# genome/breakdancer

Hardware: AMD Instinct MI355X
Metric: read-pairs/s, records resident in HBM -> scored SV table (SURVEY 8d timing i); end to end from BAM: config.timings.bam_to_table (vs_baseline is taken there) (higher is better)
Workload: dtype int32

## Files before the change

breakdancer_amd/csrc/bdx_api.hip:

```cpp
#include <hip/hip_runtime.h>

#include <algorithm>
#include <sys/mman.h>
#include <atomic>
#include <functional>
#include <chrono>
#include <cmath>
#include <cstdio>
#include <cstddef>
#include <cstring>
#include <string>
#include <thread>
#include <unordered_map>
#include <utility>
#include <vector>

#include "../../include/bdx.h"
#include "bdx_dev.h"
#include "bdx_k3.h"
#include "bdx_shard.h"
#include "bdx_scan.h"
#include "bdx_walk.h"
#include "bdx_bam_dev.h"

using namespace bdx;

namespace {

inline bool alloc_trace() { static const bool on = getenv("BDX_ALLOC_TRACE") != nullptr; return on; }

struct DevBuf {
    void* p = nullptr;
    size_t bytes = 0;
    hipError_t ensure(size_t b) {
        if (b <= bytes) return hipSuccess;
        const auto t0 = std::chrono::steady_clock::now();
        const bool had = p != nullptr;
        if (p) (void)hipFree(p);
        p = nullptr;
        bytes = 0;
        size_t want = b + b / 8 + 256;
        hipError_t e = hipMalloc(&p, want);
        if (alloc_trace()) fprintf(stderr, "[bdx alloc] device %12zu B %8.1f us%s\n", want, std::chrono::duration<double, std::micro>(std::chrono::steady_clock::now() - t0).count(), had ? " (regrown: hipFree first)" : "");
        if (e == hipSuccess) bytes = want;
        return e;
    }
    void release() { if (p) (void)hipFree(p); p = nullptr; bytes = 0; }
    template <class T> T* as() const { return (T*)p; }
};

struct PinBuf {
    void* p = nullptr;
    size_t bytes = 0;
    void* map_base = nullptr;
    size_t map_len = 0;
    static std::atomic<bool>& registered_switch() { static std::atomic<bool> on{true}; return on; }
    static bool use_registered() { return registered_switch().load(std::memory_order_relaxed); }
    hipError_t ensure(size_t b) {
        if (b <= bytes) return hipSuccess;
        release();
        size_t want = b + b / 8 + 256;
        const auto t0 = std::chrono::steady_clock::now();
        hipError_t e = hipErrorOutOfMemory;
        constexpr size_t kHuge = (size_t)2 << 20;
        if (want >= 2 * kHuge && use_registered()) {
            const size_t len = (want + kHuge - 1) & ~(kHuge - 1);
            void* base = mmap(nullptr, len + kHuge, PROT_READ | PROT_WRITE, MAP_PRIVATE | MAP_ANONYMOUS, -1, 0);
            if (base != MAP_FAILED) {
                void* al = (void*)(((uintptr_t)base + kHuge - 1) & ~(uintptr_t)(kHuge - 1));
                (void)madvise(al, len, MADV_HUGEPAGE);
                for (size_t o = 0; o < len; o += 4096) ((volatile char*)al)[o] = 0;
                void* dev = nullptr;
                if (hipHostRegister(al, len, hipHostRegisterMapped) == hipSuccess && hipHostGetDevicePointer(&dev, al, 0) == hipSuccess && dev == al) {
                    p = al; map_base = base; map_len = len + kHuge; want = len; e = hipSuccess;
                } else {
                    (void)hipHostUnregister(al);
                    (void)hipGetLastError();
                    munmap(base, len + kHuge);
                }
            }
        }
        if (e != hipSuccess) {
            e = hipHostMalloc(&p, want, hipHostMallocDefault);
            if (e == hipSuccess && want <= ((size_t)1 << 20)) memset(p, 0, want);
        }
        if (alloc_trace()) fprintf(stderr, "[bdx alloc] pinned %12zu B %8.1f us%s\n", want, std::chrono::duration<double, std::micro>(std::chrono::steady_clock::now() - t0).count(), map_base ? " (registered huge pages)" : "");
        if (e == hipSuccess) bytes = want; else p = nullptr;
        return e;
    }
    void release() {
        if (p && map_base) { (void)hipHostUnregister(p); munmap(map_base, map_len); }
        else if (p) (void)hipHostFree(p);
        p = nullptr; bytes = 0; map_base = nullptr; map_len = 0;
    }
    template <class T> T* as() const { return (T*)p; }
};

constexpr int kNumStages = 12;
constexpr int kK1MaxGrid = 8192;
constexpr uint32_t kK1EventPeriod = 4;

}

struct bdx_ctx {
    int device = 0;
    hipStream_t stream = nullptr;
    bdx_opts opts{};
    std::vector<bdx_lib> libs;
    int nlibs = 0, nbams = 0, ntids = 0, nkeys = 0, w0 = 0;
    std::string err;

    ReadsSoA d{};
    size_t n = 0, cap = 0;
    bool adopted = false;
    DevBuf b_tid, b_pos, b_mtid, b_mpos, b_isize, b_flag, b_qlen, b_mapq, b_lib, b_bam, b_key, b_check;
    bool groups_in_hbm = false;
    bool defer_walk = false;
    DevBuf b_groups;
    bool use_check = false;

    DevBuf b_libs, b_cls, b_tile_tot, b_tile_pre, b_tile_mono, b_blk_cnt, b_cnt, b_p1, b_fold, b_stash, b_chunk_tot;
    DevBuf b_c_tid, b_c_pos, b_c_isize, b_c_meta, b_c_key, b_c_check, b_c_idx, b_c_nn, b_c_pk;
    DevBuf b_cand, b_pre_q, b_pre_rev, b_pre_nonctx, b_c_first, b_c_maxq, b_c_rid, b_region_of, b_counts;
    DevBuf b_bcnt, b_boff, b_bcur, b_e_key, b_e_idx, b_partner, b_t_key, b_t_idx;
    DevBuf b_x_key, b_x_check, b_x_order, b_x_region, b_x_meta, b_x_isize, b_x_n;
    DevBuf b_lib_mean;
    DevBuf b_r_rec, b_r_pk, b_out_deg, b_parts, b_kdens, b_rs, b_slot, b_members, b_own, b_lib_stage, b_cn_stage,
        b_t_lambda, b_t_k, b_ws6;
    PinBuf h_p1, h_cnt, h_counts, h_regs, h_pk, h_groups, h_terms;
    DevBuf b_sv_src, b_dlists, b_ltail, b_pair_lo;
    PinBuf h_hs_rec, h_hs_aux, h_hs_lists, h_printed;
    DevBuf b_ins, b_member_ids;
    PinBuf h_flags;
    uint32_t seq = 0;
    int dbg_no_stash = 0, dbg_max_chunks = 0, dbg_ins_plain = 0, dbg_gather_walk = 0, dbg_regions_copy = 0, dbg_asm_plain = 0;
    uint32_t lb_seq = 0;
    float k1_ms_last = 0;
    bool k1_timed = false;
    bool stage_timing = false;
    bool poll = true;
    bool materialized = true;
    bool rows_packed = false;
    uint32_t n_sv_total = 0, n_groups_total = 0, n_terms_total = 0, n_cn_total = 0;
    PinBuf h_counts0, h_counts2, h_sv_out, h_lib_index, h_lib_pairs, h_cn_key, h_cn_value, h_ltail_dev;
    hipEvent_t ev_groups = nullptr, ev_regions = nullptr;
    int big_walk_mode = -1;
    int64_t last_big_groups = -1;
    FinalizeParams fp_deferred{};
    bool finalize2_deferred = false;
    bool bucketed_join = false;
    bool host_walk_only = false;
    K6Arrays k6{};
    const GroupRec* k6_in_groups = nullptr;
    const uint32_t* k6_in_goff = nullptr;
    bool force_direct_join = false;
    uint32_t k6_cap = 0;
    const RegionRec* k6_r_rec = nullptr;
    const uint32_t* k6_r_pk = nullptr;
    uint8_t* k6_taint = nullptr;
    const uint32_t* k3_tid_tail = nullptr;
    bool table_in_hbm = false;
    DevBuf b_sv_out, b_lib_index_out, b_lib_pairs_out, b_cn_key_out, b_cn_value_out, b_ltail_out, b_sv_key;

    bool ran = false;
    Pass1 p1{};
    StageCounts counts{};
    std::vector<uint32_t> cnt;
    std::vector<uint32_t> cnt_local;
    uint32_t g_covered = 0;
    int32_t g_window = 0;
    uint32_t nn_base = 0;
    int stage = 0;
    uint32_t ntiles = 0, tstride = 0;
    Compact cp{};
    K3Arrays k3{};
    K4Arrays k4{};
    std::vector<double> log_tail;
    bool collect_support = false;
    std::vector<uint32_t> ov_cnt;
    uint32_t ov_covered = 0;
    bool replayed = false;
    bool use_stash = false;
    std::atomic<int> sizing{0};
    std::string sizing_err;
    std::vector<uint32_t> sup_off;
    std::vector<uint64_t> sup_idx;
    std::vector<uint8_t> sup_flag;
    std::vector<float> seqcov, lib_density, key_density;
    std::vector<HostRegion> regions;
    std::vector<uint32_t> r_pk;
    const HostRegion* reg = nullptr;
    size_t nreg = 0;
    const uint32_t* rpk = nullptr;
    std::vector<GroupPart> parts;
    WalkResult walk;
    WalkScratch* walk_scratch = nullptr;
    uint32_t n_printed = 0;
    uint32_t n_sv_host = 0;
    int speculate = 2;
    int spec_test = 0;
    uint32_t last_na = 0;
    size_t last_n = 0;
    uint32_t na_alloc = 0;
    bool region_of_fused = false;
    uint32_t join_table_clean = 0;
    float stage_ms[kNumStages] = {0};
    hipEvent_t ev[8] = {nullptr};

    hipStream_t copy_stream = nullptr;
    hipEvent_t ev_copy = nullptr;
    bool copy_pending = false;
    bool k1_live = false;
    uint32_t k1_done = 0, k1_cap_tiles = 0;
    struct Stage {
        PinBuf buf;
        size_t cap = 0;
        hipEvent_t done = nullptr;
        bool busy = false;
    };
    Stage ring[4];
    int ring_next = 0, ring_cur = -1;
    struct KeySeg { uint64_t begin; const uint64_t* host; const uint16_t* host_qlen; const uint64_t* host_check; };
    std::vector<KeySeg> key_segs;
    DevBuf b_seg, b_lb;

    size_t cls_n = (size_t)-1;
    DevBuf b_jq, b_jc;
};

namespace {

thread_local std::string* t_err_sink = nullptr;
int fail(bdx_ctx* c, int code, const std::string& msg) {
    if (t_err_sink) *t_err_sink = msg;
    else if (c) c->err = msg;
    return code;
}
struct Sizing { uint32_t na; };
#define NOT_WHILE_SIZING(c)                                                                                                              \
    do {                                                                                                                                 \
        if ((c)->sizing.load(std::memory_order_acquire))                                                                                 \
            return fail(c, BDX_ESTATE, "the buffers of the later stages are being sized on another thread (bdx_bamdec_finish has not returned)"); \
    } while (0)
int hipfail(bdx_ctx* c, hipError_t e, const char* what) {
    return fail(c, BDX_EHIP, std::string(what) + ": " + hipGetErrorString(e));
}
#define HIPCHK(ctx, expr)                                   \
    do {                                                    \
        hipError_t _e = (expr);                             \
        if (_e != hipSuccess) return hipfail(ctx, _e, #expr); \
    } while (0)

size_t round_up(size_t x, size_t m) { return (x + m - 1) / m * m; }

hipError_t next_lb_stamp(bdx_ctx* c, uint32_t* out) {
    if (((++c->lb_seq) & 0x3FFFFFFFu) == 0) {
        if (c->b_lb.p) { const hipError_t e = hipMemsetAsync(c->b_lb.p, 0, c->b_lb.bytes, c->stream); if (e != hipSuccess) return e; }
        if (c->b_ws6.p) { const hipError_t e = hipMemsetAsync(c->b_ws6.p, 0, c->b_ws6.bytes, c->stream); if (e != hipSuccess) return e; }
        ++c->lb_seq;
    }
    *out = c->lb_seq & 0x3FFFFFFFu;
    return hipSuccess;
}

int alloc_reads(bdx_ctx* c, size_t cap) {
    cap = round_up(std::max<size_t>(cap, 1), 1024);
    if (cap <= c->cap) return BDX_OK;
    if (c->copy_stream) HIPCHK(c, hipStreamSynchronize(c->copy_stream));
    HIPCHK(c, hipStreamSynchronize(c->stream));
    c->k1_live = false;
    struct Col { DevBuf* b; size_t esz; const void** slot; };
    Col cols[] = {{&c->b_tid, 4, (const void**)&c->d.tid},     {&c->b_pos, 4, (const void**)&c->d.pos},
                  {&c->b_mtid, 4, (const void**)&c->d.mtid},   {&c->b_mpos, 4, (const void**)&c->d.mpos},
                  {&c->b_isize, 4, (const void**)&c->d.isize}, {&c->b_flag, 2, (const void**)&c->d.flag},
                  {&c->b_qlen, 2, (const void**)&c->d.qlen},   {&c->b_mapq, 1, (const void**)&c->d.mapq},
                  {&c->b_lib, 1, (const void**)&c->d.lib},     {&c->b_bam, 1, (const void**)&c->d.bam},
                  {&c->b_key, 8, (const void**)&c->d.key},     {&c->b_check, 8, (const void**)&c->d.check}};
    for (Col& col : cols) {
        if (col.b == &c->b_check && !c->use_check) continue;
        DevBuf nb;
        HIPCHK(c, nb.ensure(cap * col.esz));
        if (c->n) HIPCHK(c, hipMemcpyAsync(nb.p, col.b->p, c->n * col.esz, hipMemcpyDeviceToDevice, c->stream));
        HIPCHK(c, hipStreamSynchronize(c->stream));
        col.b->release();
        *col.b = nb;
        *col.slot = nb.p;
    }
    c->cap = cap;
    return BDX_OK;
}

void stage_view(const bdx_ctx::Stage& st, bdx_batch_buf* out) {
    char* p = (char*)st.buf.p;
    const size_t K = st.cap;
    out->name_key = (uint64_t*)p; p += K * 8;
    out->name_check = (uint64_t*)p; p += K * 8;
    out->tid = (int32_t*)p; p += K * 4;
    out->pos = (int32_t*)p; p += K * 4;
    out->mtid = (int32_t*)p; p += K * 4;
    out->mpos = (int32_t*)p; p += K * 4;
// ... 26 lines not shown
        if (tiles <= 0xFFFFFFFFull) {
            const int rc = pass1_prepare(c, (uint32_t)tiles);
            if (rc != BDX_OK) return rc;
            c->k1_live = true;
        }
    }
    hipStream_t s2 = s;
    HIPCHK(c, hipMemcpyAsync((void*)(c->d.tid + o), b.tid, n * 4, hipMemcpyHostToDevice, s));
    HIPCHK(c, hipMemcpyAsync((void*)(c->d.pos + o), b.pos, n * 4, hipMemcpyHostToDevice, s2));
    HIPCHK(c, hipMemcpyAsync((void*)(c->d.mtid + o), b.mtid, n * 4, hipMemcpyHostToDevice, s));
    HIPCHK(c, hipMemcpyAsync((void*)(c->d.mpos + o), b.mpos, n * 4, hipMemcpyHostToDevice, s2));
    HIPCHK(c, hipMemcpyAsync((void*)(c->d.isize + o), b.isize, n * 4, hipMemcpyHostToDevice, s));
    HIPCHK(c, hipMemcpyAsync((void*)(c->d.flag + o), b.flag, n * 2, hipMemcpyHostToDevice, s2));
    HIPCHK(c, hipMemcpyAsync((void*)(c->d.mapq + o), b.mapq, n, hipMemcpyHostToDevice, s2));
    if (c->nlibs > 1) HIPCHK(c, hipMemcpyAsync((void*)(c->d.lib + o), b.lib, n, hipMemcpyHostToDevice, s2));
    if (c->nbams > 1) HIPCHK(c, hipMemcpyAsync((void*)(c->d.bam + o), b.bam, n, hipMemcpyHostToDevice, s2));
    const uint64_t* dev_view = nullptr;
    const uint16_t* dev_qlen = nullptr;
    const uint64_t* dev_check = nullptr;
    if (lazy_keys && c->key_segs.size() < 64) {
        auto device_view = [](const void* hp) -> void* {
            hipPointerAttribute_t attr{};
            void* dp = nullptr;
            if (hipPointerGetAttributes(&attr, hp) == hipSuccess && attr.type == hipMemoryTypeHost &&
                hipHostGetDevicePointer(&dp, (void*)hp, 0) == hipSuccess)
                return dp;
            (void)hipGetLastError();
            return nullptr;
        };
        dev_view = (const uint64_t*)device_view(b.name_key);
        dev_qlen = dev_view ? (const uint16_t*)device_view(b.qlen) : nullptr;
        if (dev_qlen && c->use_check) dev_check = (const uint64_t*)device_view(b.name_check);
        if (!dev_qlen || (c->use_check && !dev_check)) dev_view = nullptr;
    }
    if (!dev_view) {
        HIPCHK(c, hipMemcpyAsync((void*)(c->d.key + o), b.name_key, n * 8, hipMemcpyHostToDevice, s2));
        HIPCHK(c, hipMemcpyAsync((void*)(c->d.qlen + o), b.qlen, n * 2, hipMemcpyHostToDevice, s));
        if (c->use_check) HIPCHK(c, hipMemcpyAsync((void*)(c->d.check + o), b.name_check, n * 8, hipMemcpyHostToDevice, s2));
    }
    if (c->key_segs.empty() || dev_view || c->key_segs.back().host)
        c->key_segs.push_back(bdx_ctx::KeySeg{(uint64_t)o, dev_view, dev_qlen, dev_check});
    HIPCHK(c, hipEventRecord(c->ev_copy, s));
    c->copy_pending = true;
    c->n += n;
    c->ran = false;
    if (c->k1_live) {
        const uint32_t full = (uint32_t)(c->n / kTile);
        if (full >= c->k1_done + kStreamTilesMin) {
            HIPCHK(c, hipStreamWaitEvent(c->stream, c->ev_copy, 0));
            c->copy_pending = false;
            const int rc = pass1_classify(c, full, false);
            if (rc != BDX_OK) return rc;
        }
    }
    return BDX_OK;
}

}

extern "C" {

void bdx_opts_default(bdx_opts* o) {
    if (!o) return;
    o->min_len = 7; o->cut_sd = 3; o->max_sd = 1000000000; o->min_map_qual = 35; o->min_read_pair = 2;
    o->seq_coverage_lim = 1000; o->buffer_size = 100; o->transchr_rearrange = 0; o->fisher = 0;
    o->illumina_long_insert = 0; o->cn_lib = 0; o->print_af = 0; o->score_threshold = 30; o->chr_restricted = 0;
}

const char* bdx_strerror(int code) {
    switch (code) {
        case BDX_OK: return "ok";
        case BDX_EINVAL: return "invalid argument";
        case BDX_ENOMEM: return "out of memory";
        case BDX_EHIP: return "HIP runtime error";
        case BDX_ESTATE: return "call out of order";
        case BDX_ELIMIT: return "limit exceeded";
        default: return "internal error";
    }
}
const char* bdx_last_error(const bdx_ctx* ctx) { return ctx ? ctx->err.c_str() : ""; }
int bdx_device(const bdx_ctx* ctx) { return ctx ? ctx->device : -1; }
void* bdx_stream(const bdx_ctx* ctx) { return ctx ? (void*)ctx->stream : nullptr; }

int bdx_create(bdx_ctx** out, const bdx_opts* opts, const bdx_lib* libs, int nlibs, int nbams, int ntids,
               int max_read_window_size0, int device) {
    if (!out || !opts || !libs || nlibs < 1 || nbams < 1) return BDX_EINVAL;
    if (nlibs > 255 || nbams > 254) return BDX_ELIMIT;
    const int nkeys = opts->cn_lib ? nlibs : nbams;
    if (nkeys > 60) return BDX_ELIMIT;
    for (int i = 0; i < nlibs; ++i)
        if (libs[i].bam_index < 0 || libs[i].bam_index >= nbams) return BDX_EINVAL;
    int ndev = 0;
    if (hipGetDeviceCount(&ndev) != hipSuccess || ndev <= 0 || device < 0 || device >= ndev) return BDX_EHIP;
    if (hipSetDevice(device) != hipSuccess) return BDX_EHIP;
    bdx_ctx* c = new (std::nothrow) bdx_ctx;
    if (!c) return BDX_ENOMEM;
    c->device = device;
    c->opts = *opts;
    c->libs.assign(libs, libs + nlibs);
    c->nlibs = nlibs; c->nbams = nbams; c->ntids = ntids; c->nkeys = nkeys; c->w0 = max_read_window_size0;
    if (hipStreamCreateWithFlags(&c->stream, hipStreamNonBlocking) != hipSuccess) { delete c; return BDX_EHIP; }
    for (auto& e : c->ev)
        if (hipEventCreate(&e) != hipSuccess) { delete c; return BDX_EHIP; }
    if (hipStreamCreateWithFlags(&c->copy_stream, hipStreamNonBlocking) != hipSuccess) { delete c; return BDX_EHIP; }
    if (hipEventCreateWithFlags(&c->ev_copy, hipEventDisableTiming) != hipSuccess) { delete c; return BDX_EHIP; }
    for (auto& st : c->ring)
        if (hipEventCreateWithFlags(&st.done, hipEventDisableTiming) != hipSuccess) { delete c; return BDX_EHIP; }
    if (hipEventCreateWithFlags(&c->ev_groups, hipEventDisableTiming) != hipSuccess) { delete c; return BDX_EHIP; }
    if (hipEventCreateWithFlags(&c->ev_regions, hipEventDisableTiming) != hipSuccess) { delete c; return BDX_EHIP; }
    std::vector<DevLib> dl(nlibs);
    for (int i = 0; i < nlibs; ++i) {
        dl[i].upper = libs[i].uppercutoff;
        dl[i].lower = libs[i].lowercutoff;
        dl[i].min_mapq = libs[i].min_mapping_quality < 0 ? opts->min_map_qual : libs[i].min_mapping_quality;
        dl[i].key = opts->cn_lib ? i : libs[i].bam_index;
    }
    std::vector<float> means(nlibs);
    for (int i = 0; i < nlibs; ++i) means[i] = libs[i].mean_insertsize;
    if (c->b_libs.ensure(nlibs * sizeof(DevLib)) != hipSuccess ||
        hipMemcpy(c->b_libs.p, dl.data(), nlibs * sizeof(DevLib), hipMemcpyHostToDevice) != hipSuccess ||
        c->b_lib_mean.ensure(nlibs * 4) != hipSuccess ||
        hipMemcpy(c->b_lib_mean.p, means.data(), nlibs * 4, hipMemcpyHostToDevice) != hipSuccess) {
        bdx_destroy(c);
        return BDX_EHIP;
    }
    *out = c;
    return BDX_OK;
}

void bdx_destroy(bdx_ctx* c) {
    if (!c) return;
    (void)hipSetDevice(c->device);
    if (c->copy_stream) (void)hipStreamSynchronize(c->copy_stream);
    if (c->stream) (void)hipStreamSynchronize(c->stream);
    for (auto& st : c->ring) {
        st.buf.release();
        if (st.done) (void)hipEventDestroy(st.done);
    }
    c->b_seg.release();
    c->b_lb.release();
    if (c->ev_copy) (void)hipEventDestroy(c->ev_copy);
    if (c->copy_stream) (void)hipStreamDestroy(c->copy_stream);
    DevBuf* bufs[] = {&c->b_tid, &c->b_pos, &c->b_mtid, &c->b_mpos, &c->b_isize, &c->b_flag, &c->b_qlen, &c->b_mapq, &c->b_lib,
                      &c->b_bam, &c->b_key, &c->b_check, &c->b_c_check, &c->b_x_check, &c->b_groups, &c->b_libs, &c->b_cls, &c->b_stash, &c->b_chunk_tot, &c->b_tile_tot, &c->b_tile_pre, &c->b_tile_mono,
                      &c->b_blk_cnt, &c->b_cnt, &c->b_p1, &c->b_c_tid, &c->b_c_pos, &c->b_c_isize,
                      &c->b_c_meta, &c->b_c_key, &c->b_c_idx, &c->b_c_nn, &c->b_c_pk, &c->b_cand, &c->b_pre_q, &c->b_pre_rev,
                      &c->b_pre_nonctx, &c->b_c_first, &c->b_c_maxq, &c->b_c_rid, &c->b_region_of,
                      &c->b_counts, &c->b_bcnt, &c->b_boff, &c->b_bcur, &c->b_e_key, &c->b_e_idx, &c->b_partner, &c->b_t_key,
                      &c->b_t_idx, &c->b_x_key, &c->b_x_order, &c->b_x_region,
                      &c->b_x_meta, &c->b_x_isize, &c->b_x_n, &c->b_fold, &c->b_lib_mean, &c->b_pair_lo, &c->b_sv_src, &c->b_dlists, &c->b_ltail, &c->b_r_rec, &c->b_r_pk, &c->b_out_deg,
                      &c->b_parts, &c->b_kdens, &c->b_rs, &c->b_slot, &c->b_members, &c->b_own, &c->b_lib_stage,
                      &c->b_cn_stage, &c->b_t_lambda, &c->b_t_k, &c->b_ws6, &c->b_ins, &c->b_member_ids,
                      &c->b_sv_out, &c->b_lib_index_out, &c->b_lib_pairs_out, &c->b_cn_key_out, &c->b_cn_value_out, &c->b_ltail_out, &c->b_sv_key,
                      &c->b_jq, &c->b_jc};
    for (DevBuf* b : bufs) b->release();
    PinBuf* pins[] = {&c->h_p1, &c->h_cnt, &c->h_counts, &c->h_regs, &c->h_pk, &c->h_groups, &c->h_terms, &c->h_flags, &c->h_hs_rec, &c->h_hs_aux, &c->h_hs_lists, &c->h_printed, &c->h_counts0, &c->h_counts2,
                      &c->h_sv_out, &c->h_lib_index, &c->h_lib_pairs, &c->h_cn_key, &c->h_cn_value, &c->h_ltail_dev};
    for (PinBuf* b : pins) b->release();
    if (c->walk_scratch) walk_scratch_free(c->walk_scratch);
    for (auto& e : c->ev)
        if (e) (void)hipEventDestroy(e);
    if (c->ev_groups) (void)hipEventDestroy(c->ev_groups);
    if (c->ev_regions) (void)hipEventDestroy(c->ev_regions);
    if (c->stream) (void)hipStreamDestroy(c->stream);
    delete c;
}

int bdx_reserve(bdx_ctx* c, size_t n_reads) {
    if (!c) return BDX_EINVAL;
    if (c->adopted) return fail(c, BDX_ESTATE, "reads were adopted from the caller");
    NOT_WHILE_SIZING(c);
    HIPCHK(c, hipSetDevice(c->device));
    const int rc = alloc_reads(c, n_reads);
    if (rc != BDX_OK) return rc;
    if (n_reads >= (1u << 20) && !c->ran) {
        const uint64_t prior = (uint64_t)n_reads / 32 + 4096;
        if (prior <= kMaxAnomalous) return presize_stages_here(c, (uint32_t)prior);
    }
    return BDX_OK;
}

int bdx_push(bdx_ctx* c, const bdx_batch* b) {
    if (!c || !b) return BDX_EINVAL;
    if (c->adopted) return fail(c, BDX_ESTATE, "reads were adopted from the caller");
    if (b->n == 0) return BDX_OK;
    if (!b->tid || !b->pos || !b->mtid || !b->mpos || !b->isize || !b->flag || !b->qlen || !b->mapq || !b->lib || !b->bam ||
        !b->name_key || (c->use_check && !b->name_check))
        return fail(c, BDX_EINVAL, "null array in batch");
    HIPCHK(c, hipSetDevice(c->device));
    return enqueue_batch(c, *b, true);
}

int bdx_acquire_batch(bdx_ctx* c, size_t capacity, bdx_batch_buf* out) {
    if (!c || !out || capacity == 0) return BDX_EINVAL;
    if (c->adopted) return fail(c, BDX_ESTATE, "reads were adopted from the caller");
    if (c->ring_cur >= 0) return fail(c, BDX_ESTATE, "the previous batch was not submitted");
    HIPCHK(c, hipSetDevice(c->device));
    bdx_ctx::Stage& st = c->ring[c->ring_next];
    if (st.busy) {
        HIPCHK(c, hipEventSynchronize(st.done));
        st.busy = false;
    }
    st.cap = round_up(capacity, 64);
    HIPCHK(c, st.buf.ensure(st.cap * 43 + 64));
    stage_view(st, out);
    c->ring_cur = c->ring_next;
    c->ring_next = (c->ring_next + 1) % 4;
    return BDX_OK;
}

int bdx_submit_batch(bdx_ctx* c, size_t n) {
    if (!c) return BDX_EINVAL;
    if (c->ring_cur < 0) return fail(c, BDX_ESTATE, "no batch was acquired");
    bdx_ctx::Stage& st = c->ring[c->ring_cur];
    c->ring_cur = -1;
    if (n == 0) return BDX_OK;
    HIPCHK(c, hipSetDevice(c->device));
    bdx_batch_buf v{};
    stage_view(st, &v);
    if (n > v.capacity) return fail(c, BDX_EINVAL, "more records than the acquired batch holds");
    bdx_batch b{v.tid, v.pos, v.mtid, v.mpos, v.isize, v.flag, v.qlen, v.mapq, v.lib, v.bam, v.name_key, n, v.name_check};
    const int rc = enqueue_batch(c, b, false);
    if (rc != BDX_OK) return rc;
    HIPCHK(c, hipEventRecord(st.done, c->copy_stream));
    st.busy = true;
    return BDX_OK;
}

int bdx_reset_reads(bdx_ctx* c) {
    if (!c) return BDX_EINVAL;
    HIPCHK(c, hipSetDevice(c->device));
    if (c->copy_stream) HIPCHK(c, hipStreamSynchronize(c->copy_stream));
    HIPCHK(c, hipStreamSynchronize(c->stream));
    if (c->adopted) {
        c->d = ReadsSoA{};
        c->cap = 0;
        c->adopted = false;
    }
    c->n = 0;
    c->ran = false;
    c->cls_n = (size_t)-1;
    c->k1_live = false;
    c->k1_done = 0;
    c->copy_pending = false;
    c->key_segs.clear();
    c->ring_cur = -1;
    for (auto& st : c->ring) st.busy = false;
    return BDX_OK;
}

int bdx_set_device_reads(bdx_ctx* c, const bdx_batch* b) {
    if (!c || !b) return BDX_EINVAL;
    if (c->n && !c->adopted) return fail(c, BDX_ESTATE, "context already holds pushed reads");
    const void* ptrs[] = {b->tid, b->pos, b->mtid, b->mpos, b->isize, b->flag, b->qlen, b->mapq, b->lib, b->bam, b->name_key,
                          c->use_check ? (const void*)b->name_check : (const void*)b->name_key};
    for (const void* p : ptrs)
        if (b->n && (!p || ((uintptr_t)p & 15))) return fail(c, BDX_EINVAL, "device arrays must be non-null and 16-byte aligned");
    c->d.tid = b->tid; c->d.pos = b->pos; c->d.mtid = b->mtid; c->d.mpos = b->mpos; c->d.isize = b->isize;
    c->d.flag = b->flag; c->d.qlen = b->qlen; c->d.mapq = b->mapq; c->d.lib = b->lib; c->d.bam = b->bam; c->d.key = b->name_key;
    c->d.check = c->use_check ? b->name_check : nullptr;
    c->n = b->n;
    c->cap = b->n;
    c->adopted = true;
    c->ran = false;
    c->cls_n = (size_t)-1;
    c->k1_live = false;
    c->key_segs.clear();
    return BDX_OK;
}

}

namespace {

bool wait_flag(const bdx_ctx* c, int idx, uint32_t value) {
    if (!c->poll || !c->h_flags.p) return false;
    volatile uint32_t* f = (volatile uint32_t*)c->h_flags.p + idx;
    const auto t0 = std::chrono::steady_clock::now();
    for (uint32_t spin = 0;; ++spin) {
        if (*f == value) { std::atomic_thread_fence(std::memory_order_acquire); return true; }
        __builtin_ia32_pause();
        if ((spin & 1023u) == 1023u && std::chrono::steady_clock::now() - t0 > std::chrono::milliseconds(200)) return false;
    }
}

bool flag_arrived(const bdx_ctx* c, int idx) {
    return !c->poll || !c->h_flags.p || ((volatile uint32_t*)c->h_flags.p)[idx] == c->seq;
}

int signal_ready(bdx_ctx* c, int idx, hipEvent_t ev) {
    if (c->poll) {
        if (hipStreamWriteValue32(c->stream, c->h_flags.as<uint32_t>() + idx, c->seq, 0) == hipSuccess) return BDX_OK;
        (void)hipGetLastError();
        c->poll = false;
    }
    if (ev) {
        hipError_t e = hipEventRecord(ev, c->stream);
        if (e != hipSuccess) return hipfail(c, e, "hipEventRecord");
    }
    return BDX_OK;
}

float ms_between(std::chrono::steady_clock::time_point a, std::chrono::steady_clock::time_point b) {
    return std::chrono::duration<float, std::milli>(b - a).count();
}

int do_pass1(bdx_ctx* c, uint32_t na_cap = 0, bool wait = true, bool defer_second = false);
int wait_pass1(bdx_ctx* c);

int pass1_prepare(bdx_ctx* c, uint32_t tiles_cap) {
    HIPCHK(c, hipSetDevice(c->device));
    hipStream_t s = c->stream;
    const int nlibs = c->nlibs, nbams = c->nbams, nkeys = c->nkeys;
    const int ncols = 2 + nkeys, ncnt = nlibs * kNumFlags + nlibs + nbams;
    const uint32_t tstride = (uint32_t)round_up(std::max<uint32_t>(tiles_cap, 16), 16);
    c->tstride = tstride;
    c->k1_cap_tiles = tiles_cap;
    c->k1_done = 0;
    HIPCHK(c, c->b_cls.ensure(std::max<size_t>((size_t)tiles_cap * kTile, 16)));
    c->use_stash = !c->dbg_no_stash && nkeys <= kStashKeys;
    if (c->use_stash) HIPCHK(c, c->b_stash.ensure(std::max<size_t>((size_t)tiles_cap * kStashCap * sizeof(StashRec), 64)));
    HIPCHK(c, c->b_tile_tot.ensure((size_t)ncols * tstride * 4));
    HIPCHK(c, c->b_tile_pre.ensure((size_t)ncols * tstride * 4));
    HIPCHK(c, c->b_tile_mono.ensure((size_t)nbams * tstride * sizeof(MonoRec)));
    HIPCHK(c, c->b_blk_cnt.ensure((size_t)kCntCopies * ncnt * 4));
    HIPCHK(c, c->b_cnt.ensure((size_t)ncnt * 4));
    HIPCHK(c, c->b_p1.ensure(sizeof(Pass1)));
    HIPCHK(c, c->h_p1.ensure(sizeof(Pass1)));
    HIPCHK(c, c->h_cnt.ensure((size_t)ncnt * 4));
    HIPCHK(c, c->h_counts.ensure(sizeof(StageCounts)));
    HIPCHK(c, c->b_counts.ensure(sizeof(StageCounts)));
    const size_t w_tot = (size_t)ncols * tstride, w_mono = (size_t)nbams * tstride * sizeof(MonoRec) / 4;
    if (w_tot > 0xFFFFFFFFull || w_mono > 0xFFFFFFFFull) {
        HIPCHK(c, hipMemsetAsync(c->b_tile_tot.p, 0, w_tot * 4, s));
        HIPCHK(c, hipMemsetAsync(c->b_tile_mono.p, 0xFF, w_mono * 4, s));
    }
    InitList il{};
    int k = 0;
    auto add = [&](void* p, size_t words, uint32_t value) { il.ptr[k] = (uint32_t*)p; il.words[k] = (uint32_t)words; il.value[k] = value; ++k; };
    if (w_tot <= 0xFFFFFFFFull && w_mono <= 0xFFFFFFFFull) { add(c->b_tile_tot.p, w_tot, 0u); add(c->b_tile_mono.p, w_mono, 0xFFFFFFFFu); }
    add(c->b_blk_cnt.p, (size_t)kCntCopies * ncnt, 0u);
    add(c->b_p1.p, sizeof(Pass1) / 4, 0u);
    add(c->b_counts.p, sizeof(StageCounts) / 4, 0u);
    il.n = k;
    launch_init(il, s);
    return BDX_OK;
}

int pass1_classify(bdx_ctx* c, uint32_t upto, bool timed) {
    hipStream_t s = c->stream;
    if (upto <= c->k1_done) return BDX_OK;
    K1Params k1{};
    k1.r = c->d; k1.n = c->n; k1.ntiles = upto; k1.tstride = c->tstride; k1.tile0 = c->k1_done;
    k1.nlibs = c->nlibs; k1.nbams = c->nbams; k1.nkeys = c->nkeys;
    k1.max_sd = c->opts.max_sd; k1.opt_t = c->opts.transchr_rearrange; k1.opt_l = c->opts.illumina_long_insert;
    k1.libs = c->b_libs.as<DevLib>(); k1.cls = c->b_cls.as<uint8_t>(); k1.tile_tot = c->b_tile_tot.as<uint32_t>();
    k1.tile_mono = c->b_tile_mono.as<MonoRec>();
    k1.blk_cnt = c->b_blk_cnt.as<uint32_t>();
    k1.stash = c->use_stash ? c->b_stash.as<StashRec>() : nullptr;
    const uint32_t span = upto - c->k1_done;
    const int grid1 = (int)std::min<uint32_t>((span + kWaves - 1) / kWaves, (uint32_t)kK1MaxGrid);
    launch_k1(k1, grid1, k1_lds_bytes(c->nlibs, c->nbams, c->nkeys), s, timed ? c->ev[0] : nullptr, timed ? c->ev[1] : nullptr);
    c->k1_done = upto;
    return BDX_OK;
}

int do_pass1(bdx_ctx* c, uint32_t na_cap, bool wait, bool defer_second) {
    HIPCHK(c, hipSetDevice(c->device));
    hipStream_t s = c->stream;
    const int nlibs = c->nlibs, nbams = c->nbams, nkeys = c->nkeys;
    const int ncols = 2 + nkeys, ncnt = nlibs * kNumFlags + nlibs + nbams;
    if (c->n >= ((size_t)1 << 32)) return fail(c, BDX_ELIMIT, "more than 2^32 - 1 reads in one context (read indices and the prefix counters are 32-bit)");
    const uint32_t ntiles = (uint32_t)((c->n + kTile - 1) / kTile);
    c->ntiles = ntiles;
    c->ran = false; c->stage = 0; c->replayed = false;
    c->cls_n = (size_t)-1;
    c->na_alloc = 0;
    c->regions.clear(); c->r_pk.clear(); c->parts.clear();
    c->reg = nullptr; c->nreg = 0; c->rpk = nullptr;
    c->walk.clear();
    if (!c->walk_scratch) c->walk_scratch = walk_scratch_new();
    c->n_printed = 0;
    memset(&c->counts, 0, sizeof(c->counts));
    for (float& m : c->stage_ms) m = 0;

    if (c->copy_pending) {
        HIPCHK(c, hipStreamWaitEvent(s, c->ev_copy, 0));
        c->copy_pending = false;
    }
    if (!(c->k1_live && c->k1_cap_tiles >= ntiles)) {
        const int rc = pass1_prepare(c, ntiles);
        if (rc != BDX_OK) return rc;
    }
    c->k1_live = false;
    const uint32_t tstride = c->tstride;
    const bool time_k1 = (c->stage_timing || c->seq % kK1EventPeriod == 0) && c->k1_done == 0 && ntiles > 0;
    {
        const int rc = pass1_classify(c, ntiles, time_k1);
        if (rc != BDX_OK) return rc;
    }
    FinalizeParams fp{};
    fp.ntiles = ntiles; fp.tstride = tstride; fp.nblk = 0;
    fp.nfold = std::max<uint32_t>(1, std::min<uint32_t>(64, (ntiles + 1023) / 1024));
    HIPCHK(c, c->b_fold.ensure((size_t)nbams * fp.nfold * sizeof(MonoRec)));
    fp.fold_part = c->b_fold.as<MonoRec>();
    fp.nlibs = nlibs; fp.nbams = nbams; fp.nkeys = nkeys; fp.ncols = ncols; fp.ncnt = ncnt; fp.w0 = c->w0;
    fp.tile_tot = c->b_tile_tot.as<uint32_t>(); fp.tile_pre = c->b_tile_pre.as<uint32_t>(); fp.tile_mono = c->b_tile_mono.as<MonoRec>();
    {
        const uint32_t nsuper = (ntiles + kK2TilesPerWave - 1) / kK2TilesPerWave;
        const uint32_t round = 4096;
        const uint32_t rounds = std::max<uint32_t>(1, (nsuper + round - 1) / round);
        const uint32_t max_chunks = c->dbg_max_chunks > 0 ? (uint32_t)std::min(c->dbg_max_chunks, (int)kMaxChunks) : (uint32_t)kMaxChunks;
        fp.chunk_super = round * ((rounds + max_chunks - 1) / max_chunks);
        fp.nchunk = std::max<uint32_t>(1, (nsuper + fp.chunk_super - 1) / fp.chunk_super);
        HIPCHK(c, c->b_chunk_tot.ensure((size_t)ncols * kMaxChunks * 8));
        fp.chunk_tot = c->b_chunk_tot.as<uint32_t>();
        fp.chunk_base = fp.chunk_tot + (size_t)ncols * kMaxChunks;
    }
    fp.blk_cnt = c->b_blk_cnt.as<uint32_t>(); fp.cnt = c->b_cnt.as<uint32_t>(); fp.p1 = c->b_p1.as<Pass1>();
    HIPCHK(c, c->b_kdens.ensure(64 * 4));
    fp.libs = c->b_libs.as<DevLib>(); fp.cn_lib = c->opts.cn_lib; fp.key_density = c->b_kdens.as<float>();
    fp.cnt_host = c->h_cnt.as<uint32_t>(); fp.p1_host = c->h_p1.as<Pass1>();
    memset(c->h_p1.p, 0, sizeof(Pass1));
    HIPCHK(c, c->h_flags.ensure(64));
    ++c->seq;
    fp.flag_host = c->h_flags.as<uint32_t>(); fp.flag_value = c->seq;
    fp.na_cap = na_cap;
    c->fp_deferred = fp;
    c->finalize2_deferred = defer_second;
    launch_finalize(fp, s, !defer_second);
    c->k1_timed = time_k1;
    return wait ? wait_pass1(c) : BDX_OK;
}

int wait_pass1(bdx_ctx* c) {
    const int ncnt = c->nlibs * kNumFlags + c->nlibs + c->nbams;
    if (!wait_flag(c, 0, c->seq)) {
        HIPCHK(c, hipStreamSynchronize(c->stream));
        if (c->h_flags.p && *((volatile uint32_t*)c->h_flags.p) != c->seq) return fail(c, BDX_EINTERNAL, "the pass-1 record did not arrive: its kernel was not launched");
    }
    c->p1 = *c->h_p1.as<Pass1>();
    c->cnt_local.assign(c->h_cnt.as<uint32_t>(), c->h_cnt.as<uint32_t>() + ncnt);
    if (c->k1_timed) {
        float ms = 0;
        if (hipEventElapsedTime(&ms, c->ev[0], c->ev[1]) == hipSuccess) c->k1_ms_last = ms;
    }
    c->stage_ms[0] = c->k1_ms_last;
    if (c->p1.n_anom > kMaxAnomalous) return fail(c, BDX_ELIMIT, "more than 2^31 anomalous reads in one context");
    if (!c->na_alloc && c->p1.n_anom) c->na_alloc = (uint32_t)std::min<uint64_t>((uint64_t)c->p1.n_anom + c->p1.n_anom / 8 + 1024, kMaxAnomalous);
    c->stage = 1;
    c->cls_n = c->n;
    return BDX_OK;
}

int32_t window_from(const bdx_ctx* c, const uint32_t* cnt, uint32_t covered) {
    int W = c->w0;
    for (int i = 0; i < c->nlibs; ++i) {
        const int nd = (int)(cnt[i * kNumFlags + F_LARGE] + cnt[i * kNumFlags + F_SMALL]);
        const int tmp = nd > 0 ? (int)((float)covered / (float)nd) : 50;
        W = std::min(W, tmp);
    }
    return W;
}

int set_pass1(bdx_ctx* c, const uint32_t* cnt, uint32_t covered, int32_t window, bool upload) {
    const int nlibs = c->nlibs, nkeys = c->nkeys;
    const int ncnt = nlibs * kNumFlags + nlibs + c->nbams;
    c->cnt.assign(cnt, cnt + ncnt);
    c->g_covered = covered;
    c->g_window = window;
    const uint32_t* lib_cnt = c->cnt.data() + nlibs * kNumFlags;
    const uint32_t* bam_cnt = lib_cnt + nlibs;
    c->seqcov.assign(nlibs, 0.f);
    c->lib_density.assign(nlibs, 0.f);
    c->key_density.assign(nkeys, 0.000001f);
    for (int i = 0; i < nlibs; ++i) {
        float covg = 0;
        if (lib_cnt[i] != 0 && covered != 0) covg = float(lib_cnt[i]) * c->libs[i].readlens / covered;
        c->seqcov[i] = covg;
        float dens = 0.000001f;
        if (c->opts.cn_lib) {
            if (lib_cnt[i] != 0) dens = float(lib_cnt[i]) / covered;
        } else {
            dens = float(bam_cnt[c->libs[i].bam_index]) / covered;
        }
        c->lib_density[i] = dens;
        c->key_density[c->opts.cn_lib ? i : c->libs[i].bam_index] = dens;
    }
    struct { uint32_t covered; int32_t window; } hdr{covered, window};
    static_assert(offsetof(Pass1, covered_ref_len) == 0 && offsetof(Pass1, window) == 4, "Pass1 header layout");
    if (upload) {
        HIPCHK(c, hipMemcpyAsync(c->b_p1.p, &hdr, sizeof(hdr), hipMemcpyHostToDevice, c->stream));
        HIPCHK(c, hipStreamSynchronize(c->stream));
    }
    c->stage = 2;
    return BDX_OK;
}

int do_compact(bdx_ctx* c, uint32_t nn_base, const uint32_t* pk_base, bool prepare_join, const Sizing* sz = nullptr) {
    HIPCHK(c, hipSetDevice(c->device));
    hipStream_t s = c->stream;
    const int nkeys = c->nkeys;
    const uint32_t na = sz ? sz->na : c->na_alloc;
    if (c->stage_timing && !sz) HIPCHK(c, hipEventRecord(c->ev[2], s));
    Compact cp_sz{};
    K3Arrays k3_sz{};
    Compact& cp = sz ? cp_sz : c->cp;
    K3Arrays& k3 = sz ? k3_sz : c->k3;
    cp = Compact{};
    k3 = K3Arrays{};
    if (na) {
        if (na > kMaxAnomalous) return fail(c, BDX_ELIMIT, "more than 2^31 anomalous reads in one context");
        const size_t cap = na;
        HIPCHK(c, c->b_c_tid.ensure(cap * 4)); HIPCHK(c, c->b_c_pos.ensure(cap * 4)); HIPCHK(c, c->b_c_isize.ensure(cap * 4));
        HIPCHK(c, c->b_c_meta.ensure(cap * 4)); HIPCHK(c, c->b_c_key.ensure(cap * 8)); HIPCHK(c, c->b_c_nn.ensure(cap * 4));
        HIPCHK(c, c->b_c_idx.ensure(cap * 4));
        if (c->use_check) HIPCHK(c, c->b_c_check.ensure(cap * 8));
        HIPCHK(c, c->b_c_pk.ensure(cap * 4 * nkeys));
        cp.tid = c->b_c_tid.as<int32_t>(); cp.pos = c->b_c_pos.as<int32_t>(); cp.isize = c->b_c_isize.as<int32_t>();
        cp.meta = c->b_c_meta.as<uint32_t>(); cp.key = c->b_c_key.as<uint64_t>(); cp.nn = c->b_c_nn.as<uint32_t>();
        cp.idx = c->b_c_idx.as<uint32_t>();
        cp.check = c->use_check ? c->b_c_check.as<uint64_t>() : nullptr;
        cp.pk = c->b_c_pk.as<uint32_t>(); cp.cap = na;
        K2Params k2{};
        k2.r = c->d; k2.n = c->n; k2.ntiles = c->ntiles; k2.tstride = c->tstride; k2.nkeys = nkeys; k2.nlibs = c->nlibs; k2.libs = c->b_libs.as<DevLib>();
        k2.cls = c->b_cls.as<uint8_t>(); k2.tile_pre = c->b_tile_pre.as<uint32_t>(); k2.c = cp;
        k2.tile_tot = c->b_tile_tot.as<uint32_t>(); k2.stash = c->use_stash ? c->b_stash.as<StashRec>() : nullptr;
        k2.chunk_tot = c->fp_deferred.chunk_tot; k2.chunk_base = c->fp_deferred.chunk_base; k2.chunk_super = c->fp_deferred.chunk_super;
        k2.nn_base = nn_base;
        for (int k = 0; k < nkeys; ++k) k2.pk_base[k] = pk_base ? pk_base[k] : 0u;
        HIPCHK(c, c->b_c_maxq.ensure(cap * 4));
        k2.fill_ptr[0] = c->b_c_maxq.as<uint32_t>(); k2.fill_words[0] = na; k2.fill_value[0] = 0u;
        if (!sz) c->join_table_clean = 0;
        if (prepare_join && (c->force_direct_join || (!c->bucketed_join && na <= kDirectJoinMax))) {
            const uint32_t slots = direct_join_slots(na);
            HIPCHK(c, c->b_t_key.ensure((size_t)slots * 8)); HIPCHK(c, c->b_partner.ensure((size_t)na * 4));
            k2.fill_ptr[1] = c->b_t_key.as<uint32_t>(); k2.fill_words[1] = 2 * slots; k2.fill_value[1] = 0xFFFFFFFFu;
            k2.fill_ptr[2] = c->b_partner.as<uint32_t>(); k2.fill_words[2] = na; k2.fill_value[2] = 0xFFFFFFFFu;
            HIPCHK(c, c->b_pair_lo.ensure((size_t)na * 4));
            k2.fill_ptr[3] = c->b_pair_lo.as<uint32_t>(); k2.fill_words[3] = na; k2.fill_value[3] = 0xFFFFFFFFu;
            if (!sz) c->join_table_clean = slots;
        }
        if (sz) return BDX_OK;
        {
            bool any_host = false;
            for (auto const& sg : c->key_segs) any_host |= sg.host != nullptr;
            if (any_host && !c->adopted) {
                const size_t ns = c->key_segs.size();
                std::vector<uint64_t> tab(4 * ns + 1);
                for (size_t i = 0; i < ns; ++i) {
                    const bdx_ctx::KeySeg& sg = c->key_segs[i];
                    tab[i] = sg.begin;
                    tab[ns + 1 + i] = (uint64_t)(uintptr_t)(sg.host ? sg.host - sg.begin : c->d.key);
                    tab[2 * ns + 1 + i] = (uint64_t)(uintptr_t)(sg.host ? sg.host_qlen - sg.begin : c->d.qlen);
                    tab[3 * ns + 1 + i] = (uint64_t)(uintptr_t)(sg.host ? sg.host_check - sg.begin : c->d.check);
                }
                tab[ns] = c->n;
                HIPCHK(c, c->b_seg.ensure(tab.size() * 8));
                HIPCHK(c, hipMemcpyAsync(c->b_seg.p, tab.data(), tab.size() * 8, hipMemcpyHostToDevice, s));
                HIPCHK(c, hipStreamSynchronize(s));
                k2.nseg = (int)ns;
                k2.seg_begin = c->b_seg.as<uint64_t>();
                k2.seg_ptr = (const uint64_t* const*)(c->b_seg.as<uint64_t>() + ns + 1);
                k2.seg_qlen = (const uint16_t* const*)(c->b_seg.as<uint64_t>() + 2 * ns + 1);
                k2.seg_check = (const uint64_t* const*)(c->b_seg.as<uint64_t>() + 3 * ns + 1);
            }
        }
        launch_k2(k2, k2_lds_bytes(nkeys), s, c->finalize2_deferred ? &c->fp_deferred : nullptr);
        c->finalize2_deferred = false;
    }
    if (sz) return BDX_OK;
    if (c->finalize2_deferred) {
        launch_finalize2_only(c->fp_deferred, s);
        c->finalize2_deferred = false;
    }
    if (c->stage_timing) HIPCHK(c, hipEventRecord(c->ev[3], s));
    c->nn_base = nn_base;
    return BDX_OK;
}

// ... 84 lines not shown
    K4Arrays& k4 = sz ? k4_sz : c->k4;
    k4 = K4Arrays{};
    if (!n) return BDX_OK;
    k4.g_cap = n / 2 + 1;
    if (c->groups_in_hbm) {
        HIPCHK(c, c->b_groups.ensure((size_t)k4.g_cap * sizeof(GroupRec)));
        k4.g_rec = c->b_groups.as<GroupRec>();
    } else {
        HIPCHK(c, c->h_groups.ensure((size_t)k4.g_cap * sizeof(GroupRec)));
        k4.g_rec = c->h_groups.as<GroupRec>();
    }
    const size_t n_own = en.n_local ? std::min<size_t>(n, std::max<uint32_t>(c->na_alloc, 1u)) : n;
    HIPCHK(c, c->b_partner.ensure(n_own * 4));
    k4.partner = c->b_partner.as<int32_t>();
    if (sz) return BDX_OK;
    if (c->force_direct_join || (!c->bucketed_join && n <= kDirectJoinMax)) {
        uint32_t slots = direct_join_slots(n);
        if (c->join_table_clean && (uint64_t)n * 2 <= c->join_table_clean) slots = c->join_table_clean;
        const bool want_lo = en.c_rid || en.want_pair_lo;
        if (c->join_table_clean != slots) {
            HIPCHK(c, c->b_t_key.ensure((size_t)slots * 8));
            HIPCHK(c, hipMemsetAsync(c->b_t_key.p, 0xFF, (size_t)slots * 8, s));
            HIPCHK(c, hipMemsetAsync(c->b_partner.p, 0xFF, n_own * 4, s));
            if (en.want_pair_lo) {
                HIPCHK(c, c->b_pair_lo.ensure(n_own * 4));
                HIPCHK(c, hipMemsetAsync(c->b_pair_lo.p, 0xFF, n_own * 4, s));
            }
        }
        k4.pair_lo = ((c->join_table_clean == slots && want_lo) || en.want_pair_lo) ? c->b_pair_lo.as<int32_t>() : nullptr;
        c->join_table_clean = 0;
        k4.direct = 1; k4.t_mask = slots - 1;
        k4.t_key = c->b_t_key.as<uint64_t>(); k4.t_idx = c->b_t_idx.as<int32_t>();
        if (join_only) launch_k4_join_only(k4, en, n_ptr, n, c->b_counts.as<StageCounts>(), s);
        else launch_k4(k4, en, n_ptr, n, c->b_counts.as<StageCounts>(), s);
        return BDX_OK;
    }
    uint32_t nb = 1, lg = 0;
    while (nb < (uint32_t)kMaxBuckets && (size_t)nb * 384 < n) { nb <<= 1; ++lg; }
    k4.nbuckets = nb; k4.log2b = lg;
    if ((size_t)nb * 4 > c->b_bcnt.bytes) {
        HIPCHK(c, c->b_bcnt.ensure((size_t)kMaxBuckets * 4));
        HIPCHK(c, hipMemsetAsync(c->b_bcnt.p, 0, c->b_bcnt.bytes, s));
    }
    HIPCHK(c, c->b_boff.ensure((nb + 1) * 4)); HIPCHK(c, c->b_bcur.ensure(nb * 4));
    HIPCHK(c, c->b_e_key.ensure((size_t)n * 8)); HIPCHK(c, c->b_e_idx.ensure((size_t)n * 4));
    HIPCHK(c, c->b_t_key.ensure((size_t)n * 16)); HIPCHK(c, c->b_t_idx.ensure((size_t)n * 8));
    k4.bcnt = c->b_bcnt.as<uint32_t>(); k4.boff = c->b_boff.as<uint32_t>(); k4.bcur = c->b_bcur.as<uint32_t>();
    k4.e_key = c->b_e_key.as<uint64_t>(); k4.e_idx = c->b_e_idx.as<uint32_t>();
    k4.t_key = c->b_t_key.as<uint64_t>(); k4.t_idx = c->b_t_idx.as<int32_t>();
    if (join_only) launch_k4_join_only(k4, en, n_ptr, n, c->b_counts.as<StageCounts>(), s);
    else launch_k4(k4, en, n_ptr, n, c->b_counts.as<StageCounts>(), s);
    return BDX_OK;
}

int readback(bdx_ctx* c, bool with_groups) {
    hipStream_t s = c->stream;
    const uint32_t na = c->p1.n_anom;
    if (!na) return BDX_OK;
    HIPCHK(c, hipMemcpyAsync(c->h_counts.p, c->b_counts.p, sizeof(StageCounts), hipMemcpyDeviceToHost, s));
    HIPCHK(c, hipStreamSynchronize(s));
    HIPCHK(c, hipGetLastError());
    c->counts = *c->h_counts.as<StageCounts>();
    if (c->counts.overflow) return fail(c, BDX_EINTERNAL, "group list overflow");
    (void)with_groups;
    return BDX_OK;
}

constexpr uint32_t kBorrowRegionsMin = 32768;
void decode_regions(bdx_ctx* c, const RegionRec* rr, const uint32_t* pk, uint32_t nr, uint32_t ph, bool borrow) {
    static_assert(sizeof(HostRegion) == sizeof(RegionRec) && offsetof(HostRegion, first) == offsetof(RegionRec, first), "region layout");
    const int nkeys = c->nkeys;
    if (borrow && !ph) {
        c->reg = (const HostRegion*)rr; c->nreg = nr; c->rpk = pk;
        return;
    }
    c->regions.resize(nr + ph);
    if (ph) c->regions[0] = HostRegion{-1, -1, -1, 0, 0, 0, 0, 0, 0};
    if (nr) memcpy(c->regions.data() + ph, rr, (size_t)nr * sizeof(RegionRec));
    c->r_pk.assign((size_t)ph * 2 * nkeys, 0u);
    c->r_pk.insert(c->r_pk.end(), pk, pk + (size_t)nr * 2 * nkeys);
    c->reg = c->regions.data(); c->nreg = c->regions.size(); c->rpk = c->r_pk.data();
}

void decode_groups(bdx_ctx* c, const GroupRec* gr, uint32_t ng, uint32_t ph) {
    c->parts.resize(ng);
    for (uint32_t i = 0; i < ng; ++i) {
        const uint64_t k = gr[i].key;
        c->parts[i] = GroupPart{(uint32_t)(k >> 38) + ph, (uint32_t)((k >> 12) & ((1u << 26) - 1)) + ph, (uint8_t)(k & 15),
                                (uint8_t)((k >> 4) & 255), gr[i].pairs, gr[i].sum_isize};
    }
}

int do_k6(bdx_ctx* c, bool force_host, int part = 0, const Sizing* sz = nullptr, int rounds = 0) {
    hipStream_t s = c->stream;
    K6Arrays a_sz{};
    K6Arrays& a = sz ? a_sz : c->k6;
    if (part == 2) {
        if (!a.cap) return BDX_OK;
        launch_k6_components(a, a.cap, s);
        if (!c->poll) {
            const int rc = signal_ready(c, 1, c->ev_groups);
            if (rc != BDX_OK) return rc;
        }
        if (!c->defer_walk) launch_k6_walk(a, a.cap, s);
        return BDX_OK;
    }
    if (part == 3) {
        if (a.cap) launch_k6_walk(a, a.cap, s);
        return BDX_OK;
    }
    const uint32_t na = std::max(sz ? sz->na : c->na_alloc, c->k6_cap);
    const int nkeys = c->nkeys, nlibs = c->nlibs;
    a = K6Arrays{};
    if (!na) return BDX_OK;
    const size_t cap = na;
    HIPCHK(c, c->b_out_deg.ensure(cap * 6 * 4));
    HIPCHK(c, c->b_parts.ensure(cap * sizeof(PartRec)));
    HIPCHK(c, c->b_rs.ensure(cap * sizeof(RegSum)));
    HIPCHK(c, c->b_members.ensure(cap * kK6MaxMembers * sizeof(MemberInfo)));
    HIPCHK(c, c->b_own.ensure(cap * 7 * 4 + 64 * 4 * 4));
    const int big_walk = c->big_walk_mode >= 0 ? c->big_walk_mode : (c->last_big_groups >= 0 ? c->last_big_groups > 2000 : na > 500000u);
    if (big_walk) HIPCHK(c, c->b_member_ids.ensure(cap * kK6BigMembers * 4));
    a.sv_cap = na / 2 + 1; a.term_cap = na / 2 + 1; a.cn_cap = (na / 2 + 1) * (uint32_t)nkeys;
    a.lib_stride = (uint32_t)std::min(nlibs, kK6LibStride);
    HIPCHK(c, c->b_slot.ensure(cap * sizeof(SvOut)));
    HIPCHK(c, c->b_lib_stage.ensure(cap * a.lib_stride * sizeof(LibStage)));
    HIPCHK(c, c->b_cn_stage.ensure(cap * (size_t)nkeys * sizeof(CnStage) + 16));
    HIPCHK(c, c->b_t_lambda.ensure((size_t)a.term_cap * 8)); HIPCHK(c, c->b_t_k.ensure((size_t)a.term_cap * 4));
    const size_t nblk = scan_grid(na, 1) + 1;
    if (c->table_in_hbm) {
        HIPCHK(c, c->b_sv_out.ensure((size_t)a.sv_cap * sizeof(SvOut))); HIPCHK(c, c->b_sv_key.ensure((size_t)a.sv_cap * 8));
        HIPCHK(c, c->b_lib_index_out.ensure((size_t)a.term_cap * 4)); HIPCHK(c, c->b_lib_pairs_out.ensure((size_t)a.term_cap * 4));
        HIPCHK(c, c->b_cn_key_out.ensure((size_t)a.cn_cap * 4 + 16)); HIPCHK(c, c->b_cn_value_out.ensure((size_t)a.cn_cap * 4 + 16));
        HIPCHK(c, c->b_ltail_out.ensure((size_t)a.term_cap * 8));
    } else {
        HIPCHK(c, c->h_sv_out.ensure((size_t)a.sv_cap * sizeof(SvOut)));
        HIPCHK(c, c->h_lib_index.ensure((size_t)a.term_cap * 4)); HIPCHK(c, c->h_lib_pairs.ensure((size_t)a.term_cap * 4));
        HIPCHK(c, c->h_cn_key.ensure((size_t)a.cn_cap * 4 + 16)); HIPCHK(c, c->h_cn_value.ensure((size_t)a.cn_cap * 4 + 16));
        HIPCHK(c, c->h_ltail_dev.ensure((size_t)a.term_cap * 8));
    }
    HIPCHK(c, c->h_counts2.ensure(sizeof(StageCounts)));
    HIPCHK(c, c->b_sv_src.ensure((size_t)a.sv_cap * 16)); HIPCHK(c, c->b_ltail.ensure((size_t)a.term_cap * 8));
    HIPCHK(c, c->b_dlists.ensure((size_t)a.term_cap * 4 + (size_t)a.cn_cap * 8 + 64));
    {
        size_t p2 = 1;
        while (p2 < a.sv_cap) p2 <<= 1;
        const size_t svc = a.sv_cap;
        const size_t nsort = std::min<size_t>(svc, kK6RankSortMax);
        HIPCHK(c, c->b_ins.ensure(p2 * 12 + svc * 8 + (svc + 1) * 16 + nsort * 12 + nsort * 4 * kK6RankSlices + 64));
        a.old_key = c->b_ins.as<uint64_t>(); a.hs_key_dev = a.old_key + p2;
        a.old_slot = (uint32_t*)(a.hs_key_dev + svc); a.ins_T = a.old_slot + p2; a.ins_src = a.ins_T + svc + 1;
        a.ins_pre_l = a.ins_src + svc + 1; a.ins_pre_c = a.ins_pre_l + svc + 1;
        a.sorted_key = (uint64_t*)(((uintptr_t)(a.ins_pre_c + svc + 1) + 7) & ~(uintptr_t)7); a.sorted_slot = (uint32_t*)(a.sorted_key + nsort);
        a.rank_part = a.sv_cap > 2048u ? a.sorted_slot + nsort : nullptr;
    }
    a.sv_begin = c->b_sv_src.as<uint2>(); a.sv_src = (uint32_t*)(a.sv_begin + a.sv_cap); a.ltail = c->b_ltail.as<double>();
    a.d_lib_index = c->b_dlists.as<int32_t>(); a.d_cn_key = a.d_lib_index + a.term_cap; a.d_cn_value = (float*)(a.d_cn_key + a.cn_cap);
    a.cap = na;
    a.r_rec = c->k6_r_rec ? c->k6_r_rec : c->b_r_rec.as<RegionRec>(); a.r_pk = c->k6_r_pk ? c->k6_r_pk : c->b_r_pk.as<uint32_t>();
    a.taint = c->k6_taint;
    a.region_of = c->k3.region_of; a.partner = c->k4.partner; a.pair_lo = c->k4.pair_lo; a.meta = c->cp.meta; a.isize = c->cp.isize;
    a.in_groups = c->k6_in_groups; a.in_goff = c->k6_in_goff; a.first_of = c->k6_in_groups ? c->k6_in_goff : nullptr;
    a.parts = c->b_parts.as<PartRec>();
    a.rs = c->b_rs.as<RegSum>();
    a.out_deg = c->b_out_deg.as<uint32_t>(); a.label = a.out_deg + cap; a.bad_v = a.out_deg + 2 * cap; a.bad = a.out_deg + 3 * cap;
    a.mcount = a.out_deg + 4 * cap; a.pcount = a.out_deg + 5 * cap;
    a.members = c->b_members.as<MemberInfo>();
    a.own_nsv = c->b_own.as<uint32_t>(); a.own_nacc = a.own_nsv + cap; a.own_ncn = a.own_nsv + 2 * cap; a.own_first = a.own_nsv + 3 * cap; a.slot_next = a.own_nsv + 4 * cap; a.owners = a.own_nsv + 5 * cap; a.owners_big = a.own_nsv + 6 * cap; a.emit_part = a.own_nsv + 7 * cap;
    a.member_ids = big_walk ? c->b_member_ids.as<uint32_t>() : nullptr;
    a.sv_stage = c->b_slot.as<SvOut>(); a.lib_stage = c->b_lib_stage.as<LibStage>(); a.cn_stage = c->b_cn_stage.as<CnStage>();
    if (c->table_in_hbm) {
        a.sv_out = c->b_sv_out.as<SvOut>(); a.lib_index = c->b_lib_index_out.as<int32_t>(); a.lib_pairs = c->b_lib_pairs_out.as<int32_t>();
        a.cn_key = c->b_cn_key_out.as<int32_t>(); a.cn_value = c->b_cn_value_out.as<float>();
        a.sv_key = c->b_sv_key.as<unsigned long long>();
    } else {
        a.sv_out = c->h_sv_out.as<SvOut>(); a.lib_index = c->h_lib_index.as<int32_t>(); a.lib_pairs = c->h_lib_pairs.as<int32_t>();
        a.cn_key = c->h_cn_key.as<int32_t>(); a.cn_value = c->h_cn_value.as<float>();
    }
    a.sv_vx = a.sv_key ? a.sv_src + a.sv_cap : nullptr;
    a.t_lambda = c->b_t_lambda.as<double>(); a.t_k = c->b_t_k.as<int32_t>();
    a.g_rec = c->k4.g_rec; a.g_cap = c->k4.g_cap;
    {
        const size_t words = 4 * nblk;
        if (c->b_ws6.bytes < words * 8) {
            HIPCHK(c, c->b_ws6.ensure(words * 8));
            HIPCHK(c, hipMemsetAsync(c->b_ws6.p, 0, c->b_ws6.bytes, s));
        }
        a.lb_state = c->b_ws6.as<unsigned long long>();
        if (!sz) HIPCHK(c, next_lb_stamp(c, &a.lb_stamp));
    }
    if (sz) return BDX_OK;
    a.counts = c->b_counts.as<StageCounts>();
    a.hist = c->b_cnt.as<uint32_t>();
    a.key_density = c->b_kdens.as<float>();
    a.lib_mean = c->b_lib_mean.as<float>();
    a.counts_host = c->h_counts.as<StageCounts>();
    a.counts_host2 = c->h_counts2.as<StageCounts>();
    memset(c->h_counts.p, 0, sizeof(StageCounts));
    memset(c->h_counts2.p, 0, sizeof(StageCounts));
    a.p1 = c->b_p1.as<Pass1>();
    a.nlibs = nlibs; a.nkeys = nkeys; a.min_read_pair = c->opts.min_read_pair; a.chr_restricted = c->opts.chr_restricted;
    a.period = std::max(1, c->opts.buffer_size + 1);
    a.force_host = force_host ? 1 : 0;
    a.big_walk = big_walk;
    a.ins_plain = c->dbg_ins_plain;
    a.asm_plain = c->dbg_asm_plain;
    a.propagation_rounds = rounds ? rounds : (a.big_walk ? kK6LabelRoundsBig : kK6LabelRounds);
    if (c->poll) {
        a.flag_value = c->seq;
        a.flag_groups = c->h_flags.as<uint32_t>() + 1;
        if (c->k3.host_copy_later) a.flag_regions = c->h_flags.as<uint32_t>() + 3;
        a.mirror_in_walk = (force_host || c->defer_walk) ? 0 : 1;
    }
    if (part == 4) return BDX_OK;
    if (part == 1) {
        launch_k6_pairs(a, na, s);
        return BDX_OK;
    }
    launch_k6_groups(a, na, s);
    if (!c->poll) {
        const int rc = signal_ready(c, 1, c->ev_groups);
        if (rc != BDX_OK) return rc;
    }
    launch_k6_walk(a, na, s);
    return BDX_OK;
}

int presize_stages(bdx_ctx* c, uint32_t na) {
    struct Guard {
        bdx_ctx* c;
        std::string* keep;
        explicit Guard(bdx_ctx* c_) : c(c_), keep(t_err_sink) { c->sizing.fetch_add(1, std::memory_order_acq_rel); c->sizing_err.clear(); t_err_sink = &c->sizing_err; }
        ~Guard() { t_err_sink = keep; c->sizing.fetch_sub(1, std::memory_order_acq_rel); }
    } guard(c);
    const Sizing sz{na};
    int r = do_compact(c, 0, nullptr, true, &sz);
    if (r == BDX_OK) r = do_cut(c, 0, 0, 0, true, false, &sz);
    if (r == BDX_OK) r = do_join_local(c, na, Entries{}, nullptr, true, &sz);
    if (r == BDX_OK) r = do_k6(c, false, 0, &sz);
    return r;
}

int presize_stages_here(bdx_ctx* c, uint32_t na) {
    const int r = presize_stages(c, na);
    if (r != BDX_OK) c->err = c->sizing_err;
    return r;
}

int do_k6_table(bdx_ctx* c) {
    hipStream_t s = c->stream;
    K6Arrays& a = c->k6;
    const uint32_t na = a.cap;
    if (!na) return BDX_OK;
    const WalkResult& H = c->walk;
    const uint32_t nh = (uint32_t)H.svs.size(), nt = (uint32_t)H.terms.size(), nc = (uint32_t)H.cn_key.size();
    a.nh = nh;
    if (nh) {
        const uint64_t period = (uint64_t)std::max(1, c->opts.buffer_size + 1);
        HIPCHK(c, c->h_hs_rec.ensure((size_t)nh * sizeof(SvOut)));
        HIPCHK(c, c->h_hs_aux.ensure((size_t)nh * 12 + 16));
        HIPCHK(c, c->h_hs_lists.ensure((size_t)nt * 16 + (size_t)nc * 8 + 16));
        memcpy(c->h_hs_rec.p, H.svs.data(), (size_t)nh * sizeof(HostSv));
        uint64_t* hkey = c->h_hs_aux.as<uint64_t>();
        uint32_t* hcnt = (uint32_t*)(hkey + nh);
        for (uint32_t j = 0; j < nh; ++j) {
            const uint64_t key = H.sv_key[j];
            const bool from_old = !((key >> 32) & 1ull);
            const uint64_t start = key & 0xffffffffull;
            const uint64_t T = from_old ? (key >> 33) * period : start;
            hkey[j] = (T << 34) | (from_old ? 0ull : 1ull << 33) | (start << 7);
            if (a.force_host) hkey[j] = 0;
            hcnt[j] = (uint32_t)H.svs[j].sv.lib_count | ((uint32_t)H.svs[j].sv.cn_count << 16);
        }
        double* lam = c->h_hs_lists.as<double>();
        int32_t* li = (int32_t*)(lam + nt);
        int32_t* lp = li + nt;
        int32_t* ck = lp + nt;
        float* cv = (float*)(ck + nc);
        for (uint32_t i = 0; i < nt; ++i) { lam[i] = H.terms[i].lambda; li[i] = H.lib_index[i]; lp[i] = H.lib_pairs[i]; }
        for (uint32_t i = 0; i < nc; ++i) { ck[i] = H.cn_key[i]; cv[i] = H.cn_value[i]; }
        a.hs_rec = c->h_hs_rec.as<SvOut>(); a.hs_key = hkey; a.hs_cnt = hcnt;
        a.hs_lambda = lam; a.hs_lib_index = li; a.hs_lib_pairs = lp; a.hs_cn_key = ck; a.hs_cn_value = cv;
    }
    a.ltail_host = c->table_in_hbm ? c->b_ltail_out.as<double>() : (c->opts.fisher ? c->h_ltail_dev.as<double>() : nullptr);
    a.fin_regions = (c->counts.n_regions && c->counts.n_regions <= na) ? c->counts.n_regions : na;
    HIPCHK(c, c->h_printed.ensure((size_t)k6_score_grid(a) * 4));
    a.printed_host = c->h_printed.as<uint32_t>();
    if (c->poll) { a.flag_done = c->h_flags.as<uint32_t>() + 2; a.flag_value = c->seq; }
    a.wire_rows = c->table_in_hbm ? 0 : 1;
    c->rows_packed = a.wire_rows != 0;
    launch_k6_table(a, na, std::log(10), c->opts.score_threshold, c->opts.fisher ? 0 : 1, s);
    if (!a.flag_done) {
        const int rc = signal_ready(c, 2, nullptr);
        if (rc != BDX_OK) return rc;
    }
    return BDX_OK;
}

int materialize(bdx_ctx* c) {
    if (c->materialized) return BDX_OK;
    WalkResult& M = c->walk;
    M.clear();
    const uint32_t n = c->n_sv_total, nt = c->n_terms_total, nc = c->n_cn_total;
    if (c->rows_packed) {
        const SvWire* w = c->h_sv_out.as<SvWire>();
        M.svs.resize(n);
        int32_t lb = 0, cb = 0;
        for (uint32_t i = 0; i < n; ++i) {
            const SvWire& r = w[i];
            HostSv& o = M.svs[i];
            bdx_sv& v = o.sv;
            const HostRegion& ra = c->reg[r.region[0]];
            const HostRegion& rb = r.region[1] >= 0 ? c->reg[r.region[1]] : ra;
            v.chr[0] = ra.tid; v.chr[1] = rb.tid;
            v.pos[0] = r.pos[0]; v.pos[1] = r.pos[1];
            v.fwd[0] = (int32_t)(ra.n - ra.rev); v.rev[0] = (int32_t)ra.rev;
            v.fwd[1] = (int32_t)(rb.n - rb.rev); v.rev[1] = (int32_t)rb.rev;
            v.flag = (int32_t)((r.bits >> 16) & 15u); v.size = r.size; v.score = r.score; v.num_reads = r.num_reads; v.printed = (int32_t)((r.bits >> 23) & 1u);
            v.region[0] = r.region[0]; v.region[1] = r.region[1];
            v.lib_begin = lb; v.lib_count = (int32_t)(r.bits & 255u); lb += v.lib_count;
            v.cn_begin = cb; v.cn_count = (int32_t)((r.bits >> 8) & 255u); cb += v.cn_count;
            v.allele_frequency = r.allele_frequency; v.logp = r.logp;
            o.grp_mask = (r.bits >> 20) & 7u; o.start = r.start;
        }
    } else {
        const HostSv* d = c->h_sv_out.as<HostSv>();
        M.svs.assign(d, d + n);
    }
    M.lib_index.assign(c->h_lib_index.as<int32_t>(), c->h_lib_index.as<int32_t>() + nt);
    M.lib_pairs.assign(c->h_lib_pairs.as<int32_t>(), c->h_lib_pairs.as<int32_t>() + nt);
    M.cn_key.assign(c->h_cn_key.as<int32_t>(), c->h_cn_key.as<int32_t>() + nc);
    M.cn_value.assign(c->h_cn_value.as<float>(), c->h_cn_value.as<float>() + nc);
    if (c->opts.fisher) c->log_tail.assign(c->h_ltail_dev.as<double>(), c->h_ltail_dev.as<double>() + nt); else c->log_tail.clear();
    M.n_groups = c->n_groups_total;
    c->materialized = true;
    return BDX_OK;
}

int finish_table(bdx_ctx* c) {
    hipStream_t s = c->stream;
    const auto tf0 = std::chrono::steady_clock::now();
    if (!wait_flag(c, 2, c->seq)) {
        HIPCHK(c, hipStreamSynchronize(s));
        if (!flag_arrived(c, 2)) return fail(c, BDX_EINTERNAL, "the SV table did not arrive: its kernels were not launched");
    }
    const auto tf1 = std::chrono::steady_clock::now();
    static_assert(sizeof(HostSv) == sizeof(SvOut) && offsetof(HostSv, grp_mask) == offsetof(SvOut, grp_mask) &&
                      offsetof(HostSv, start) == offsetof(SvOut, start), "SV record layout");
    c->n_sv_host = (uint32_t)c->walk.svs.size();
    c->n_groups_total = c->walk.n_groups + c->counts.n_groups_dev;
    const StageCounts c2 = *c->h_counts2.as<StageCounts>();
    if (c2.overflow) return fail(c, BDX_EINTERNAL, "SV list overflow");
    c->n_sv_total = c2.n_sv_dev; c->n_terms_total = c2.n_terms_dev; c->n_cn_total = c2.n_cn_dev;
    c->counts.n_sv_dev = c2.n_sv_dev - c->n_sv_host;
    {
        const uint32_t g = c->k6.printed_host ? k6_score_grid(c->k6) : 0u;
        const uint32_t* pb = c->k6.printed_host;
        uint32_t np = 0;
        for (uint32_t i = 0; i < g; ++i) np += pb[i];
        c->n_printed = np;
    }
    c->counts.n_old = c2.n_old;
    c->materialized = false;
    if (c->opts.fisher && !c->table_in_hbm) {
        materialize(c);
        finish_scores(c->opts, c->log_tail.data(), c->walk.svs.data(), c->walk.svs.size(), &c->n_printed);
    }
    const auto tf2 = std::chrono::steady_clock::now();
    c->stage_ms[8] = ms_between(tf0, tf1);
    c->stage_ms[9] = ms_between(tf1, tf2);
    c->stage_ms[10] = 0;
    c->ran = true;
    c->stage = 4;
    return BDX_OK;
}

int host_walk(bdx_ctx* c, int32_t last_maxq, bool any_anomalous) {
    HIPCHK(c, hipSetDevice(c->device));
    WalkInput wi{};
    wi.opts = c->opts; wi.libs = c->libs.data(); wi.nlibs = c->nlibs; wi.nbams = c->nbams; wi.nkeys = c->nkeys;
    wi.hist = c->cnt.data(); wi.covered_ref_len = c->g_covered; wi.key_density = c->key_density.data();
    wi.regions = c->reg; wi.nregions = c->nreg; wi.r_pk = c->rpk; wi.parts = &c->parts; wi.last_maxq = last_maxq;
    wi.any_anomalous = any_anomalous;
    c->walk.clear();
    if (!c->parts.empty()) greedy_walk(wi, c->walk_scratch, c->walk);
    return BDX_OK;
}

int score_host_terms(bdx_ctx* c) {
    hipStream_t s = c->stream;
    const uint32_t nt = (uint32_t)c->walk.terms.size();
    if (nt) {
        HIPCHK(c, c->h_terms.ensure((size_t)nt * 20 + 16));
        double* hl = c->h_terms.as<double>();
        int32_t* hk = (int32_t*)(hl + nt);
        double* ho = (double*)((char*)c->h_terms.p + (((size_t)nt * 12 + 7) & ~(size_t)7));
        for (uint32_t i = 0; i < nt; ++i) { hl[i] = c->walk.terms[i].lambda; hk[i] = c->walk.terms[i].k; }
        launch_k5(hl, hk, ho, nt, s);
    }
    return BDX_OK;
}

int finish_host_walk(bdx_ctx* c) {
    hipStream_t s = c->stream;
    HIPCHK(c, hipStreamSynchronize(s));
    HIPCHK(c, hipGetLastError());
    const uint32_t nt = (uint32_t)c->walk.terms.size();
    const double* host_tail = nt ? (const double*)((char*)c->h_terms.p + (((size_t)nt * 12 + 7) & ~(size_t)7)) : nullptr;
    c->log_tail.assign(host_tail, host_tail + nt);
    finish_scores(c->opts, c->log_tail.data(), c->walk.svs.data(), c->walk.svs.size(), &c->n_printed);
    c->n_sv_host = c->n_sv_total = (uint32_t)c->walk.svs.size();
    c->n_terms_total = nt; c->n_cn_total = (uint32_t)c->walk.cn_key.size();
    c->n_groups_total = c->walk.n_groups;
    c->counts.n_sv_dev = 0;
    c->materialized = true;
    c->ran = true;
    c->stage = 4;
    return BDX_OK;
}

int collect_support(bdx_ctx* c, uint32_t ph) {
    c->sup_off.assign(1, 0);
    c->sup_idx.clear();
    c->sup_flag.clear();
    const uint32_t na = c->p1.n_anom;
    std::vector<int32_t> partner(na), region_of(na);
    std::vector<uint32_t> idx(na), meta(na);
    if (na) {
        HIPCHK(c, hipMemcpy(partner.data(), c->k4.partner, (size_t)na * 4, hipMemcpyDeviceToHost));
        HIPCHK(c, hipMemcpy(region_of.data(), c->k3.region_of, (size_t)na * 4, hipMemcpyDeviceToHost));
        HIPCHK(c, hipMemcpy(idx.data(), c->cp.idx, (size_t)na * 4, hipMemcpyDeviceToHost));
        HIPCHK(c, hipMemcpy(meta.data(), c->cp.meta, (size_t)na * 4, hipMemcpyDeviceToHost));
    }
    std::vector<std::pair<uint32_t, uint32_t>> pairs;
    for (const HostSv& hs : c->walk.svs) {
        pairs.clear();
        const uint32_t rA = (uint32_t)hs.sv.region[0], rB = (uint32_t)hs.sv.region[1];
        const uint32_t glo[3] = {rA, rA, rB}, ghi_[3] = {rA, rB, rB};
        for (uint32_t g = 0; g < 3; ++g) {
            if (!(hs.grp_mask & (1u << g))) continue;
            const uint32_t lo = glo[g], hi = ghi_[g];
            const uint32_t f = c->reg[hi].first, n = c->reg[hi].n;
            for (uint32_t j = f; j < f + n; ++j) {
                const int32_t p = partner[j];
                if (p < 0 || (uint32_t)p >= j) continue;
                if ((uint32_t)(region_of[p] + (int32_t)ph) != lo) continue;
                pairs.emplace_back(j, (uint32_t)p);
            }
        }
        std::sort(pairs.begin(), pairs.end());
        for (auto const& pr : pairs) {
            c->sup_idx.push_back(idx[pr.first]); c->sup_flag.push_back((uint8_t)meta_flag(meta[pr.first]));
            c->sup_idx.push_back(idx[pr.second]); c->sup_flag.push_back((uint8_t)meta_flag(meta[pr.second]));
        }
        c->sup_off.push_back((uint32_t)c->sup_idx.size());
    }
    return BDX_OK;
}

int replay_arrays(bdx_ctx* c, uint32_t na, const uint64_t* key, const int32_t* region_of, const uint32_t* meta, const int32_t* isize, uint32_t ph,
                  std::vector<uint32_t>* sup) {
    ReadWalkInput ri{};
    WalkInput& wi = ri.base;
    wi.opts = c->opts; wi.libs = c->libs.data(); wi.nlibs = c->nlibs; wi.nbams = c->nbams; wi.nkeys = c->nkeys;
    wi.hist = c->cnt.data(); wi.covered_ref_len = c->g_covered; wi.key_density = c->key_density.data();
    wi.regions = c->reg; wi.nregions = c->nreg; wi.r_pk = c->rpk; wi.parts = nullptr; wi.last_maxq = c->counts.last_maxq;
    wi.any_anomalous = na != 0;
    ri.n_reads = na; ri.key = key; ri.region_of = region_of; ri.meta = meta; ri.isize = isize;
    ri.phantom = ph;
    if (sup) { ri.support_off = &c->sup_off; ri.support = sup; }
    c->walk.clear();
    read_level_walk(ri, c->walk);
    c->counts.n_groups = 0; c->counts.n_pairs = 0;
    int rc = score_host_terms(c);
    if (rc == BDX_OK) rc = finish_host_walk(c);
    if (rc != BDX_OK) return rc;
    c->replayed = true;
    return BDX_OK;
}

void unify_names(uint64_t* key, const uint64_t* check, size_t n) {
    struct PairHash {
        size_t operator()(const std::pair<uint64_t, uint64_t>& p) const { return (size_t)(p.first ^ (p.second * 0x9E3779B97F4A7C15ull)); }
    };
    std::unordered_map<std::pair<uint64_t, uint64_t>, uint64_t, PairHash> ids;
    ids.reserve(n);
    for (size_t i = 0; i < n; ++i) key[i] = ids.emplace(std::make_pair(key[i], check[i]), (uint64_t)ids.size()).first->second;
}

int replay_reads(bdx_ctx* c, uint32_t ph) {
    hipStream_t s = c->stream;
    HIPCHK(c, hipStreamSynchronize(s));
    const uint32_t na = c->p1.n_anom;
    std::vector<uint64_t> key(na);
    std::vector<int32_t> region_of(na), isize(na);
    std::vector<uint32_t> meta(na);
    HIPCHK(c, hipMemcpy(key.data(), c->cp.key, (size_t)na * 8, hipMemcpyDeviceToHost));
    HIPCHK(c, hipMemcpy(region_of.data(), c->k3.region_of, (size_t)na * 4, hipMemcpyDeviceToHost));
    HIPCHK(c, hipMemcpy(meta.data(), c->cp.meta, (size_t)na * 4, hipMemcpyDeviceToHost));
    HIPCHK(c, hipMemcpy(isize.data(), c->cp.isize, (size_t)na * 4, hipMemcpyDeviceToHost));
    if (c->cp.check && na) {
        std::vector<uint64_t> check(na);
        HIPCHK(c, hipMemcpy(check.data(), c->cp.check, (size_t)na * 8, hipMemcpyDeviceToHost));
        unify_names(key.data(), check.data(), na);
    }
    if (ph)
        for (int32_t& r : region_of)
            if (r >= 0) r += (int32_t)ph;
    std::vector<uint32_t> sup;
    int rc = replay_arrays(c, na, key.data(), region_of.data(), meta.data(), isize.data(), ph, c->collect_support ? &sup : nullptr);
    if (rc != BDX_OK) return rc;
    if (c->collect_support) {
        std::vector<uint32_t> idx(na);
        HIPCHK(c, hipMemcpy(idx.data(), c->cp.idx, (size_t)na * 4, hipMemcpyDeviceToHost));
        c->sup_idx.resize(sup.size());
// ... 604 lines not shown
```

breakdancer_amd/csrc/bdx_dev.h:

```cpp
#pragma once
#include <hip/hip_runtime.h>
#include <stdint.h>

namespace bdx {

constexpr int kTile = 256;
constexpr int kBlock = 256;
constexpr int kWaves = kBlock / 64;
constexpr int kNumFlags = 11;
constexpr int kK2TilesPerWave = 4;
constexpr int kCntCopies = 64;
constexpr int kMaxChunks = 64;
constexpr int kStashCap = 16;
constexpr int kStashKeys = 2;

struct StashRec {
    int32_t tid, pos, isize;
    uint32_t meta;
    uint32_t where;
    uint32_t proper;
    uint32_t pad[2];
};
static_assert(sizeof(StashRec) == 32, "two 16-byte stores");

enum : int { F_NA = 0, F_FF = 1, F_LARGE = 2, F_SMALL = 3, F_RF = 4, F_RR = 5, F_NORMAL_FR = 6, F_NORMAL_RF = 7,
             F_CTX = 8, F_MATE_UNMAPPED = 9, F_UNMAPPED = 10 };

struct DevLib {
    float upper, lower;
    int32_t min_mapq;
    int32_t key;
};

struct ReadsSoA {
    const int32_t *tid, *pos, *mtid, *mpos, *isize;
    const uint16_t *flag, *qlen;
    const uint8_t *mapq, *lib, *bam;
    const uint64_t* key;
    const uint64_t* check;
};

struct MonoRec {
    int32_t ft, fp, lt, lp;
    long long sum;
};

constexpr int kColAnom = 0, kColNormal = 1, kColKey0 = 2;

struct K1Params {
    ReadsSoA r;
    uint64_t n;
    uint32_t ntiles, tstride;
    uint32_t tile0;
    int nlibs, nbams, nkeys;
    int max_sd, opt_t, opt_l;
    const DevLib* libs;
    uint8_t* cls;
    uint32_t* tile_tot;
    MonoRec* tile_mono;
    uint32_t* blk_cnt;
    StashRec* stash;
};

struct Pass1 {
    uint32_t covered_ref_len;
    int32_t window;
    uint32_t n_anom;
    uint32_t n_normal;
    uint32_t key_tot[60];
    unsigned long long ref_len[256];
};

struct FinalizeParams {
    uint32_t ntiles, tstride, nblk;
    uint32_t nfold;
    MonoRec* fold_part;
    int nlibs, nbams, nkeys, ncols, ncnt;
    int w0;
    const uint32_t* tile_tot;
    uint32_t* tile_pre;
    uint32_t* chunk_tot;
    uint32_t* chunk_base;
    uint32_t chunk_super, nchunk;
    const MonoRec* tile_mono;
    const uint32_t* blk_cnt;
    uint32_t* cnt;
    Pass1* p1;
    uint32_t* cnt_host;
    Pass1* p1_host;
    const DevLib* libs;
    int cn_lib;
    float* key_density;
    uint32_t* flag_host;
    uint32_t flag_value;
    uint32_t na_cap;
};

struct InitList {
    uint32_t* ptr[6];
    uint32_t words[6];
    uint32_t value[6];
    int n;
};
void launch_init(const InitList& l, hipStream_t s);

struct Compact {
    int32_t* tid;
    int32_t* pos;
    int32_t* isize;
    uint32_t* meta;
    uint64_t* key;
    uint64_t* check;
    uint32_t* idx;
    uint32_t* nn;
    uint32_t* pk;
    uint32_t cap;
};

struct K2Params {
    ReadsSoA r;
    uint64_t n;
    uint32_t ntiles, tstride;
    int nkeys, nlibs;
    const DevLib* libs;
    const uint8_t* cls;
    const uint32_t* tile_pre;
    const uint32_t* chunk_tot;
    const uint32_t* chunk_base;
    uint32_t chunk_super;
    const uint32_t* tile_tot;
    const StashRec* stash;
    Compact c;
    uint32_t nn_base;
    uint32_t pk_base[60];
    uint32_t* fill_ptr[4];
    uint32_t fill_words[4];
    uint32_t fill_value[4];
    int nseg;
    const uint64_t* seg_begin;
    const uint64_t* const* seg_ptr;
    const uint16_t* const* seg_qlen;
    const uint64_t* const* seg_check;
};

__device__ __forceinline__ uint32_t meta_pack(int flag, int rev, int lib, int qlen) {
    return (uint32_t)flag | ((uint32_t)rev << 4) | ((uint32_t)lib << 8) | ((uint32_t)qlen << 16);
}
__host__ __device__ __forceinline__ int meta_flag(uint32_t m) { return m & 15; }
__host__ __device__ __forceinline__ int meta_rev(uint32_t m) { return (m >> 4) & 1; }
__host__ __device__ __forceinline__ int meta_lib(uint32_t m) { return (m >> 8) & 255; }
__host__ __device__ __forceinline__ int meta_qlen(uint32_t m) { return m >> 16; }

__device__ __forceinline__ int lane_id() { return threadIdx.x & 63; }
__device__ __forceinline__ int wave_id() { return threadIdx.x >> 6; }
__device__ __forceinline__ uint64_t ballot64(bool p) { return __builtin_amdgcn_ballot_w64(p); }
__device__ __forceinline__ int popc64(uint64_t m) { return __popcll(m); }

__device__ __forceinline__ uint32_t wave_incl_scan(uint32_t v) {
    const int l = lane_id();
#pragma unroll
    for (int o = 1; o < 64; o <<= 1) {
        uint32_t t = __shfl_up(v, o);
        if (l >= o) v += t;
    }
    return v;
}

struct K8Params {
    const int32_t *tid, *pos, *isize;
    const uint8_t* key;
    const uint8_t* cls;
    uint64_t n;
    const int32_t *q_tid, *q_a, *q_b;
    uint32_t nq;
    int nkeys;
    int32_t lmax;
    uint32_t* counts;
};

void launch_k8(const K8Params& p, hipStream_t s);
void launch_k1(const K1Params& p, int grid, size_t lds, hipStream_t s, hipEvent_t start = nullptr, hipEvent_t stop = nullptr);
size_t k1_lds_bytes(int nlibs, int nbams, int nkeys);
void launch_finalize(const FinalizeParams& p, hipStream_t s, bool second_level = true);
void launch_finalize2_only(const FinalizeParams& p, hipStream_t s);
void launch_k2(const K2Params& p, size_t lds, hipStream_t s, const FinalizeParams* side = nullptr);
size_t k2_lds_bytes(int nkeys);

}
```

breakdancer_amd/csrc/bdx_finalize.h:

```cpp
#pragma once
#include <cstddef>

#include "bdx_dev.h"

namespace bdx {

__device__ __forceinline__ MonoRec mono_combine(const MonoRec& a, const MonoRec& b) {
    if (a.ft == -1) return b;
    if (b.ft == -1) return a;
    MonoRec r;
    r.ft = a.ft; r.fp = a.fp; r.lt = b.lt; r.lp = b.lp;
    r.sum = a.sum + b.sum + (a.lt == b.ft ? (long long)b.fp - (long long)a.lp : 0ll);
    return r;
}
__device__ __forceinline__ MonoRec mono_shfl_down(const MonoRec& a, int o) {
    MonoRec r;
    r.ft = __shfl_down(a.ft, o); r.fp = __shfl_down(a.fp, o); r.lt = __shfl_down(a.lt, o); r.lp = __shfl_down(a.lp, o);
    r.sum = __shfl_down(a.sum, o);
    return r;
}

__device__ __forceinline__ void finalize2_body(const FinalizeParams& p) {
    __shared__ uint32_t s_acc[255 * 12 + 256];
    __shared__ unsigned long long s_ref[256];
    __shared__ uint32_t s_head[2];
    __shared__ uint32_t s_col[64];
    const int t = threadIdx.x, lane = t & 63, w = t >> 6;
    for (int i = t; i < p.ncnt; i += 256) s_acc[i] = 0;
    __syncthreads();
    for (int idx = t; idx < kCntCopies * p.ncnt; idx += 256) {
        const uint32_t v = p.blk_cnt[idx];
        if (v) atomicAdd(&s_acc[idx % p.ncnt], v);
    }
    __syncthreads();
    for (int i = t; i < p.ncnt; i += 256) {
        const uint32_t v = s_acc[i];
        p.cnt[i] = v;
        if (p.cnt_host) p.cnt_host[i] = v;
    }
    for (int c0 = 0; c0 < p.ncols; c0 += 4) {
        const int c = c0 + w;
        uint32_t v = (c < p.ncols && (uint32_t)lane < p.nchunk) ? p.chunk_tot[(size_t)c * kMaxChunks + lane] : 0u;
        {
            uint32_t inc = v;
#pragma unroll
            for (int o = 1; o < 64; o <<= 1) {
                const uint32_t u = __shfl_up(inc, o);
                if (lane >= o) inc += u;
            }
            if (c < p.ncols) p.chunk_base[(size_t)c * kMaxChunks + lane] = inc - v;
        }
#pragma unroll
        for (int o = 32; o > 0; o >>= 1) v += __shfl_xor(v, o);
        if (lane == 0 && c < p.ncols) {
            s_col[c] = v;
            if (c == kColAnom) p.p1->n_anom = v;
            else if (c == kColNormal) p.p1->n_normal = v;
            else p.p1->key_tot[c - kColKey0] = v;
        }
    }
    for (int b0 = 0; b0 < p.nbams; b0 += 4) {
        const int b = b0 + w;
        MonoRec acc;
        acc.ft = -1; acc.fp = 0; acc.lt = 0; acc.lp = 0; acc.sum = 0;
        if (b < p.nbams && (uint32_t)lane < p.nfold) acc = p.fold_part[(size_t)b * p.nfold + lane];
#pragma unroll
        for (int o = 1; o < 64; o <<= 1) {
            const MonoRec other = mono_shfl_down(acc, o);
            if (lane + o < 64 && ((lane & (2 * o - 1)) == 0)) acc = mono_combine(acc, other);
        }
        if (lane == 0 && b < p.nbams) {
            const unsigned long long r = acc.ft == -1 ? 0ull : (unsigned long long)acc.sum;
            s_ref[b] = r;
            p.p1->ref_len[b] = r;
        }
    }
    __syncthreads();
    if (t == 0) {
        uint32_t covered = 0;
        for (int b = 0; b < p.nbams; ++b)
            if ((unsigned long long)covered < s_ref[b]) covered = (uint32_t)s_ref[b];
        p.p1->covered_ref_len = covered;
        int W = p.w0;
        for (int i = 0; i < p.nlibs; ++i) {
            const int nd = (int)(s_acc[i * kNumFlags + F_LARGE] + s_acc[i * kNumFlags + F_SMALL]);
            const int tmp = nd > 0 ? (int)__fdiv_rn((float)covered, (float)nd) : 50;
            W = min(W, tmp);
        }
        p.p1->window = W;
        s_head[0] = covered; s_head[1] = (uint32_t)W;
        if (p.key_density) {
            const uint32_t* lib_cnt = s_acc + p.nlibs * kNumFlags;
            const uint32_t* bam_cnt = lib_cnt + p.nlibs;
            for (int k = 0; k < p.nkeys; ++k) p.key_density[k] = 0.000001f;
            for (int i = 0; i < p.nlibs; ++i) {
                const int key = p.libs[i].key;
                float dens = 0.000001f;
                if (p.cn_lib) {
                    if (lib_cnt[i] != 0) dens = __fdiv_rn((float)lib_cnt[i], (float)covered);
                } else {
                    dens = __fdiv_rn((float)bam_cnt[key], (float)covered);
                }
                p.key_density[key] = dens;
            }
        }
    }
    if (p.p1_host) {
        __syncthreads();
        uint32_t* dst = (uint32_t*)p.p1_host;
        static_assert(offsetof(Pass1, covered_ref_len) == 0 && offsetof(Pass1, window) == 4 && offsetof(Pass1, n_anom) == 8 &&
                          offsetof(Pass1, n_normal) == 12 && offsetof(Pass1, key_tot) == 16 && offsetof(Pass1, ref_len) % 8 == 0, "Pass1 mirror");
        static_assert(kColAnom == 0 && kColNormal == 1 && kColKey0 == 2, "the record's words 2.. are the column totals in column order");
        constexpr int kRefWord = (int)(offsetof(Pass1, ref_len) / 4);
        const int words = kRefWord + 2 * p.nbams;
        for (int i = t; i < words; i += 256) {
            uint32_t v;
            if (i < 2) v = s_head[i];
            else if (i < kRefWord) v = i - 2 < p.ncols ? s_col[i - 2] : 0u;
            else v = (uint32_t)(s_ref[(i - kRefWord) >> 1] >> (32 * ((i - kRefWord) & 1)));
            dst[i] = v;
        }
        if (p.flag_host) {
            __threadfence_system();
            __syncthreads();
            if (t == 0) *(volatile uint32_t*)p.flag_host = p.flag_value;
        }
    }
    if (p.na_cap) {
        __syncthreads();
        if (t == 0 && s_col[kColAnom] > p.na_cap) p.p1->n_anom = 0;
    }
}

}
```

breakdancer_amd/csrc/bdx_k3.h:

```cpp
#pragma once
#include "../../include/bdx.h"
#include "bdx_dev.h"

namespace bdx {

struct U4;

struct StageCounts {
    uint32_t n_cand;
    uint32_t n_regions;
    int32_t last_maxq;
    uint32_t n_pairs;
    uint32_t n_groups;
    uint32_t n_entries;
    uint32_t overflow;
    uint32_t n_printed;
    uint32_t n_sv_dev;
    uint32_t n_terms_dev;
    uint32_t n_cn_dev;
    uint32_t n_groups_dev;
    uint32_t stage_sv;
    uint32_t stage_lib;
    uint32_t stage_cn;
    uint32_t n_owners;
    uint32_t n_owners_big;
    uint32_t n_groups_big;
    uint32_t n_old;
    uint32_t n_ins;
    uint32_t sort_done;
    uint32_t irregular;
};

struct RegionRec {
    int32_t tid, start, end;
    uint32_t n, rev, nonctx, nnormal;
    int32_t maxq;
    uint32_t first;
};

struct GroupRec {
    uint64_t key;
    uint32_t pairs;
    uint32_t sum_isize;
};

struct K3Arrays {
    uint32_t cap;
    int32_t* cand;
    uint32_t *pre_q, *pre_rev, *pre_nonctx;
    uint32_t* c_first;
    int32_t* c_maxq;
    int32_t* c_rid;
    int32_t* region_of;
    RegionRec* r_rec;
    uint32_t* r_pk;
    RegionRec* r_rec_dev;
    uint32_t* r_pk_dev;
    int host_copy_later;
    uint32_t* out_deg;
    unsigned long long* lb_state;
    uint32_t lb_stamp;
    StageCounts* counts;
    StageCounts* counts_host;
};

struct K3Tail {
    int has_next;
    int32_t qlen;
    uint32_t nn;
    const uint32_t* tid_tail;
};

void launch_k3(const K3Arrays& a, const Compact& cp, const Pass1* p1, uint32_t n_anom_host, int min_len, int seq_coverage_lim,
               int nkeys, uint32_t nn_base, K3Tail tail, bool region_of_launch, hipStream_t s);

constexpr int kMaxBuckets = 8192;
constexpr int kJoinLdsSlots = 8192;
constexpr uint32_t kDirectJoinMax = 1u << 22;
inline uint32_t direct_join_slots(uint32_t n) {
    uint32_t slots = 1024;
    while (slots < 4 * (uint64_t)n) slots <<= 1;
    return slots;
}
constexpr int kAggSlots = 4096;

struct K4Arrays {
    uint32_t nbuckets;
    uint32_t log2b;
    uint32_t* bcnt;
    uint32_t* boff;
    uint32_t* bcur;
    uint64_t* e_key;
    uint32_t* e_idx;
    int32_t* partner;
    int32_t* pair_lo;
    uint64_t* t_key;
    int32_t* t_idx;
    uint32_t direct;
    uint32_t t_mask;
    GroupRec* g_rec;
    uint32_t g_cap;
};

__host__ __device__ __forceinline__ uint64_t group_pack(uint32_t rlo, uint32_t rhi, uint32_t lib, uint32_t flag) {
    return ((uint64_t)rlo << 38) | ((uint64_t)rhi << 12) | ((uint64_t)lib << 4) | (uint64_t)flag;
}
constexpr uint32_t kMaxRegions = (1u << 26) - 2;
constexpr uint32_t kMaxAnomalous = 0x7FFFFF00u;

struct Entries {
    const uint64_t* key;
    const uint64_t* check;
    const int32_t* region;
    const uint32_t* order;
    const uint32_t* meta;
    const int32_t* isize;
    int32_t region_base;
    const int32_t* cand;
    const int32_t* c_rid;
    int32_t* region_out;
    const RegionRec* r_rec_dev;
    const uint32_t* r_pk_dev;
    RegionRec* r_rec_host;
    uint32_t* r_pk_host;
    const StageCounts* counts;
    int nkeys2;
    uint32_t* k6_scratch;
    uint32_t scratch_cap;
    const uint32_t* n_local;
    const uint64_t* fkey;
    const uint64_t* fcheck;
    const int32_t* fregion;
    int want_pair_lo;
};

void launch_k4(const K4Arrays& k4, const Entries& e, const uint32_t* n_ptr, uint32_t n_upper, StageCounts* counts, hipStream_t s);

constexpr int kMaxRanks = 64;
struct ExchangeEntry {
    uint64_t key;
    uint32_t order;
    int32_t region;
    uint32_t meta;
    int32_t isize;
    uint64_t check;
};
static_assert(sizeof(ExchangeEntry) == 32, "exchange entries travel as four 64-bit words");
__host__ __device__ __forceinline__ uint32_t exchange_owner(uint64_t k, uint32_t world) {
    k = (k ^ (k >> 33)) * 0xff51afd7ed558ccdull;
    k ^= k >> 29;
    return (uint32_t)(k % world);
}
struct GatherPackage { uint64_t regions_off, pk_off, groups_off; uint32_t nr, ng; };
struct GatherDesc { GatherPackage p[kMaxRanks]; int world; };
void launch_k8_place_regions(const char* all, const GatherDesc& D, uint32_t max_nr, const uint64_t* rbase, int ntids, int nkeys2, RegionRec* r_rec,
                             uint32_t* r_pk, uint32_t* err, hipStream_t s);

void launch_k4_join_only(const K4Arrays& k4, const Entries& e, const uint32_t* n_ptr, uint32_t n_upper, StageCounts* counts, hipStream_t s);

void launch_k5(const double* lambda, const int32_t* k, double* out, uint32_t n, hipStream_t s);

constexpr int kK6MaxMembers = 4;
constexpr int kK6MaxIn = 3;
constexpr int kK6BigMembers = 64;
constexpr int kK6LibStride = 16;
constexpr int kK6LabelRoundsBig = 8;
constexpr uint32_t kK6RankSlices = 16;
constexpr uint32_t kK6RankSortMax = 1u << 17;
constexpr int kK6LabelRounds = 2;
constexpr int kK6LabelRoundsGather = 3;

struct RegSum {
    uint32_t np_all;
    uint32_t np_emit;
    uint32_t np_self;
    uint32_t w_self;
    uint32_t n_in;
    uint32_t n_pairs;
    uint32_t n_weak;
    uint32_t big;
    uint32_t e_lo[kK6MaxIn];
    uint32_t e_w[kK6MaxIn];
    uint32_t e_off[kK6MaxIn];
    uint32_t e_cnt[kK6MaxIn];
};
constexpr uint64_t kWeakPart = 1ull << 63;

struct PartRec {
    uint64_t key;
    uint32_t pairs;
    uint32_t sum;
};

struct MemberInfo {
    uint32_t r;
    RegionRec rec;
    uint32_t np_all, np_self, w_self, n_in;
    uint32_t e_lo[kK6MaxIn], e_w[kK6MaxIn], e_off[kK6MaxIn], e_cnt[kK6MaxIn];
    uint32_t stored;
    uint32_t pad;
};
constexpr int kMemberWords = sizeof(MemberInfo) / 4;

struct SvOut {
    bdx_sv sv;
    uint32_t grp_mask;
    uint32_t start;
};

struct SvWire {
    int32_t pos[2], region[2];
    int32_t size, score, num_reads;
    float allele_frequency;
    double logp;
    uint32_t start;
    uint32_t bits;
};
static_assert(sizeof(SvWire) == 48, "twelve 32-bit words");
constexpr int kWireWords = sizeof(SvWire) / 4;

struct LibStage { int32_t lib, rc; double lambda; };
struct CnStage { int32_t key; float value; };

struct K6Arrays {
    uint32_t cap;
    const RegionRec* r_rec;
    const uint32_t* r_pk;
    const int32_t* region_of;
    const int32_t* partner;
    const int32_t* pair_lo;
    const uint32_t* meta;
    const int32_t* isize;
    const GroupRec* in_groups;
    const uint32_t* in_goff;
    const uint32_t* first_of;
    PartRec* parts;
    RegSum* rs;
    uint32_t* out_deg;
    uint32_t* label;
    uint32_t* bad_v;
    uint32_t* bad;
    uint32_t* mcount;
    uint32_t* pcount;
    MemberInfo* members;
    uint32_t* owners;
    uint32_t* own_nsv;
    uint32_t* own_nacc;
    uint32_t* own_ncn;
    uint32_t* own_first;
    uint32_t* slot_next;
    uint32_t* emit_part;
    uint32_t* owners_big;
    uint32_t* member_ids;
    SvOut* sv_stage;
    LibStage* lib_stage;
    CnStage* cn_stage;
    uint32_t lib_stride;
    uint32_t* sv_src;
    uint2* sv_begin;
    uint32_t* sv_vx;
    int32_t* d_lib_index;
    int32_t* d_cn_key;
    float* d_cn_value;
    double* t_lambda;
    int32_t* t_k;
    SvOut* sv_out;
    int32_t* lib_index;
    int32_t* lib_pairs;
    int32_t* cn_key;
    float* cn_value;
    uint32_t sv_cap, term_cap, cn_cap;
    double* ltail;
    uint32_t* printed_host;
    double* ltail_host;
    const SvOut* hs_rec;
    const uint64_t* hs_key;
    const uint32_t* hs_cnt;
    uint64_t* old_key;
    uint32_t* old_slot;
    uint64_t* sorted_key;
    uint32_t* sorted_slot;
    uint32_t* rank_part;
    uint64_t* hs_key_dev;
    uint32_t* ins_T;
    uint32_t* ins_src;
    uint32_t* ins_pre_l;
    uint32_t* ins_pre_c;
    const int32_t* hs_lib_index;
    const int32_t* hs_lib_pairs;
    const double* hs_lambda;
    const int32_t* hs_cn_key;
    const float* hs_cn_value;
    uint32_t nh;
    GroupRec* g_rec;
    uint32_t g_cap;
    unsigned long long* lb_state;
    uint32_t lb_stamp;
    StageCounts* counts;
    StageCounts* counts_host;
    StageCounts* counts_host2;
    uint32_t* flag_regions;
    uint32_t* flag_groups;
    uint32_t* flag_done;
    uint32_t flag_value;
    const uint32_t* hist;
    const float* key_density;
    const float* lib_mean;
    const Pass1* p1;
    int nlibs, nkeys, min_read_pair, chr_restricted, period, force_host;
    int mirror_in_walk;
    int big_walk;
    uint32_t fin_regions;
    int asm_plain;
    int ins_plain;
    int propagation_rounds;
    uint8_t* taint;
    int wire_rows;
    unsigned long long* sv_key;
};

void launch_k6_groups(const K6Arrays& a, uint32_t n_anom_host, hipStream_t s);
void launch_k6_pairs(const K6Arrays& a, uint32_t n_upper, hipStream_t s);
void launch_k6_components(const K6Arrays& a, uint32_t n_upper, hipStream_t s);
void launch_k6_scratch_init(uint32_t* out_deg, uint32_t cap, hipStream_t s);
void launch_k6_walk(const K6Arrays& a, uint32_t n_anom_host, hipStream_t s);
void launch_k6_table(const K6Arrays& a, uint32_t n_anom_host, double ln10, int score_threshold, int with_scores, hipStream_t s);
uint32_t k6_score_grid(const K6Arrays& a);

}
```

breakdancer_amd/csrc/k1_classify.hip:

```cpp
#include <cstddef>

#include <hip/hip_ext.h>

#include "bdx_dev.h"
#include "bdx_finalize.h"

#include <limits.h>

#ifdef BDX_KPROF
#include "bdx_scan.h"
#else
#define KPROF(row, col) do {} while (0)
#endif

namespace bdx {

constexpr int kMixedLibs = 8;

typedef int v4i __attribute__((ext_vector_type(4)));
typedef unsigned short v4us __attribute__((ext_vector_type(4)));
typedef unsigned char v4uc __attribute__((ext_vector_type(4)));
__device__ __forceinline__ int4 ldnt(const int32_t* p) { const v4i v = __builtin_nontemporal_load((const v4i*)p); return make_int4(v.x, v.y, v.z, v.w); }
__device__ __forceinline__ ushort4 ldnt(const uint16_t* p) { const v4us v = __builtin_nontemporal_load((const v4us*)p); return make_ushort4(v.x, v.y, v.z, v.w); }
__device__ __forceinline__ uchar4 ldnt(const uint8_t* p) { const v4uc v = __builtin_nontemporal_load((const v4uc*)p); return make_uchar4(v.x, v.y, v.z, v.w); }
// ... 425 lines not shown
                        if (lane_r == 0) atomicAdd(&s_libcnt[v], (unsigned)popc64(m));
                        todo &= ~m;
                    }
                    todo = ballot64(p1c[r]);
                    while (todo) {
                        const int ld = __ffsll((long long)todo) - 1;
                        const unsigned v = __shfl(bam[r], ld);
                        const uint64_t m = ballot64(p1c[r] && bam[r] == v);
                        if (lane_r == 0) atomicAdd(&s_bamcnt[v], (unsigned)popc64(m));
                        todo &= ~m;
                    }
                }
            }
            if (!uni) {
                for (int k = 0; k < nkeys_r; ++k) {
                    unsigned ck = 0;
#pragma unroll
                    for (int r = 0; r < 4; ++r) ck += popc64(ballot64(pk[r] && key[r] == k));
                    if (lane_r == kColKey0 + k) colval = ck;
                }
            }
            if (lane_r < ncols_r) p.tile_tot[(size_t)lane_r * p.tstride + tile] = colval;
            if (p.stash && na && one_key) {
                unsigned ra = 0;
#pragma unroll
                for (int r = 0; r < 4; ++r) ra = __builtin_amdgcn_mbcnt_hi((uint32_t)(ba[r] >> 32), __builtin_amdgcn_mbcnt_lo((uint32_t)ba[r], ra));
                uint32_t* idx = (uint32_t*)s_stash[w];
#pragma unroll
                for (int r = 0; r < 4; ++r) {
                    if (anom[r] && ra < (unsigned)kStashCap) idx[ra] = (uint32_t)(lane_r * 4 + r);
                    ra += anom[r] ? 1u : 0u;
                }
                __builtin_amdgcn_wave_barrier();
                const unsigned nrec = na < (unsigned)kStashCap ? na : (unsigned)kStashCap;
                const uint32_t where = idx[(unsigned)lane_r < nrec ? lane_r : 0];
                const unsigned l = where >> 2, rr = where & 3u;
                const uint64_t below = (1ull << l) - 1ull;
                unsigned rn = 0, rk = 0;
#pragma unroll
                for (int r = 0; r < 4; ++r) {
                    const uint64_t mn = ballot64(nleft[r]), mp = ballot64(pk[r]);
                    rn += popc64(mn & below) + ((unsigned)r < rr ? (unsigned)((mn >> l) & 1ull) : 0u);
                    rk += popc64(mp & below) + ((unsigned)r <= rr ? (unsigned)((mp >> l) & 1ull) : 0u);
                }
                if ((unsigned)lane_r < nrec) {
                    const uint64_t i = (uint64_t)tile * kTile + where;
                    const unsigned cb = (idx[kStashCap + l] >> (8 * rr)) & 0xffu;
                    unsigned L = nlibs_r > 1 ? (unsigned)p.r.lib[i] : 0u;
                    if (L >= (unsigned)nlibs_r) L = 0;
                    typedef unsigned v4u __attribute__((ext_vector_type(4)));
                    const v4u x0 = {(uint32_t)p.r.tid[i], (uint32_t)p.r.pos[i], (uint32_t)abs(p.r.isize[i]), (cb & 15u) | ((((unsigned)p.r.flag[i] >> 4) & 1u) << 4) | (L << 8)};
                    const v4u x1 = {where | (rn << 8) | ((uint32_t)k_first << 20), rk, 0u, 0u};
                    v4u* dst = (v4u*)(p.stash + (size_t)tile * kStashCap + lane_r);
                    dst[0] = x0;
                    dst[1] = x1;
                }
                __builtin_amdgcn_wave_barrier();
            } else if (p.stash && (unsigned)lane_r < (na < (unsigned)kStashCap ? na : (unsigned)kStashCap)) {
                p.stash[(size_t)tile * kStashCap + lane_r].where = 0xFFFFFFFFu;
            }
        }
        }

        {
            const int tw = __builtin_amdgcn_readfirstlane(tid[0]);
            bool same = true;
#pragma unroll
            for (int r = 0; r < 4; ++r) same = same && (r >= nvalid || tid[r] == tw);
            const bool one_tid = __all(same);
            if (one_tid && one_file && __all(nvalid == 4)) {
                const int first = __builtin_amdgcn_readfirstlane(pos[0]), last = __builtin_amdgcn_readlane(pos[3], 63);
                if (lane == 0) {
                    MonoRec m;
                    m.ft = tw; m.fp = first; m.lt = tw; m.lp = last; m.sum = (long long)last - (long long)first;
                    p.tile_mono[(size_t)file0 * p.tstride + tile] = m;
                }
            } else {
            int lane_m = lane, nbams_m = nbams;
            asm volatile("" : "+v"(lane_m), "+s"(nbams_m));
            unsigned bam[4];
#pragma unroll
            for (int r = 0; r < 4; ++r) {
                const unsigned v = (bamp >> (8 * r)) & 0xffu;
                bam[r] = v < (unsigned)nbams_m ? v : 0u;
            }
            if (one_tid && nbams_m <= 64) {
                int my_first = 0, my_last = 0;
                bool present = false;
                unsigned pending = (1u << nvalid) - 1u;
                while (true) {
                    const uint64_t any = ballot64(pending != 0);
                    if (!any) break;
                    const int ld = __ffsll((long long)any) - 1;
                    const int lowp = pending ? __ffs(pending) - 1 : 0;
                    const unsigned v = __shfl(bam[lowp], ld);
                    unsigned mine = 0;
#pragma unroll
                    for (int r = 0; r < 4; ++r)
                        if (((pending >> r) & 1u) && bam[r] == v) mine |= 1u << r;
                    pending &= ~mine;
                    const uint64_t M = ballot64(mine != 0);
                    const int fl = __ffsll((long long)M) - 1, ll = 63 - __clzll((long long)M);
                    const int fs = mine ? __ffs(mine) - 1 : 0, ls = mine ? 31 - __clz(mine) : 0;
                    const int first = __shfl(pos[fs], fl), last = __shfl(pos[ls], ll);
                    if (lane_m == (int)v) { present = true; my_first = first; my_last = last; }
                }
                if (present) {
                    MonoRec m;
                    m.ft = tw; m.fp = my_first; m.lt = tw; m.lp = my_last; m.sum = (long long)my_last - (long long)my_first;
                    p.tile_mono[(size_t)lane_m * p.tstride + tile] = m;
                }
            } else {
                if (lane_m == 0)
                    for (int b = 0; b < nbams_m; ++b) my_mono[b].ft = -1;
                for (int L = 0; L < 64; ++L) {
#pragma unroll
                    for (int r = 0; r < 4; ++r) {
                        const int nv = __shfl(nvalid, L);
                        if (r >= nv) continue;
                        const int rt = __shfl(tid[r], L), rp = __shfl(pos[r], L);
                        const unsigned rb = __shfl(bam[r], L);
                        if (lane_m == 0) {
                            MonoRec m = my_mono[rb];
                            if (m.ft == -1) { m.ft = rt; m.fp = rp; m.sum = 0; }
                            else if (m.lt == rt) m.sum += (long long)rp - (long long)m.lp;
                            m.lt = rt; m.lp = rp;
                            my_mono[rb] = m;
                        }
                    }
                }
                if (lane_m == 0)
                    for (int b = 0; b < nbams_m; ++b)
                        if (my_mono[b].ft != -1) p.tile_mono[(size_t)b * p.tstride + tile] = my_mono[b];
            }
            }
        }
    }
    __syncthreads();
    uint32_t* out = p.blk_cnt + (size_t)(blockIdx.x & (kCntCopies - 1)) * ncnt;
    for (int i = t; i < ncnt; i += kBlock) {
        const uint32_t v = s_cnt[i];
        if (v) atomicAdd(&out[i], v);
    }
}

void launch_k1(const K1Params& p, int grid, size_t lds, hipStream_t s, hipEvent_t start, hipEvent_t stop) {
    auto kernel = p.opt_l ? k1_classify_kernel<true> : k1_classify_kernel<false>;
    if (start && stop) hipExtLaunchKernelGGL(kernel, dim3(grid), dim3(kBlock), (uint32_t)lds, s, start, stop, 0u, p);
    else hipLaunchKernelGGL(kernel, dim3(grid), dim3(kBlock), lds, s, p);
}

constexpr int kFinBlock = 1024;

__global__ __launch_bounds__(kFinBlock) void finalize_kernel(const FinalizeParams p) {
    __shared__ uint32_t s_carry;
    __shared__ MonoRec s_mono[kFinBlock / 64];
    const int t = threadIdx.x, lane = t & 63, w = t >> 6;
    KPROF(blockIdx.x * 16 + w, 0);

    const uint32_t nscan = (uint32_t)p.ncols * p.nchunk;
    if (blockIdx.x < nscan) {
        const int c = (int)(blockIdx.x / p.nchunk);
        const uint32_t g = blockIdx.x % p.nchunk;
        const uint32_t tile_lo = g * p.chunk_super * kK2TilesPerWave;
        const uint32_t tile_hi = min(p.ntiles, (g + 1) * p.chunk_super * kK2TilesPerWave);
        const uint32_t* in = p.tile_tot + (size_t)c * p.tstride;
        uint32_t* out = p.tile_pre + (size_t)c * p.tstride;
        if (t == 0) s_carry = 0;
        __syncthreads();
        constexpr int kQ = 4;
        static_assert(kK2TilesPerWave == 4 && kFinBlock == 1024, "one 16-byte load per super tile");
        __shared__ uint32_t s_wt[kQ * (kFinBlock / 64)];
        __shared__ uint32_t s_round;
        const uint32_t row_hi = min(p.tstride, (g + 1) * p.chunk_super * kK2TilesPerWave);
        for (uint32_t base = tile_lo; base < tile_hi; base += kFinBlock * kQ * 4) {
            uint32_t sum[kQ], inc[kQ];
#pragma unroll
            for (int q = 0; q < kQ; ++q) {
                const uint32_t i = base + ((uint32_t)q * kFinBlock + t) * 4;
                uint4 x = make_uint4(0, 0, 0, 0);
                if (i < row_hi) x = *(const uint4*)(in + i);
                sum[q] = x.x + x.y + x.z + x.w;
            }
            if (sum[0] != 0xFFFFFFFFu) KPROF(blockIdx.x * 16 + w, 1);
#pragma unroll
            for (int q = 0; q < kQ; ++q) inc[q] = wave_incl_scan(sum[q]);
            if (lane == 63) {
#pragma unroll
                for (int q = 0; q < kQ; ++q) s_wt[q * (kFinBlock / 64) + w] = inc[q];
            }
            __syncthreads();
            if (w == 0) {
                static_assert(kQ * (kFinBlock / 64) == 64, "one wave total per lane");
                const uint32_t v = s_wt[lane];
                const uint32_t li = wave_incl_scan(v);
                s_wt[lane] = li - v;
                if (lane == 63) s_round = li;
            }
            __syncthreads();
#pragma unroll
            for (int q = 0; q < kQ; ++q) {
                const uint32_t i = base + ((uint32_t)q * kFinBlock + t) * 4;
                if (i < row_hi) out[i / 4] = s_carry + s_wt[q * (kFinBlock / 64) + w] + inc[q] - sum[q];
            }
            __syncthreads();
            if (t == 0) s_carry += s_round;
            __syncthreads();
        }
        if (t == 0) p.chunk_tot[(size_t)c * kMaxChunks + g] = s_carry;
        KPROF(blockIdx.x * 16 + w, 2);
        return;
    }

    const uint32_t fb = blockIdx.x - nscan;
    const uint32_t chunk = (p.ntiles + p.nfold - 1) / p.nfold;
    const uint32_t c0 = fb * chunk, c1 = min(c0 + chunk, p.ntiles);
    const uint32_t per = (chunk + kFinBlock - 1) / kFinBlock;
    for (int b = 0; b < p.nbams; ++b) {
        const MonoRec* mo = p.tile_mono + (size_t)b * p.tstride;
        MonoRec acc;
        acc.ft = -1; acc.fp = 0; acc.lt = 0; acc.lp = 0; acc.sum = 0;
        const uint32_t t0 = min(c0 + (uint32_t)t * per, c1), t1 = min(t0 + per, c1);
        for (uint32_t i = t0; i < t1; i += 8) {
            MonoRec e[8];
#pragma unroll
            for (int q = 0; q < 8; ++q) {
                if (i + q < t1) e[q] = mo[i + q];
                else e[q].ft = -1;
            }
#pragma unroll
            for (int q = 0; q < 8; ++q) acc = mono_combine(acc, e[q]);
        }
        if (acc.ft != -12345) KPROF(blockIdx.x * 16 + w, 1);
#pragma unroll
        for (int o = 1; o < 64; o <<= 1) {
            const MonoRec other = mono_shfl_down(acc, o);
            if (lane + o < 64 && ((lane & (2 * o - 1)) == 0)) acc = mono_combine(acc, other);
        }
        if (lane == 0) s_mono[w] = acc;
        __syncthreads();
        if (t == 0) {
            MonoRec tot = s_mono[0];
            for (int k = 1; k < kFinBlock / 64; ++k) tot = mono_combine(tot, s_mono[k]);
            p.fold_part[(size_t)b * p.nfold + fb] = tot;
        }
        __syncthreads();
    }
    KPROF(blockIdx.x * 16 + w, 2);
}

__global__ __launch_bounds__(256) void finalize2_kernel(const FinalizeParams p) { finalize2_body(p); }

__global__ __launch_bounds__(256) void k0_init_kernel(const InitList l) {
    for (int f = 0; f < l.n; ++f)
        for (uint32_t i = blockIdx.x * 256 + threadIdx.x; i < l.words[f]; i += gridDim.x * 256) l.ptr[f][i] = l.value[f];
}

void launch_init(const InitList& l, hipStream_t s) {
    uint32_t mx = 0;
    for (int f = 0; f < l.n; ++f) mx = l.words[f] > mx ? l.words[f] : mx;
    if (!mx) return;
    const uint32_t g = (mx + 1023) / 1024;
    hipLaunchKernelGGL(k0_init_kernel, dim3(g < 1024u ? g : 1024u), dim3(256), 0, s, l);
}

void launch_finalize(const FinalizeParams& p, hipStream_t s, bool second_level) {
    hipLaunchKernelGGL(finalize_kernel, dim3(p.ncols * p.nchunk + p.nfold), dim3(kFinBlock), 0, s, p);
    if (second_level) hipLaunchKernelGGL(finalize2_kernel, dim3(1), dim3(256), 0, s, p);
}

void launch_finalize2_only(const FinalizeParams& p, hipStream_t s) { hipLaunchKernelGGL(finalize2_kernel, dim3(1), dim3(256), 0, s, p); }

}

__global__ void k1_noop_kernel() {}
namespace bdx { void warm_k1(hipStream_t s) { hipLaunchKernelGGL(k1_noop_kernel, dim3(1), dim3(64), 0, s); } }

#ifdef BDX_KPROF
extern "C" int bdx_debug_kprof1(unsigned long long* out, size_t n) {
    const int rc = (int)hipMemcpyFromSymbol(out, HIP_SYMBOL(bdx::g_kprof), n * sizeof(unsigned long long));
    void* p = nullptr;
    if (hipGetSymbolAddress(&p, HIP_SYMBOL(bdx::g_kprof)) == hipSuccess) (void)hipMemset(p, 0, sizeof(unsigned long long) * 8 * 65536);
    return rc;
}
#endif
```

breakdancer_amd/csrc/k2_compact.hip:

```cpp
#include <cstdlib>

#include "bdx_dev.h"
#include "bdx_finalize.h"

namespace bdx {

size_t k2_lds_bytes(int) { return 0; }

constexpr int kSub = kK2TilesPerWave;
constexpr int kPerLane = 4 * kSub;
constexpr int kTile2 = kTile * kSub;
constexpr int kSlice = 256;
constexpr int kOffBits = 10;
static_assert(kPerLane <= 32 && kTile2 <= (1 << kOffBits), "K2 super tile");

__device__ __forceinline__ unsigned class_byte(const uint64_t (&cq)[kSub / 2], int r) {
    uint64_t v = cq[0];
#pragma unroll
    for (int q = 1; q < kSub / 2; ++q) v = (r >> 3) == q ? cq[q] : v;
    return (unsigned)((v >> (8 * (r & 7))) & 255u);
}

__device__ __forceinline__ void key_and_qlen_of(const K2Params& p, uint64_t i, uint64_t& key, int& qlen, uint64_t& check) {
    if (p.nseg == 0) {
        key = p.r.key[i];
        qlen = (int)p.r.qlen[i];
        if (p.c.check) check = p.r.check[i];
        return;
    }
    int lo = 0, hi = p.nseg - 1;
    while (lo < hi) {
        const int mid = (lo + hi + 1) >> 1;
        if (p.seg_begin[mid] <= i) lo = mid; else hi = mid - 1;
    }
    key = p.seg_ptr[lo][i];
    qlen = (int)p.seg_qlen[lo][i];
    if (p.c.check) check = p.seg_check[lo][i];
}

__device__ __forceinline__ uint32_t wave_sum_below(uint32_t v, uint32_t chunk, int lane) {
    v = (uint32_t)lane < chunk ? v : 0u;
#pragma unroll
    for (int o = 32; o > 0; o >>= 1) v += __shfl_xor(v, o);
    return v;
}
__device__ __forceinline__ int lib_of(const K2Params& p, uint64_t i) {
    if (p.nlibs <= 1) return 0;
    const int l = p.r.lib[i];
    return l < p.nlibs ? l : 0;
}

template <bool kBases> __device__ __forceinline__ uint32_t chunk_word(const K2Params& p, int col, uint32_t chunk, int lane) {
    return kBases ? p.chunk_base[(size_t)col * kMaxChunks + chunk] : p.chunk_tot[(size_t)col * kMaxChunks + lane];
}
template <bool kBases> __device__ __forceinline__ uint32_t chunk_sum(uint32_t word, uint32_t chunk, int lane) {
    return kBases ? word : wave_sum_below(word, chunk, lane);
}
template <bool kBases> __device__ __forceinline__ uint32_t col_prefix(const K2Params& p, int col, uint32_t tile2, uint32_t chunk, int lane) {
    return p.tile_pre[(size_t)col * p.tstride + tile2] + chunk_sum<kBases>(chunk_word<kBases>(p, col, chunk, lane), chunk, lane);
}

template <bool kBases> __device__ __forceinline__ void k2_body(const K2Params& p, uint32_t nblk) {
    __shared__ uint32_t s_src[kWaves * kSlice];
    __shared__ uint32_t s_nn[kWaves * kSlice];
    const int nkeys = p.nkeys;
    const int lane = threadIdx.x & 63, w = threadIdx.x >> 6;
    const uint32_t nwaves = nblk * kWaves;
    const uint32_t ntiles2 = (p.ntiles + kSub - 1) / kSub;
    for (uint32_t tile2 = blockIdx.x * kWaves + w; tile2 < ntiles2; tile2 += nwaves) {
        const uint64_t base = (uint64_t)tile2 * kTile2 + (uint64_t)lane * kPerLane;
        const uint32_t chunk = tile2 / p.chunk_super;
        const uint32_t l_norm = p.tile_pre[(size_t)kColNormal * p.tstride + tile2], c_norm = chunk_word<kBases>(p, kColNormal, chunk, lane);
        const uint32_t l_anom = p.tile_pre[(size_t)kColAnom * p.tstride + tile2], c_anom = chunk_word<kBases>(p, kColAnom, chunk, lane);
        const uint32_t l_k0 = p.tile_pre[(size_t)kColKey0 * p.tstride + tile2], c_k0 = chunk_word<kBases>(p, kColKey0, chunk, lane);
        const uint32_t l_k1 = nkeys > 1 ? p.tile_pre[(size_t)(kColKey0 + 1) * p.tstride + tile2] : 0u;
        const uint32_t c_k1 = nkeys > 1 ? chunk_word<kBases>(p, kColKey0 + 1, chunk, lane) : 0u;
        if (p.stash) {
            static_assert(kSub == 4 && kStashKeys == 2, "lane layout of the totals");
            const int t = lane & 3, col = lane >> 2;
            uint32_t v = 0;
            if (col < 2 + nkeys && tile2 * kSub + t < p.ntiles) v = p.tile_tot[(size_t)col * p.tstride + tile2 * kSub + t];
            const uint32_t a0 = __shfl(v, 0), a1 = __shfl(v, 1), a2 = __shfl(v, 2), a3 = __shfl(v, 3);
            const uint32_t A = a0 + a1 + a2 + a3;
            if (A == 0) continue;
            if (max(max(a0, a1), max(a2, a3)) <= (uint32_t)kStashCap) {
                const uint32_t pre_norm = l_norm + chunk_sum<kBases>(c_norm, chunk, lane), rank0 = l_anom + chunk_sum<kBases>(c_anom, chunk, lane);
                const uint32_t pre_k0 = l_k0 + chunk_sum<kBases>(c_k0, chunk, lane), pre_k1 = l_k1 + chunk_sum<kBases>(c_k1, chunk, lane);
                const uint32_t q = (uint32_t)lane;
                const uint32_t tq = (q >= a0 ? 1u : 0u) + (q >= a0 + a1 ? 1u : 0u) + (q >= a0 + a1 + a2 ? 1u : 0u);
                const uint32_t before = tq == 0 ? 0u : (tq == 1 ? a0 : (tq == 2 ? a0 + a1 : a0 + a1 + a2));
                uint32_t e[3];
#pragma unroll
                for (int c = 1; c <= 3; ++c) {
                    const uint32_t x0 = __shfl(v, c * 4), x1 = __shfl(v, c * 4 + 1), x2 = __shfl(v, c * 4 + 2);
                    e[c - 1] = tq == 0 ? 0u : (tq == 1 ? x0 : (tq == 2 ? x0 + x1 : x0 + x1 + x2));
                }
                const uint32_t j = rank0 + q;
                const uint32_t tile = tile2 * kSub + min(tq, 3u);
                uint4 r0 = make_uint4(0u, 0u, 0u, 0u);
                uint2 r1 = make_uint2(0u, 0u);
                if (q < A) {
                    const StashRec* src = p.stash + (size_t)tile * kStashCap + (q - before);
                    r0 = *(const uint4*)src;
                    r1 = *(const uint2*)&src->where;
                }
                if (!__any(r1.x == 0xFFFFFFFFu)) {
                    if (q < A && j < p.c.cap) {
                        const uint64_t i = (uint64_t)tile * kTile + (r1.x & 255u);
                        const uint32_t k0 = (r1.x >> 20) & 63u;
                        uint64_t key, check = 0;
                        int qlen;
                        key_and_qlen_of(p, i, key, qlen, check);
                        p.c.tid[j] = (int32_t)r0.x;
                        p.c.pos[j] = (int32_t)r0.y;
                        p.c.isize[j] = (int32_t)r0.z;
                        p.c.meta[j] = r0.w | ((uint32_t)qlen << 16);
                        p.c.key[j] = key;
                        if (p.c.check) p.c.check[j] = check;
                        p.c.idx[j] = (uint32_t)i;
                        p.c.nn[j] = p.nn_base + pre_norm + e[0] + ((r1.x >> 8) & 511u);
                        p.c.pk[j] = p.pk_base[0] + pre_k0 + e[1] + (k0 == 0 ? r1.y : 0u);
                        if (nkeys > 1) p.c.pk[(size_t)p.c.cap + j] = p.pk_base[1] + pre_k1 + e[2] + (k0 == 1 ? r1.y : 0u);
                    }
                    continue;
                }
            }
        }
        uint64_t cq[kSub / 2];
#pragma unroll
        for (int q = 0; q < kSub / 2; ++q) cq[q] = 0;
        int nvalid = 0;
        if (base + kPerLane <= p.n) {
            nvalid = kPerLane;
#pragma unroll
            for (int q = 0; q < kSub / 4; ++q) {
                const uint4 x = *(const uint4*)(p.cls + base + 16 * q);
                cq[2 * q] = (uint64_t)x.x | ((uint64_t)x.y << 32);
                cq[2 * q + 1] = (uint64_t)x.z | ((uint64_t)x.w << 32);
            }
        } else {
#pragma unroll
            for (int r = 0; r < kPerLane; ++r)
                if (base + r < p.n) { ++nvalid; cq[r >> 3] |= (uint64_t)p.cls[base + r] << (8 * (r & 7)); }
        }
        uint32_t m_anom = 0, m_nleft = 0, m_pk = 0;
#pragma unroll
        for (int r = 0; r < kPerLane; ++r) {
            const unsigned c = (unsigned)((cq[r >> 3] >> (8 * (r & 7))) & 255u);
            const unsigned f = c & 15u;
            const bool pass = r < nvalid && (c & 0x10u);
            const bool normal = f == F_NORMAL_FR || f == F_NORMAL_RF;
            m_anom |= (pass && !normal) ? 1u << r : 0u;
            m_nleft |= (pass && (c & 0x40u)) ? 1u << r : 0u;
            m_pk |= (pass && (c & 0x20u)) ? 1u << r : 0u;
        }
        if (!__any(m_anom != 0)) continue;
        const uint32_t pre_norm = l_norm + chunk_sum<kBases>(c_norm, chunk, lane), rank0 = l_anom + chunk_sum<kBases>(c_anom, chunk, lane);
        const uint32_t pre_k0 = l_k0 + chunk_sum<kBases>(c_k0, chunk, lane), pre_k1 = l_k1 + chunk_sum<kBases>(c_k1, chunk, lane);

        const uint32_t tot = (uint32_t)__popc(m_anom) + ((uint32_t)__popc(m_nleft) << 16);
        const uint32_t ex0 = wave_incl_scan(tot) - tot;
        const uint32_t nn0 = p.nn_base + pre_norm + (ex0 >> 16);
        const uint32_t local0 = ex0 & 0xFFFFu;
        const uint32_t cnt = __shfl((ex0 + tot) & 0xFFFFu, 63);
        for (uint32_t win = 0; win < cnt; win += kSlice) {
            {
                uint32_t local = local0;
                for (uint32_t mm = m_anom; mm; mm &= mm - 1, ++local) {
                    if (local < win || local >= win + kSlice) continue;
                    const int r = __builtin_ctz(mm);
                    s_src[w * kSlice + (local - win)] = (uint32_t)(lane * kPerLane + r) | (class_byte(cq, r) << kOffBits);
                    s_nn[w * kSlice + (local - win)] = nn0 + (uint32_t)__popc(m_nleft & ((1u << r) - 1u));
                }
            }
            __builtin_amdgcn_wave_barrier();
            const uint32_t wcnt = min((uint32_t)kSlice, cnt - win);
            for (uint32_t b = 0; b < wcnt; b += 64) {
                const uint32_t q = b + lane;
                if (q < wcnt && rank0 + win + q < p.c.cap) {
                    const uint32_t src = s_src[w * kSlice + q];
                    const uint64_t i = (uint64_t)tile2 * kTile2 + (src & ((1u << kOffBits) - 1u));
                    const uint32_t j = rank0 + win + q;
                    const unsigned sam = p.r.flag[i];
                    p.c.tid[j] = p.r.tid[i];
                    p.c.pos[j] = p.r.pos[i];
                    p.c.isize[j] = abs(p.r.isize[i]);
                    uint64_t key, check = 0;
                    int qlen;
                    key_and_qlen_of(p, i, key, qlen, check);
                    p.c.meta[j] = meta_pack((int)((src >> kOffBits) & 15u), (sam >> 4) & 1u, lib_of(p, i), qlen);
                    p.c.key[j] = key;
                    if (p.c.check) p.c.check[j] = check;
                    p.c.idx[j] = (uint32_t)i;
                    p.c.nn[j] = s_nn[w * kSlice + q];
                }
            }
            __builtin_amdgcn_wave_barrier();
        }
        uint64_t kq[kSub / 2];
#pragma unroll
        for (int q = 0; q < kSub / 2; ++q) kq[q] = 0;
        if (nkeys > 1) {
#pragma unroll
            for (int r = 0; r < kPerLane; ++r)
                if (r < nvalid) kq[r >> 3] |= (uint64_t)(p.libs[lib_of(p, base + r)].key & 255) << (8 * (r & 7));
        }
        for (int k0 = 0; k0 < nkeys; k0 += 2) {
            uint32_t mk0 = 0, mk1 = 0;
            if (nkeys > 1) {
#pragma unroll
                for (int r = 0; r < kPerLane; ++r) {
                    const int key = (int)((kq[r >> 3] >> (8 * (r & 7))) & 255u);
                    if ((m_pk >> r) & 1u) { mk0 |= key == k0 ? 1u << r : 0u; mk1 |= key == k0 + 1 ? 1u << r : 0u; }
                }
            } else {
                mk0 = m_pk;
            }
            const uint32_t v = (uint32_t)__popc(mk0) + ((uint32_t)__popc(mk1) << 16);
            const uint32_t ex = wave_incl_scan(v) - v;
            const uint32_t b0 = p.pk_base[k0] + (k0 == 0 ? pre_k0 : col_prefix<kBases>(p, kColKey0 + k0, tile2, chunk, lane));
            const uint32_t b1 = k0 + 1 < nkeys ? p.pk_base[k0 + 1] + (k0 == 0 ? pre_k1 : col_prefix<kBases>(p, kColKey0 + k0 + 1, tile2, chunk, lane)) : 0u;
            uint32_t j = rank0 + local0;
            for (uint32_t mm = m_anom; mm; mm &= mm - 1, ++j) {
                if (j >= p.c.cap) break;
                const int r = __builtin_ctz(mm);
                const uint32_t upto = (2u << r) - 1u;
                p.c.pk[(size_t)k0 * p.c.cap + j] = b0 + (ex & 0xFFFFu) + (uint32_t)__popc(mk0 & upto);
                if (k0 + 1 < nkeys) p.c.pk[(size_t)(k0 + 1) * p.c.cap + j] = b1 + (ex >> 16) + (uint32_t)__popc(mk1 & upto);
            }
        }
    }
}

__device__ __forceinline__ void k2_fills(const K2Params& p) {
#pragma unroll
    for (int f = 0; f < 4; ++f)
        for (uint32_t i = blockIdx.x * kBlock + threadIdx.x; i < p.fill_words[f]; i += gridDim.x * kBlock) p.fill_ptr[f][i] = p.fill_value[f];
}

__global__ __launch_bounds__(kBlock) void k2_compact_kernel(const K2Params p) {
    k2_fills(p);
    k2_body<true>(p, gridDim.x);
}

__global__ __launch_bounds__(kBlock) void k2_compact_side_kernel(const K2Params p, const FinalizeParams fp) {
    k2_fills(p);
    if (blockIdx.x == gridDim.x - 1) {
        finalize2_body(fp);
        return;
    }
    k2_body<false>(p, gridDim.x - 1);
}

void launch_k2(const K2Params& p, size_t lds, hipStream_t s, const FinalizeParams* side) {
    const uint32_t ntiles2 = (p.ntiles + kSub - 1) / kSub;
    const uint32_t nblk = (ntiles2 + kWaves - 1) / kWaves;
    const uint32_t cap = 8192u;
    const uint32_t grid = nblk < cap ? nblk : cap;
    if (side) hipLaunchKernelGGL(k2_compact_side_kernel, dim3(grid + 1), dim3(kBlock), lds, s, p, *side);
    else hipLaunchKernelGGL(k2_compact_kernel, dim3(grid), dim3(kBlock), lds, s, p);
}

}

__global__ void k2_noop_kernel() {}
namespace bdx { void warm_k2(hipStream_t s) { hipLaunchKernelGGL(k2_noop_kernel, dim3(1), dim3(64), 0, s); } }
```

breakdancer_amd/csrc/k6_assemble.hip:

```cpp
#include <algorithm>
#include <cstdint>

#include "bdx_k3.h"

#include "bdx_poisson.h"
#include "bdx_scan.h"

namespace bdx {

namespace {

__device__ __forceinline__ uint64_t readlane64(uint64_t v, int l) {
    const uint32_t lo = (uint32_t)__builtin_amdgcn_readlane((int)(uint32_t)v, l);
    const uint32_t hi = (uint32_t)__builtin_amdgcn_readlane((int)(uint32_t)(v >> 32), l);
    return ((uint64_t)hi << 32) | lo;
}

__device__ __forceinline__ uint32_t wave_sum_u32(uint32_t v) {
#pragma unroll
    for (int o = 32; o > 0; o >>= 1) v += __shfl_xor(v, o);
    return v;
}

__device__ __forceinline__ uint32_t wave_reserve(uint32_t need, uint32_t* counter) {
// ... 883 lines not shown
                if (pl > 0 && wq[pl] != wq[pl - 1]) firstp = pl;
                win4 |= (uint32_t)firstp << (2 * pl);
            }
#pragma unroll
            for (int i = 0; i < kK6MaxMembers; ++i)
                if (i < k) {
                    if (np_all[i]) touch ^= (uint32_t)P[first[i]].key ^ (uint32_t)P[first[i] + np_all[i] - 1].key;
                    touch ^= a.r_pk[(size_t)mr[i] * 2 * nk] ^ a.r_pk[(size_t)mr[i] * 2 * nk + 2 * nk - 1];
                }
        }
        KPROF(blockIdx.x, 4);
        int ncalls = 0;
        {
            uint32_t self_done = 0, edge_done = 0, self_alive = self_has, edge_alive = edge_has;
            for (int f = 0; f < k;) {
                int fe = f + 1;
                while (fe < k && (int)((win4 >> (2 * fe)) & 3u) == f) ++fe;
                uint32_t visited = 0;
                for (int sv = 0; sv < fe; ++sv) {
                    if (visited & (1u << sv)) continue;
                    int nt = 1;
                    uint32_t tails = (uint32_t)sv;
                    while (nt) {
                        int nn = 0;
                        uint32_t newtails = 0;
                        for (int ti = 0; ti < nt; ++ti) {
                            const int tail = (int)((tails >> (2 * ti)) & 3u);
                            if (visited & (1u << tail)) continue;
                            for (int nb = 0; nb < fe; ++nb) {
                                int A, B;
                                if (nb == tail) {
                                    if (tail < f) continue;
                                    if (!((self_ok & ~self_done) & (1u << tail))) continue;
                                    self_done |= 1u << tail;
                                    A = tail; B = -1;
                                } else {
                                    const int x = min(nb, tail), y = max(nb, tail), pi = pair_index(x, y);
                                    if (y < f) continue;
                                    if (!((edge_ok & ~edge_done) & (1u << pi))) continue;
                                    edge_done |= 1u << pi;
                                    A = x; B = y;
                                }
                                if (nn < 12) { newtails |= (uint32_t)nb << (2 * nn); ++nn; }
                                const bool stA = (stored >> A) & 1u, stB = (stored >> (B >= 0 ? B : A)) & 1u;
                                uint32_t g = 0;
                                if ((self_alive & (1u << A)) && stA) { g |= 1u; self_alive &= ~(1u << A); }
                                if (B >= 0) {
                                    const int pi = pair_index(A, B);
                                    if ((edge_alive & (1u << pi)) && stA && stB) { g |= 2u; edge_alive &= ~(1u << pi); }
                                    if ((self_alive & (1u << B)) && stB) { g |= 4u; self_alive &= ~(1u << B); }
                                }
                                if (g != 0 || mrp <= 0) T.call(ncalls++) = (uint32_t)A | ((uint32_t)(B + 1) << 2) | (g << 5) | ((uint32_t)sv << 8) | ((uint32_t)f << 10);
                            }
                            visited |= 1u << tail;
                        }
                        nt = nn;
                        tails = newtails;
                    }
                }
                f = fe;
            }
        }
        if (nk < 0) a.counts->overflow = touch;
        KPROF(blockIdx.x, 5);
        {
            const GrpRange none{0, 0};
            int cur_f = -1, cur_sv = -1, max_readlen = 0;
            uint32_t W = 0, start = 0, nseq = 0, nsv = 0, nacc_tot = 0, ncn_tot = 0, prev_slot = 0;
            bool from_old = false;
            for (int c = 0; c < ncalls; ++c) {
                const uint32_t d = T.call(c);
                const int A = (int)(d & 3u), B = (int)((d >> 2) & 7u) - 1, sv = (int)((d >> 8) & 3u), f = (int)((d >> 10) & 3u);
                const uint32_t g = (d >> 5) & 7u;
                if (f != cur_f) {
                    W = T.rid(f) / period;
                    const uint32_t rl = (W + 1) * period - 1;
                    max_readlen = f == 0 ? mrl0 : (rl < NR ? a.r_rec[rl].maxq : mq_last);
                    nseq = 0;
                }
                if (f != cur_f || sv != cur_sv) {
                    if (cur_f >= 0 && !from_old && nsv) { a.own_nsv[start] = nsv; a.own_nacc[start] = nacc_tot; a.own_ncn[start] = ncn_tot; }
                    cur_f = f; cur_sv = sv;
                    start = T.rid(sv);
                    from_old = sv < f;
                    nsv = 0; nacc_tot = 0; ncn_tot = 0; prev_slot = 0;
                }
                const uint32_t slot = B >= 0 ? T.Eslot(pair_index(A, B)) : T.Sslot(A);
                const int Bi = B >= 0 ? B : A;
                GrpRange gs[3] = {none, none, none};
                if (g & 1u) gs[0] = GrpRange{T.Sbeg(A), T.Scnt(A)};
                if (g & 2u) gs[1] = GrpRange{T.Ebeg(pair_index(A, Bi)), T.Ecnt(pair_index(A, Bi))};
                if (g & 4u) gs[2] = GrpRange{T.Sbeg(Bi), T.Scnt(Bi)};
                RegionRec recA{}, recB{};
                recA.tid = (int32_t)T.Rtid(A); recA.start = (int32_t)T.Rstart(A); recA.end = (int32_t)T.Rend(A); recA.n = T.Rn(A); recA.rev = T.Rrev(A);
                recB.tid = (int32_t)T.Rtid(Bi); recB.start = (int32_t)T.Rstart(Bi); recB.end = (int32_t)T.Rend(Bi); recB.n = T.Rn(Bi); recB.rev = T.Rrev(Bi);
                const uint32_t rA = T.rid(A), rB = T.rid(Bi);
                const uint32_t* pkA = a.r_pk + (size_t)rA * 2 * nk + nk;
                const uint32_t* pkB = a.r_pk + (size_t)rB * 2 * nk;
                uint32_t nacc = 0, ncn = 0;
                if (assemble_sv(a, rc_, P, rA, B >= 0 ? (int32_t)rB : -1, recA, recB, pkA, pkB, gs, max_readlen, slot, start, true, &nacc, &ncn,
                                c == 0 ? 16384u + blockIdx.x : ~0u)) {
                    if (from_old) {
                        const uint32_t q = atomicAdd(&a.counts->n_old, 1u);
                        a.old_key[q] = ((uint64_t)(W * period) << kKeyShiftT) | ((uint64_t)start << kKeyShiftStart) | (uint64_t)(nseq & kKeySeqMask);
                        a.old_slot[q] = slot;
                        ++nseq;
                    } else {
                        if (nsv == 0) a.own_first[start] = slot; else a.slot_next[prev_slot] = slot;
                    }
                    prev_slot = slot;
                    ++nsv;
                    nacc_tot += nacc;
                    ncn_tot += ncn;
                }
                if (c == 0) KPROF(blockIdx.x, 6);
            }
            if (cur_f >= 0 && !from_old && nsv) { a.own_nsv[start] = nsv; a.own_nacc[start] = nacc_tot; a.own_ncn[start] = ncn_tot; }
        }
    }
    KPROF(blockIdx.x, 7);
}

__global__ __launch_bounds__(256) void k6_walk_big_kernel(K6Arrays a) {
    __shared__ BigTab s_big[4];
    const int lane = threadIdx.x & 63, w = threadIdx.x >> 6;
    const uint32_t NR = a.counts->n_regions, n = a.counts->n_owners_big;
    for (uint32_t oi = blockIdx.x * 4 + w; oi < n; oi += gridDim.x * 4) {
        walk_big(a, s_big[w], a.owners_big[oi], lane, NR);
        __builtin_amdgcn_wave_barrier();
    }
}

namespace {
__device__ __forceinline__ uint32_t count_below(const uint32_t* v, uint32_t n, uint32_t x) {
    uint32_t lo = 0, hi = n;
    while (lo < hi) {
        const uint32_t mid = (lo + hi) / 2;
        if (v[mid] < x) lo = mid + 1; else hi = mid;
    }
    return lo;
}
__device__ __forceinline__ uint32_t count_below64(const uint64_t* v, uint32_t n, uint64_t x) {
    uint32_t lo = 0, hi = n;
    while (lo < hi) {
        const uint32_t mid = (lo + hi) / 2;
        if (v[mid] < x) lo = mid + 1; else hi = mid;
    }
    return lo;
}
}

constexpr uint32_t kInsLds = 2048;
constexpr uint32_t kInsThreads = 1024;
constexpr uint32_t kInsBucketMax = 8192;
constexpr uint32_t kInsCntLds = 10240;
constexpr uint32_t kInsBuckets = 2048;
constexpr uint32_t kInsBucketDepth = 128;
constexpr uint32_t kInsPerBucketPath = kInsBucketMax / kInsThreads;
constexpr uint32_t kRankGrid = 256;
__device__ __forceinline__ void rank_layout(uint32_t nd, uint32_t* nchunk, uint32_t* nslice, uint32_t* per) {
    *nchunk = (nd + kScanBlock - 1) / kScanBlock;
    *nslice = min(kK6RankSlices, max(1u, kRankGrid / *nchunk));
    *per = (nd + *nslice - 1) / *nslice;
}

struct InsertJob {
    K6Arrays a;
    __device__ void operator()() const;
};

__device__ void InsertJob::operator()() const {
    constexpr uint32_t kThreads = kInsThreads;
    constexpr uint32_t kPer = kInsCntLds / kThreads;
    __shared__ uint64_t s_ord[kInsBucketMax];
    __shared__ uint32_t s_cnt[kInsCntLds];
    __shared__ uint64_t s_hk[kInsLds];
    __shared__ uint32_t s_hist[kInsBuckets + 1];
    __shared__ uint32_t s_ws[2][kThreads / 64];
    __shared__ uint32_t s_crowded;
    uint64_t* const s_dk = s_ord;
    uint32_t* const s_dv = (uint32_t*)(s_ord + kInsLds);
    uint64_t* const s_tmp = s_ord + 2 * kInsLds;
    static_assert(2 * kInsLds + kThreads <= kInsBucketMax, "keys, slots and the rank-counting copy of the smaller paths fit s_ord");
    const uint32_t tid = threadIdx.x;
    const int lane = tid & 63, w = tid >> 6;
    const uint32_t nh = a.nh;
    const uint32_t nd = a.counts->n_old;
    uint64_t* hk = nh <= kInsLds ? s_hk : a.hs_key_dev;
    for (uint32_t i = tid; i < nh; i += kThreads) hk[i] = a.hs_key[i];
    uint32_t hc[kInsLds / kThreads];
#pragma unroll
    for (uint32_t q = 0; q < kInsLds / kThreads; ++q) hc[q] = (nh <= kInsLds && tid + q * kThreads < nh) ? a.hs_cnt[tid + q * kThreads] : 0u;
    const uint32_t n = nh + nd;
    if (n > a.sv_cap) {
        if (tid == 0) { a.counts->overflow = 1; a.counts->n_ins = 0; a.ins_pre_l[0] = 0; a.ins_pre_c[0] = 0; }
        return;
    }
    if (tid == 0) a.counts->n_ins = n;
    if (n == 0) {
        if (tid == 0) { a.ins_pre_l[0] = 0; a.ins_pre_c[0] = 0; }
        return;
    }
    const bool by_rank = nd <= kThreads;
    bool by_bucket = !by_rank && nd <= kInsBucketMax && a.ins_plain != 1;
    const bool small = n <= kInsCntLds;
    uint64_t* dk = nullptr;
    uint32_t* dv = nullptr;
    uint32_t my_cnt = 0;
    if (by_bucket) {
        const uint32_t period = (uint32_t)max(a.period, 1);
        const uint32_t nwin = a.counts->n_regions / period + 2;
        constexpr uint32_t kSub = 64;
        const uint64_t span = (uint64_t)nwin * kSub + 1;
        auto bucket_of = [&](uint64_t key) {
            const uint32_t T = (uint32_t)(key >> kKeyShiftT), own = (uint32_t)(key >> 33) & 1u, start = (uint32_t)(key >> kKeyShiftStart) & 0x3FFFFFFu;
            const uint32_t W = T / period, r = T - W * period;
            uint32_t sub = kSub;
            if (!r && !own) {
                if (start >= T) sub = kSub - 1;
                else if (start + period >= T) sub = kSub / 2 + min(kSub / 2 - 1, (uint32_t)(((uint64_t)(start + period - T) * (kSub / 2)) / period));
                else sub = (uint32_t)(((uint64_t)start * (kSub / 2)) / T);
            }
            return (uint32_t)min((uint64_t)(kInsBuckets - 1), (((uint64_t)W * kSub + sub) * kInsBuckets) / span);
        };
        for (uint32_t i = tid; i <= kInsBuckets; i += kThreads) s_hist[i] = 0;
        if (tid == 0) s_crowded = a.ins_plain == 2 ? 1u : 0u;
        __syncthreads();
        uint64_t key[kInsPerBucketPath];
        uint32_t slot[kInsPerBucketPath], bk[kInsPerBucketPath], at[kInsPerBucketPath], cnt[kInsPerBucketPath];
#pragma unroll
        for (uint32_t k = 0; k < kInsPerBucketPath; ++k) {
            const uint32_t d = tid + k * kThreads;
            key[k] = d < nd ? a.old_key[d] : ~0ull;
            slot[k] = d < nd ? a.old_slot[d] : 0u;
        }
#pragma unroll
        for (uint32_t k = 0; k < kInsPerBucketPath; ++k) {
            const uint32_t d = tid + k * kThreads;
            bk[k] = 0; at[k] = 0; cnt[k] = 0;
            if (d < nd) {
                cnt[k] = (uint32_t)a.sv_stage[slot[k]].sv.lib_count | ((uint32_t)a.sv_stage[slot[k]].sv.cn_count << 16);
                bk[k] = bucket_of(key[k]);
                at[k] = atomicAdd(&s_hist[bk[k]], 1u);
                if (at[k] >= kInsBucketDepth) s_crowded = 1u;
            }
        }
        __syncthreads();
        by_bucket = s_crowded == 0;
        if (by_bucket) {
            static_assert(kInsBuckets == 2 * kThreads, "two buckets per thread");
            const uint32_t h0 = s_hist[2 * tid], h1 = s_hist[2 * tid + 1];
            const uint32_t inc = wave_incl_scan_t(h0 + h1);
            if (lane == 63) s_ws[0][w] = inc;
            __syncthreads();
            uint32_t off = inc - (h0 + h1);
            for (int q = 0; q < w; ++q) off += s_ws[0][q];
            s_hist[2 * tid] = off; s_hist[2 * tid + 1] = off + h0;
            if (tid == 0) s_hist[kInsBuckets] = nd;
            __syncthreads();
#pragma unroll
            for (uint32_t k = 0; k < kInsPerBucketPath; ++k)
                if (tid + k * kThreads < nd) s_ord[s_hist[bk[k]] + at[k]] = key[k];
            __syncthreads();
            auto below = [&](uint64_t x, uint32_t b) {
                const uint32_t lo = s_hist[b], hi = s_hist[b + 1];
                uint32_t r = lo;
                for (uint32_t j = lo; j < hi; ++j) r += s_ord[j] < x ? 1u : 0u;
                return r;
            };
#pragma unroll
            for (uint32_t k = 0; k < kInsPerBucketPath; ++k)
                if (tid + k * kThreads < nd) {
                    const uint32_t pos = below(key[k], bk[k]) + count_below64(hk, nh, key[k]);
                    a.ins_T[pos] = (uint32_t)(key[k] >> kKeyShiftT);
                    a.ins_src[pos] = slot[k];
                    if (small) s_cnt[pos] = cnt[k];
                    else { a.ins_pre_l[pos] = cnt[k] & 0xffffu; a.ins_pre_c[pos] = cnt[k] >> 16; }
                }
            static_assert(kInsLds / kThreads == 2, "two prefetched host counts per thread");
            for (uint32_t j = tid; j < nh; j += kThreads) {
                const uint64_t x = hk[j];
                const uint32_t pos = j + below(x, bucket_of(x)), c = nh <= kInsLds ? (j < kThreads ? hc[0] : hc[1]) : a.hs_cnt[j];
                a.ins_T[pos] = (uint32_t)(x >> kKeyShiftT);
                a.ins_src[pos] = 0x80000000u | j;
                if (small) s_cnt[pos] = c;
                else { a.ins_pre_l[pos] = c & 0xffffu; a.ins_pre_c[pos] = c >> 16; }
            }
        }
        __syncthreads();
    }
    if (by_bucket) {
    } else if (by_rank) {
        dk = s_dk; dv = s_dv;
        const uint64_t key = tid < nd ? a.old_key[tid] : ~0ull;
        const uint32_t slot = tid < nd ? a.old_slot[tid] : 0u;
        if (tid < nd) my_cnt = (uint32_t)a.sv_stage[slot].sv.lib_count | ((uint32_t)a.sv_stage[slot].sv.cn_count << 16);
        s_tmp[tid] = key;
        __syncthreads();
        uint32_t rank = 0;
        for (uint32_t q = 0; q < nd; ++q) rank += s_tmp[q] < key ? 1u : 0u;
        if (tid < nd) { dk[rank] = key; dv[rank] = slot; }
        __syncthreads();
        if (tid < nd) {
            const uint32_t pos = rank + count_below64(hk, nh, key);
            a.ins_T[pos] = (uint32_t)(key >> kKeyShiftT);
            a.ins_src[pos] = slot;
            if (small) s_cnt[pos] = my_cnt;
// ... 183 lines not shown
            if (g == 3) { hb1 = count_below(Tt, nh, j + 1); break; }
        }
    }
    const uint32_t ex_sv = inc.x - e.x, ex_l = inc.y - e.y, ex_c = inc.z - e.z;
    if (valid && j == n - 1) {
        const uint32_t tsv = inc.x + nh, tl = inc.y + h_l, tc = inc.z + h_c;
        a.counts->n_sv_dev = tsv; a.counts->n_terms_dev = tl; a.counts->n_cn_dev = tc;
        if (a.counts_host2) { a.counts_host2->n_sv_dev = tsv; a.counts_host2->n_terms_dev = tl; a.counts_host2->n_cn_dev = tc; a.counts_host2->n_old = a.counts->n_old; }
        if (tsv > a.sv_cap || tl > a.term_cap || tc > a.cn_cap) {
            a.counts->overflow = 1;
            if (a.counts_host2) a.counts_host2->overflow = 1;
        }
    }
    const bool wg_ok = !(carry.x + tot.x + nh > a.sv_cap || carry.y + tot.y + h_l > a.term_cap || carry.z + tot.z + h_c > a.cn_cap);
    if (!wg_ok) return;
    s_ex[0][tid] = ex_sv; s_ex[1][tid] = ex_l; s_ex[2][tid] = ex_c;
    if (tid == 0) { s_lohi[0] = nh ? count_below(Tt, nh, base) : 0u; s_lohi[1] = nh ? count_below(Tt, nh, min(n, base + kScanBlock)) : 0u; }
    __syncthreads();
    for (uint32_t jj = s_lohi[0] + tid; jj < s_lohi[1]; jj += kScanBlock) {
        const uint32_t v = Tt[jj], vt = v - base;
        const uint32_t pos = s_ex[0][vt] + jj;
        a.sv_src[pos] = a.ins_src[jj];
        a.sv_begin[pos] = make_uint2(s_ex[1][vt] + a.ins_pre_l[jj], s_ex[2][vt] + a.ins_pre_c[jj]);
        if (a.sv_vx) a.sv_vx[pos] = v;
    }
    if (!valid || !e.x) return;
    uint32_t lb = ex_l + a.ins_pre_l[hb1], cb = ex_c + a.ins_pre_c[hb1], slot = slot0;
    for (uint32_t q = 0; q < e.x; ++q) {
        const uint32_t pos = ex_sv + hb1 + q;
        a.sv_src[pos] = slot;
        a.sv_begin[pos] = make_uint2(lb, cb);
        if (a.sv_vx) a.sv_vx[pos] = j;
        if (q + 1 < e.x) {
            lb += (uint32_t)a.sv_stage[slot].sv.lib_count;
            cb += (uint32_t)a.sv_stage[slot].sv.cn_count;
            slot = a.slot_next[slot];
        }
    }
}

__global__ __launch_bounds__(kScanBlock) void k6_score_kernel(K6Arrays a, double ln10, int score_threshold, int with_scores) {
    __shared__ uint32_t s_rec[kScanBlock / 64][64 * kSvWords];
    __shared__ uint32_t s_fromw[kScanBlock / 64][64];
    __shared__ uint32_t s_printed;
    const uint32_t tid = threadIdx.x;
    const int lane = tid & 63, w = tid >> 6;
    const uint32_t bid = blockIdx.x;
    const uint32_t kp = 32768u + 16384u + (bid * 4 + w < 16384u ? bid * 4 + w : 16383u);
    (void)kp;
    KPROF(kp, 0);
    if (tid == 0) s_printed = 0;
    __syncthreads();
    const uint32_t n_sv = a.counts->overflow ? 0u : a.counts->n_sv_dev;
    for (uint32_t c0 = (bid * (kScanBlock / 64) + (uint32_t)w) * 64u; c0 < n_sv; c0 += gridDim.x * kScanBlock) {
        const uint32_t cnt = min(64u, n_sv - c0);
        const bool act = (uint32_t)lane < cnt;
        uint32_t* rec = s_rec[w];
        const uint32_t from = act ? a.sv_src[c0 + lane] : 0u;
        const uint2 bg = act ? a.sv_begin[c0 + lane] : make_uint2(0u, 0u);
        s_fromw[w][lane] = from;
        __builtin_amdgcn_wave_barrier();
        for (uint32_t i = lane; i < cnt * kSvWords; i += 64) {
            const uint32_t sv = i / kSvWords, wd = i - sv * kSvWords;
            const uint32_t f = s_fromw[w][sv];
            const uint32_t* src = (f & 0x80000000u) ? (const uint32_t*)(a.hs_rec + (f & 0x7FFFFFFFu)) : (const uint32_t*)(a.sv_stage + f);
            rec[i] = src[wd];
        }
        __builtin_amdgcn_wave_barrier();
        KPROF(kp, 3);
        SvOut* o = (SvOut*)rec + (act ? lane : 0);
        const bool hosted = (from & 0x80000000u) != 0;
        const int32_t nl = act ? o->sv.lib_count : 0, ncn = act ? o->sv.cn_count : 0;
        const int32_t l0 = o->sv.lib_begin, k0 = o->sv.cn_begin;
        if (act) { o->sv.lib_begin = (int32_t)bg.x; o->sv.cn_begin = (int32_t)bg.y; }
        int32_t max_nl = nl, max_ncn = ncn;
#pragma unroll
        for (int off = 32; off > 0; off >>= 1) { max_nl = max(max_nl, __shfl_xor(max_nl, off)); max_ncn = max(max_ncn, __shfl_xor(max_ncn, off)); }
        double logp = 0.0, err = 0.0;
        for (int32_t q = 0; q < max_nl; ++q) {
            const bool a2 = q < nl;
            double lam = 1.0;
            int32_t k = 0, li = 0;
            if (a2) {
                if (hosted) { lam = a.hs_lambda[l0 + q]; k = a.hs_lib_pairs[l0 + q]; li = a.hs_lib_index[l0 + q]; }
                else { const LibStage t = a.lib_stage[(size_t)from * a.lib_stride + q]; lam = t.lambda; k = t.rc; li = t.lib; }
            }
            const double lt = poisson_term(lam, k, a2, lane);
            if (a2) {
                a.lib_index[bg.x + q] = li;
                a.lib_pairs[bg.x + q] = k;
                if (a.ltail_host) a.ltail_host[bg.x + q] = lt;
                const double tmp_a = __dsub_rn(lt, err);
                const double tmp_b = __dadd_rn(logp, tmp_a);
                err = __dsub_rn(__dsub_rn(tmp_b, logp), tmp_a);
                logp = tmp_b;
            }
        }
        for (int32_t t = 0; t < max_ncn; ++t) {
            if (t < ncn) {
                int32_t key;
                float value;
                if (hosted) { key = a.hs_cn_key[k0 + t]; value = a.hs_cn_value[k0 + t]; }
                else { const CnStage cn = a.cn_stage[(size_t)from * a.nkeys + t]; key = cn.key; value = cn.value; }
                a.cn_key[bg.y + t] = key;
                a.cn_value[bg.y + t] = value;
            }
        }
        bool pr = false;
        if (act && with_scores) {
            const double phred_tmp = __ddiv_rn(__dmul_rn(-10.0, logp), ln10);
            const double r = __dadd_rn(phred_tmp, 0.5);
            int phred;
            if (phred_tmp > 99.0) phred = 99;
            else if (r != r || r >= 2147483648.0 || r <= -2147483649.0) phred = INT32_MIN;
            else phred = (int)r;
            pr = phred > score_threshold;
            o->sv.logp = logp;
            o->sv.score = phred;
            o->sv.printed = pr ? 1 : 0;
        }
        if (a.sv_key && act) {
            const unsigned long long T = a.sv_vx[c0 + lane], st = o->start;
            a.sv_key[c0 + lane] = (T << kKeyShiftT) | (T == st ? 1ull << 33 : 0ull) | (st << kKeyShiftStart);
        }
        const uint32_t npr = (uint32_t)__popcll(__ballot(pr));
        if (lane == 0 && npr) atomicAdd(&s_printed, npr);
        KPROF(kp, 4);
        __builtin_amdgcn_wave_barrier();
        if (a.wire_rows) {
            SvWire wr{};
            if (act) {
                wr.pos[0] = o->sv.pos[0]; wr.pos[1] = o->sv.pos[1]; wr.region[0] = o->sv.region[0]; wr.region[1] = o->sv.region[1];
                wr.size = o->sv.size; wr.score = o->sv.score; wr.num_reads = o->sv.num_reads; wr.allele_frequency = o->sv.allele_frequency;
                wr.logp = o->sv.logp; wr.start = o->start;
                wr.bits = ((uint32_t)o->sv.lib_count & 255u) | (((uint32_t)o->sv.cn_count & 255u) << 8) | (((uint32_t)o->sv.flag & 15u) << 16) |
                          ((o->grp_mask & 7u) << 20) | ((o->sv.printed ? 1u : 0u) << 23);
            }
            __builtin_amdgcn_wave_barrier();
            if (act) {
                uint32_t* q = rec + lane * kWireWords;
                const uint32_t* src = (const uint32_t*)&wr;
#pragma unroll
                for (int k = 0; k < kWireWords; ++k) q[k] = src[k];
            }
            __builtin_amdgcn_wave_barrier();
            uint32_t* dst = (uint32_t*)a.sv_out + (size_t)c0 * kWireWords;
            for (uint32_t i = lane; i < cnt * kWireWords; i += 64) dst[i] = rec[i];
        } else {
            uint32_t* dst = (uint32_t*)(a.sv_out + c0);
            for (uint32_t i = lane; i < cnt * kSvWords; i += 64) dst[i] = rec[i];
        }
        __builtin_amdgcn_wave_barrier();
    }
    __syncthreads();
    if (tid == 0) {
        if (s_printed) atomicAdd(&a.counts->n_printed, s_printed);
        if (a.printed_host) a.printed_host[bid] = s_printed;
    }
    KPROF(kp, 5);
}

__global__ __launch_bounds__(64) void k6_done_kernel(K6Arrays a) {
    if (threadIdx.x == 0) {
        if (a.counts_host2) a.counts_host2->n_printed = a.counts->n_printed;
        if (a.flag_done) {
            __threadfence_system();
            *(volatile uint32_t*)a.flag_done = a.flag_value;
        }
    }
}

__global__ __launch_bounds__(256) void k6_scratch_init_kernel(uint32_t* out_deg, uint32_t cap) {
    for (uint32_t j = blockIdx.x * 256 + threadIdx.x; j < cap; j += gridDim.x * 256) {
        out_deg[j] = 0;
        out_deg[(size_t)cap + j] = j;
        out_deg[2 * (size_t)cap + j] = 0;
        out_deg[3 * (size_t)cap + j] = 0;
        out_deg[4 * (size_t)cap + j] = 0;
        out_deg[5 * (size_t)cap + j] = 0;
    }
}

void launch_k6_scratch_init(uint32_t* out_deg, uint32_t cap, hipStream_t s) {
    if (!cap) return;
    hipLaunchKernelGGL(k6_scratch_init_kernel, dim3(std::min<uint32_t>((cap + 255) / 256, 4096u)), dim3(256), 0, s, out_deg, cap);
}

void launch_k6_pairs(const K6Arrays& a, uint32_t n_anom_host, hipStream_t s) {
    if (n_anom_host == 0) return;
    const uint32_t gp = std::min<uint32_t>((n_anom_host / 8 + 3) / 4 + 1, 16384u);
    hipLaunchKernelGGL(k6_pairs_kernel, dim3(gp), dim3(256), 0, s, a);
}

void launch_k6_components(const K6Arrays& a, uint32_t n_anom_host, hipStream_t s) {
    if (n_anom_host == 0) return;
    constexpr uint32_t kRegionThreads = 64;
    const uint32_t grs = (n_anom_host + kRegionThreads - 1) / kRegionThreads;
    if (!a.force_host)
        for (int i = 1; i < a.propagation_rounds; ++i) hipLaunchKernelGGL(k6_label_kernel, dim3(grs), dim3(kRegionThreads), 0, s, a);
    hipLaunchKernelGGL(k6_classify_kernel, dim3(grs), dim3(kRegionThreads), 0, s, a);
    hipLaunchKernelGGL(k6_emit_kernel, dim3(grs), dim3(kRegionThreads), 0, s, a);
    if (a.counts_host && !a.mirror_in_walk) hipLaunchKernelGGL(k6_mirror_kernel, dim3(1), dim3(64), 0, s, a);
}

void launch_k6_groups(const K6Arrays& a, uint32_t n_anom_host, hipStream_t s) {
    launch_k6_pairs(a, n_anom_host, s);
    launch_k6_components(a, n_anom_host, s);
}

void launch_k6_walk(const K6Arrays& a, uint32_t n_anom_host, hipStream_t s) {
    if (n_anom_host == 0 || a.force_host) return;
    const uint32_t gp = std::min<uint32_t>((n_anom_host / 8 + 3) / 4 + 1, 16384u);
    hipLaunchKernelGGL(k6_walk_kernel, dim3(std::min<uint32_t>(n_anom_host / WalkTab::kStride / 4 + 1, 8192u)), dim3(64), 0, s, a);
    if (a.big_walk) hipLaunchKernelGGL(k6_walk_big_kernel, dim3(gp / 8 + 1), dim3(256), 0, s, a);
    if (a.rank_part) hipLaunchKernelGGL(k6_ranksort_kernel, dim3(kRankGrid), dim3(kScanBlock), 0, s, a);
}

uint32_t k6_score_grid(const K6Arrays& a) { return std::max(1u, std::min(1024u, (a.sv_cap + kScanBlock - 1) / kScanBlock)); }

void launch_k6_table(const K6Arrays& a, uint32_t n_anom_host, double ln10, int score_threshold, int with_scores, hipStream_t s) {
    if (n_anom_host) {
        hipLaunchKernelGGL(k6_insert_kernel, dim3(1), dim3(kInsThreads), 0, s, a);
        hipLaunchKernelGGL(k6_place_kernel, dim3(scan_grid(a.fin_regions ? a.fin_regions : a.cap, 1)), dim3(kScanBlock), 0, s, a);
        hipLaunchKernelGGL(k6_score_kernel, dim3(k6_score_grid(a)), dim3(kScanBlock), 0, s, a, ln10, score_threshold, with_scores);
    }
    if (!a.printed_host || a.flag_done) hipLaunchKernelGGL(k6_done_kernel, dim3(1), dim3(64), 0, s, a);
}

}

__global__ void k6_noop_kernel() {}
namespace bdx { void warm_k6(hipStream_t s) { hipLaunchKernelGGL(k6_noop_kernel, dim3(1), dim3(64), 0, s); } }

#ifdef BDX_KPROF
extern "C" int bdx_debug_kprof(unsigned long long* out, size_t n) {
    const int rc = (int)hipMemcpyFromSymbol(out, HIP_SYMBOL(bdx::g_kprof), n * sizeof(unsigned long long));
    void* p = nullptr;
    if (hipGetSymbolAddress(&p, HIP_SYMBOL(bdx::g_kprof)) == hipSuccess) (void)hipMemset(p, 0, sizeof(unsigned long long) * 8 * 65536);
    return rc;
}
#endif
```

Measured before the change: 28.54 billion.

## Fold finalize2 and k6 done into last-block tickets; group k2 tiles; gate ranksort

Drops two separate single-block kernel launches by using an atomic ticket counter, so the last finishing block of finalize_kernel runs the second-level reduction and the last block of k6_score_kernel publishes the done flag. k2 compaction now handles groups of four super-tiles per wave when a stash is present, which reduces block count and repeated prefix loads. The rank-partition sort in k6 only runs when the previous insert list was long, or the anomaly count is large, or specific options are set. These changes remove launch and serialization overhead but add atomic and fence cost and a correctness dependence on the ticket counters wrapping back to zero.

```diff
diff --git a/breakdancer_amd/csrc/bdx_api.hip b/breakdancer_amd/csrc/bdx_api.hip
--- a/breakdancer_amd/csrc/bdx_api.hip
+++ b/breakdancer_amd/csrc/bdx_api.hip
@@ -131,6 +131,7 @@
     DevBuf b_sv_src, b_dlists, b_ltail, b_pair_lo;
     PinBuf h_hs_rec, h_hs_aux, h_hs_lists, h_printed;
     DevBuf b_ins, b_member_ids;
+    DevBuf b_tickets;
     PinBuf h_flags;
     uint32_t seq = 0;
     int dbg_no_stash = 0, dbg_max_chunks = 0, dbg_ins_plain = 0, dbg_gather_walk = 0, dbg_regions_copy = 0, dbg_asm_plain = 0;
@@ -146,6 +147,7 @@
     hipEvent_t ev_groups = nullptr, ev_regions = nullptr;
     int big_walk_mode = -1;
     int64_t last_big_groups = -1;
+    int64_t last_n_old = -1;
     FinalizeParams fp_deferred{};
     bool finalize2_deferred = false;
     bool bucketed_join = false;
@@ -478,7 +480,7 @@
                       &c->b_parts, &c->b_kdens, &c->b_rs, &c->b_slot, &c->b_members, &c->b_own, &c->b_lib_stage,
                       &c->b_cn_stage, &c->b_t_lambda, &c->b_t_k, &c->b_ws6, &c->b_ins, &c->b_member_ids,
                       &c->b_sv_out, &c->b_lib_index_out, &c->b_lib_pairs_out, &c->b_cn_key_out, &c->b_cn_value_out, &c->b_ltail_out, &c->b_sv_key,
-                      &c->b_jq, &c->b_jc};
+                      &c->b_jq, &c->b_jc, &c->b_tickets};
     for (DevBuf* b : bufs) b->release();
     PinBuf* pins[] = {&c->h_p1, &c->h_cnt, &c->h_counts, &c->h_regs, &c->h_pk, &c->h_groups, &c->h_terms, &c->h_flags, &c->h_hs_rec, &c->h_hs_aux, &c->h_hs_lists, &c->h_printed, &c->h_counts0, &c->h_counts2,
                       &c->h_sv_out, &c->h_lib_index, &c->h_lib_pairs, &c->h_cn_key, &c->h_cn_value, &c->h_ltail_dev};
@@ -691,6 +693,14 @@
     return BDX_OK;
 }
 
+
+int ensure_tickets(bdx_ctx* c) {
+    if (c->b_tickets.p) return BDX_OK;
+    HIPCHK(c, c->b_tickets.ensure(64));
+    HIPCHK(c, hipMemsetAsync(c->b_tickets.p, 0, 64, c->stream));
+    return BDX_OK;
+}
+
 int do_pass1(bdx_ctx* c, uint32_t na_cap, bool wait, bool defer_second) {
     HIPCHK(c, hipSetDevice(c->device));
     hipStream_t s = c->stream;
@@ -752,6 +762,11 @@
     ++c->seq;
     fp.flag_host = c->h_flags.as<uint32_t>(); fp.flag_value = c->seq;
     fp.na_cap = na_cap;
+    {
+        const int rc = ensure_tickets(c);
+        if (rc != BDX_OK) return rc;
+    }
+    fp.ticket = c->b_tickets.as<uint32_t>();
     c->fp_deferred = fp;
     c->finalize2_deferred = defer_second;
     launch_finalize(fp, s, !defer_second);
@@ -1142,7 +1157,8 @@
         a.old_slot = (uint32_t*)(a.hs_key_dev + svc); a.ins_T = a.old_slot + p2; a.ins_src = a.ins_T + svc + 1;
         a.ins_pre_l = a.ins_src + svc + 1; a.ins_pre_c = a.ins_pre_l + svc + 1;
         a.sorted_key = (uint64_t*)(((uintptr_t)(a.ins_pre_c + svc + 1) + 7) & ~(uintptr_t)7); a.sorted_slot = (uint32_t*)(a.sorted_key + nsort);
-        a.rank_part = a.sv_cap > 2048u ? a.sorted_slot + nsort : nullptr;
+        const bool long_list = c->dbg_ins_plain == 1 || c->opts.transchr_rearrange || c->last_n_old > (int64_t)(kK6InsBucketMax / 2) || na > (1u << 20);
+        a.rank_part = a.sv_cap > 2048u && long_list ? a.sorted_slot + nsort : nullptr;
     }
     a.sv_begin = c->b_sv_src.as<uint2>(); a.sv_src = (uint32_t*)(a.sv_begin + a.sv_cap); a.ltail = c->b_ltail.as<double>();
     a.d_lib_index = c->b_dlists.as<int32_t>(); a.d_cn_key = a.d_lib_index + a.term_cap; a.d_cn_value = (float*)(a.d_cn_key + a.cn_cap);
@@ -1276,7 +1292,12 @@
     a.fin_regions = (c->counts.n_regions && c->counts.n_regions <= na) ? c->counts.n_regions : na;
     HIPCHK(c, c->h_printed.ensure((size_t)k6_score_grid(a) * 4));
     a.printed_host = c->h_printed.as<uint32_t>();
-    if (c->poll) { a.flag_done = c->h_flags.as<uint32_t>() + 2; a.flag_value = c->seq; }
+    if (c->poll) {
+        a.flag_done = c->h_flags.as<uint32_t>() + 2; a.flag_value = c->seq;
+        const int rc = ensure_tickets(c);
+        if (rc != BDX_OK) return rc;
+        a.done_ticket = c->b_tickets.as<uint32_t>() + 1;
+    }
     a.wire_rows = c->table_in_hbm ? 0 : 1;
     c->rows_packed = a.wire_rows != 0;
     launch_k6_table(a, na, std::log(10), c->opts.score_threshold, c->opts.fisher ? 0 : 1, s);
@@ -1351,6 +1372,7 @@
         c->n_printed = np;
     }
     c->counts.n_old = c2.n_old;
+    c->last_n_old = c2.n_old;
     c->materialized = false;
     if (c->opts.fisher && !c->table_in_hbm) {
         materialize(c);
diff --git a/breakdancer_amd/csrc/bdx_dev.h b/breakdancer_amd/csrc/bdx_dev.h
--- a/breakdancer_amd/csrc/bdx_dev.h
+++ b/breakdancer_amd/csrc/bdx_dev.h
@@ -94,6 +94,7 @@
     uint32_t* flag_host;
     uint32_t flag_value;
     uint32_t na_cap;
+    uint32_t* ticket;
 };
 
 struct InitList {
diff --git a/breakdancer_amd/csrc/bdx_finalize.h b/breakdancer_amd/csrc/bdx_finalize.h
--- a/breakdancer_amd/csrc/bdx_finalize.h
+++ b/breakdancer_amd/csrc/bdx_finalize.h
@@ -20,25 +20,26 @@
     return r;
 }
 
-__device__ __forceinline__ void finalize2_body(const FinalizeParams& p) {
+template <int kThreads> __device__ __forceinline__ void finalize2_body(const FinalizeParams& p) {
+    constexpr int kW = kThreads / 64;
     __shared__ uint32_t s_acc[255 * 12 + 256];
     __shared__ unsigned long long s_ref[256];
     __shared__ uint32_t s_head[2];
     __shared__ uint32_t s_col[64];
     const int t = threadIdx.x, lane = t & 63, w = t >> 6;
-    for (int i = t; i < p.ncnt; i += 256) s_acc[i] = 0;
+    for (int i = t; i < p.ncnt; i += kThreads) s_acc[i] = 0;
     __syncthreads();
-    for (int idx = t; idx < kCntCopies * p.ncnt; idx += 256) {
+    for (int idx = t; idx < kCntCopies * p.ncnt; idx += kThreads) {
         const uint32_t v = p.blk_cnt[idx];
         if (v) atomicAdd(&s_acc[idx % p.ncnt], v);
     }
     __syncthreads();
-    for (int i = t; i < p.ncnt; i += 256) {
+    for (int i = t; i < p.ncnt; i += kThreads) {
         const uint32_t v = s_acc[i];
         p.cnt[i] = v;
         if (p.cnt_host) p.cnt_host[i] = v;
     }
-    for (int c0 = 0; c0 < p.ncols; c0 += 4) {
+    for (int c0 = 0; c0 < p.ncols; c0 += kW) {
         const int c = c0 + w;
         uint32_t v = (c < p.ncols && (uint32_t)lane < p.nchunk) ? p.chunk_tot[(size_t)c * kMaxChunks + lane] : 0u;
         {
@@ -59,7 +60,7 @@
             else p.p1->key_tot[c - kColKey0] = v;
         }
     }
-    for (int b0 = 0; b0 < p.nbams; b0 += 4) {
+    for (int b0 = 0; b0 < p.nbams; b0 += kW) {
         const int b = b0 + w;
         MonoRec acc;
         acc.ft = -1; acc.fp = 0; acc.lt = 0; acc.lp = 0; acc.sum = 0;
@@ -113,7 +114,7 @@
         static_assert(kColAnom == 0 && kColNormal == 1 && kColKey0 == 2, "the record's words 2.. are the column totals in column order");
         constexpr int kRefWord = (int)(offsetof(Pass1, ref_len) / 4);
         const int words = kRefWord + 2 * p.nbams;
-        for (int i = t; i < words; i += 256) {
+        for (int i = t; i < words; i += kThreads) {
             uint32_t v;
             if (i < 2) v = s_head[i];
             else if (i < kRefWord) v = i - 2 < p.ncols ? s_col[i - 2] : 0u;
diff --git a/breakdancer_amd/csrc/bdx_k3.h b/breakdancer_amd/csrc/bdx_k3.h
--- a/breakdancer_amd/csrc/bdx_k3.h
+++ b/breakdancer_amd/csrc/bdx_k3.h
@@ -165,6 +165,7 @@
 constexpr int kK6BigMembers = 64;
 constexpr int kK6LibStride = 16;
 constexpr int kK6LabelRoundsBig = 8;
+constexpr uint32_t kK6InsBucketMax = 8192;
 constexpr uint32_t kK6RankSlices = 16;
 constexpr uint32_t kK6RankSortMax = 1u << 17;
 constexpr int kK6LabelRounds = 2;
@@ -302,6 +303,7 @@
     uint32_t* flag_regions;
     uint32_t* flag_groups;
     uint32_t* flag_done;
+    uint32_t* done_ticket;
     uint32_t flag_value;
     const uint32_t* hist;
     const float* key_density;
diff --git a/breakdancer_amd/csrc/k1_classify.hip b/breakdancer_amd/csrc/k1_classify.hip
--- a/breakdancer_amd/csrc/k1_classify.hip
+++ b/breakdancer_amd/csrc/k1_classify.hip
@@ -601,7 +601,7 @@
 
 constexpr int kFinBlock = 1024;
 
-__global__ __launch_bounds__(kFinBlock) void finalize_kernel(const FinalizeParams p) {
+__device__ __forceinline__ void finalize_first_level(const FinalizeParams& p) {
     __shared__ uint32_t s_carry;
     __shared__ MonoRec s_mono[kFinBlock / 64];
     const int t = threadIdx.x, lane = t & 63, w = t >> 6;
@@ -698,7 +698,20 @@
     KPROF(blockIdx.x * 16 + w, 2);
 }
 
-__global__ __launch_bounds__(256) void finalize2_kernel(const FinalizeParams p) { finalize2_body(p); }
+__global__ __launch_bounds__(kFinBlock) void finalize_kernel(const FinalizeParams p) {
+    __shared__ uint32_t s_last;
+    finalize_first_level(p);
+    if (!p.ticket) return;
+    __threadfence();
+    __syncthreads();
+    if (threadIdx.x == 0) s_last = atomicInc(p.ticket, gridDim.x - 1) == gridDim.x - 1 ? 1u : 0u;
+    __syncthreads();
+    if (!s_last) return;
+    __threadfence();
+    finalize2_body<kFinBlock>(p);
+}
+
+__global__ __launch_bounds__(256) void finalize2_kernel(const FinalizeParams p) { finalize2_body<256>(p); }
 
 __global__ __launch_bounds__(256) void k0_init_kernel(const InitList l) {
     for (int f = 0; f < l.n; ++f)
@@ -714,8 +727,10 @@
 }
 
 void launch_finalize(const FinalizeParams& p, hipStream_t s, bool second_level) {
-    hipLaunchKernelGGL(finalize_kernel, dim3(p.ncols * p.nchunk + p.nfold), dim3(kFinBlock), 0, s, p);
-    if (second_level) hipLaunchKernelGGL(finalize2_kernel, dim3(1), dim3(256), 0, s, p);
+    FinalizeParams q = p;
+    if (!second_level) q.ticket = nullptr;
+    hipLaunchKernelGGL(finalize_kernel, dim3(p.ncols * p.nchunk + p.nfold), dim3(kFinBlock), 0, s, q);
+    if (second_level && !q.ticket) hipLaunchKernelGGL(finalize2_kernel, dim3(1), dim3(256), 0, s, p);
 }
 
 void launch_finalize2_only(const FinalizeParams& p, hipStream_t s) { hipLaunchKernelGGL(finalize2_kernel, dim3(1), dim3(256), 0, s, p); }
diff --git a/breakdancer_amd/csrc/k2_compact.hip b/breakdancer_amd/csrc/k2_compact.hip
--- a/breakdancer_amd/csrc/k2_compact.hip
+++ b/breakdancer_amd/csrc/k2_compact.hip
@@ -58,6 +58,219 @@
 }
 template <bool kBases> __device__ __forceinline__ uint32_t col_prefix(const K2Params& p, int col, uint32_t tile2, uint32_t chunk, int lane) {
     return p.tile_pre[(size_t)col * p.tstride + tile2] + chunk_sum<kBases>(chunk_word<kBases>(p, col, chunk, lane), chunk, lane);
+}
+
+struct K2Pre { uint32_t l_norm, l_anom, l_k0, l_k1, c_norm, c_anom, c_k0, c_k1; };
+
+template <bool kBases, bool kSummed>
+__device__ __forceinline__ void k2_from_columns(const K2Params& p, uint32_t tile2, uint32_t chunk, const K2Pre& pre, uint32_t* s_src, uint32_t* s_nn) {
+    const int nkeys = p.nkeys;
+    const int lane = threadIdx.x & 63, w = threadIdx.x >> 6;
+    const uint64_t base = (uint64_t)tile2 * kTile2 + (uint64_t)lane * kPerLane;
+    uint64_t cq[kSub / 2];
+#pragma unroll
+    for (int q = 0; q < kSub / 2; ++q) cq[q] = 0;
+    int nvalid = 0;
+    if (base + kPerLane <= p.n) {
+        nvalid = kPerLane;
+#pragma unroll
+        for (int q = 0; q < kSub / 4; ++q) {
+            const uint4 x = *(const uint4*)(p.cls + base + 16 * q);
+            cq[2 * q] = (uint64_t)x.x | ((uint64_t)x.y << 32);
+            cq[2 * q + 1] = (uint64_t)x.z | ((uint64_t)x.w << 32);
+        }
+    } else {
+#pragma unroll
+        for (int r = 0; r < kPerLane; ++r)
+            if (base + r < p.n) { ++nvalid; cq[r >> 3] |= (uint64_t)p.cls[base + r] << (8 * (r & 7)); }
+    }
+    uint32_t m_anom = 0, m_nleft = 0, m_pk = 0;
+#pragma unroll
+    for (int r = 0; r < kPerLane; ++r) {
+        const unsigned c = (unsigned)((cq[r >> 3] >> (8 * (r & 7))) & 255u);
+        const unsigned f = c & 15u;
+        const bool pass = r < nvalid && (c & 0x10u);
+        const bool normal = f == F_NORMAL_FR || f == F_NORMAL_RF;
+        m_anom |= (pass && !normal) ? 1u << r : 0u;
+        m_nleft |= (pass && (c & 0x40u)) ? 1u << r : 0u;
+        m_pk |= (pass && (c & 0x20u)) ? 1u << r : 0u;
+    }
+    if (!__any(m_anom != 0)) return;
+    const uint32_t pre_norm = kSummed ? pre.l_norm : pre.l_norm + chunk_sum<kBases>(pre.c_norm, chunk, lane);
+    const uint32_t rank0 = kSummed ? pre.l_anom : pre.l_anom + chunk_sum<kBases>(pre.c_anom, chunk, lane);
+    const uint32_t pre_k0 = kSummed ? pre.l_k0 : pre.l_k0 + chunk_sum<kBases>(pre.c_k0, chunk, lane);
+    const uint32_t pre_k1 = kSummed ? pre.l_k1 : pre.l_k1 + chunk_sum<kBases>(pre.c_k1, chunk, lane);
+
+    const uint32_t tot = (uint32_t)__popc(m_anom) + ((uint32_t)__popc(m_nleft) << 16);
+    const uint32_t ex0 = wave_incl_scan(tot) - tot;
+    const uint32_t nn0 = p.nn_base + pre_norm + (ex0 >> 16);
+    const uint32_t local0 = ex0 & 0xFFFFu;
+    const uint32_t cnt = __shfl((ex0 + tot) & 0xFFFFu, 63);
+    for (uint32_t win = 0; win < cnt; win += kSlice) {
+        {
+            uint32_t local = local0;
+            for (uint32_t mm = m_anom; mm; mm &= mm - 1, ++local) {
+                if (local < win || local >= win + kSlice) continue;
+                const int r = __builtin_ctz(mm);
+                s_src[w * kSlice + (local - win)] = (uint32_t)(lane * kPerLane + r) | (class_byte(cq, r) << kOffBits);
+                s_nn[w * kSlice + (local - win)] = nn0 + (uint32_t)__popc(m_nleft & ((1u << r) - 1u));
+            }
+        }
+        __builtin_amdgcn_wave_barrier();
+        const uint32_t wcnt = min((uint32_t)kSlice, cnt - win);
+        for (uint32_t b = 0; b < wcnt; b += 64) {
+            const uint32_t q = b + lane;
+            if (q < wcnt && rank0 + win + q < p.c.cap) {
+                const uint32_t src = s_src[w * kSlice + q];
+                const uint64_t i = (uint64_t)tile2 * kTile2 + (src & ((1u << kOffBits) - 1u));
+                const uint32_t j = rank0 + win + q;
+                const unsigned sam = p.r.flag[i];
+                p.c.tid[j] = p.r.tid[i];
+                p.c.pos[j] = p.r.pos[i];
+                p.c.isize[j] = abs(p.r.isize[i]);
+                uint64_t key, check = 0;
+                int qlen;
+                key_and_qlen_of(p, i, key, qlen, check);
+                p.c.meta[j] = meta_pack((int)((src >> kOffBits) & 15u), (sam >> 4) & 1u, lib_of(p, i), qlen);
+                p.c.key[j] = key;
+                if (p.c.check) p.c.check[j] = check;
+                p.c.idx[j] = (uint32_t)i;
+                p.c.nn[j] = s_nn[w * kSlice + q];
+            }
+        }
+        __builtin_amdgcn_wave_barrier();
+    }
+    uint64_t kq[kSub / 2];
+#pragma unroll
+    for (int q = 0; q < kSub / 2; ++q) kq[q] = 0;
+    if (nkeys > 1) {
+#pragma unroll
+        for (int r = 0; r < kPerLane; ++r)
+            if (r < nvalid) kq[r >> 3] |= (uint64_t)(p.libs[lib_of(p, base + r)].key & 255) << (8 * (r & 7));
+    }
+    for (int k0 = 0; k0 < nkeys; k0 += 2) {
+        uint32_t mk0 = 0, mk1 = 0;
+        if (nkeys > 1) {
+#pragma unroll
+            for (int r = 0; r < kPerLane; ++r) {
+                const int key = (int)((kq[r >> 3] >> (8 * (r & 7))) & 255u);
+                if ((m_pk >> r) & 1u) { mk0 |= key == k0 ? 1u << r : 0u; mk1 |= key == k0 + 1 ? 1u << r : 0u; }
+            }
+        } else {
+            mk0 = m_pk;
+        }
+        const uint32_t v = (uint32_t)__popc(mk0) + ((uint32_t)__popc(mk1) << 16);
+        const uint32_t ex = wave_incl_scan(v) - v;
+        const uint32_t b0 = p.pk_base[k0] + (k0 == 0 ? pre_k0 : col_prefix<kBases>(p, kColKey0 + k0, tile2, chunk, lane));
+        const uint32_t b1 = k0 + 1 < nkeys ? p.pk_base[k0 + 1] + (k0 == 0 ? pre_k1 : col_prefix<kBases>(p, kColKey0 + k0 + 1, tile2, chunk, lane)) : 0u;
+        uint32_t j = rank0 + local0;
+        for (uint32_t mm = m_anom; mm; mm &= mm - 1, ++j) {
+            if (j >= p.c.cap) break;
+            const int r = __builtin_ctz(mm);
+            const uint32_t upto = (2u << r) - 1u;
+            p.c.pk[(size_t)k0 * p.c.cap + j] = b0 + (ex & 0xFFFFu) + (uint32_t)__popc(mk0 & upto);
+            if (k0 + 1 < nkeys) p.c.pk[(size_t)(k0 + 1) * p.c.cap + j] = b1 + (ex >> 16) + (uint32_t)__popc(mk1 & upto);
+        }
+    }
+}
+
+constexpr int kGroupSuper = 4;
+constexpr int kGroupTiles = kGroupSuper * kSub;
+static_assert(kGroupTiles == 16 && 2 + kStashKeys <= 64 / kGroupTiles, "lane layout of a group's totals: 16 tiles x (2 + kStashKeys) columns");
+static_assert(kColAnom == 0 && kColNormal == 1 && kColKey0 == 2, "the lanes of a group's totals are in column order");
+
+template <bool kBases> __device__ __forceinline__ void k2_group(const K2Params& p, uint32_t grp, uint32_t ntiles2, uint32_t* s_src, uint32_t* s_nn) {
+    const int nkeys = p.nkeys, ncols = 2 + nkeys;
+    const int lane = threadIdx.x & 63;
+    const int tt = lane & (kGroupTiles - 1), col = lane >> 4;
+    const uint32_t tile0 = grp * kGroupTiles, super0 = grp * kGroupSuper;
+    const uint32_t chunk = super0 / p.chunk_super;
+    uint32_t v = 0;
+    if (col < ncols && tile0 + tt < p.ntiles) v = p.tile_tot[(size_t)col * p.tstride + tile0 + tt];
+    uint32_t pre16 = 0;
+    if (lane < 4 * kGroupSuper && (lane >> 2) < ncols && super0 + (lane & 3) < ntiles2) pre16 = p.tile_pre[(size_t)(lane >> 2) * p.tstride + super0 + (lane & 3)];
+    uint32_t cw[4];
+#pragma unroll
+    for (int c = 0; c < 4; ++c) cw[c] = c < ncols ? chunk_word<kBases>(p, c, chunk, lane) : 0u;
+    const uint32_t a = __shfl(v, tt);
+    uint32_t A = a;
+#pragma unroll
+    for (int o = 1; o < kGroupTiles; o <<= 1) A += __shfl_xor(A, o);
+    if (A == 0) return;
+    bool bad = a > (uint32_t)kStashCap;
+    if (lane < kGroupTiles && a != 0 && !bad) bad = p.stash[(size_t)(tile0 + tt) * kStashCap].where == 0xFFFFFFFFu;
+    const uint32_t badm = (uint32_t)ballot64(lane < kGroupTiles && bad);
+    const uint32_t f = ((badm >> (tt & ~3)) & 15u) ? 0u : a;
+    uint32_t F = f;
+#pragma unroll
+    for (int o = 1; o < kGroupTiles; o <<= 1) {
+        const uint32_t u = __shfl_up(F, o);
+        if (tt >= o) F += u;
+    }
+    const uint32_t Ftot = __shfl(F, kGroupTiles - 1);
+    uint32_t tb;
+    {
+        const uint32_t u1 = __shfl_up(v, 1), u2 = __shfl_up(v, 2), u3 = __shfl_up(v, 3);
+        const int k = tt & 3;
+        uint32_t cs = 0;
+#pragma unroll
+        for (int c = 0; c < 4; ++c) {
+            const uint32_t x = chunk_sum<kBases>(cw[c], chunk, lane);
+            cs = col == c ? x : cs;
+        }
+        tb = __shfl(pre16, col * 4 + (tt >> 2)) + cs + (k >= 1 ? u1 : 0u) + (k >= 2 ? u2 : 0u) + (k >= 3 ? u3 : 0u);
+    }
+    if (Ftot) {
+        uint32_t Fi[kGroupTiles];
+#pragma unroll
+        for (int i = 0; i < kGroupTiles; ++i) Fi[i] = __shfl(F, i);
+        for (uint32_t b = 0; b < Ftot; b += 64) {
+            const uint32_t q = b + (uint32_t)lane;
+            uint32_t tq = 0, before = 0;
+#pragma unroll
+            for (int i = 0; i < kGroupTiles; ++i) {
+                const bool ge = Fi[i] <= q;
+                tq += ge ? 1u : 0u;
+                before = ge ? Fi[i] : before;
+            }
+            const bool act = q < Ftot;
+            tq = min(tq, (uint32_t)kGroupTiles - 1u);
+            const uint32_t tile = tile0 + tq;
+            uint4 r0 = make_uint4(0u, 0u, 0u, 0u);
+            uint2 r1 = make_uint2(0u, 0u);
+            if (act) {
+                const StashRec* src = p.stash + (size_t)tile * kStashCap + (q - before);
+                r0 = *(const uint4*)src;
+                r1 = *(const uint2*)&src->where;
+            }
+            const uint32_t j = __shfl(tb, (int)tq) + (q - before);
+            const uint32_t b_nn = __shfl(tb, kGroupTiles + (int)tq), b_k0 = __shfl(tb, 2 * kGroupTiles + (int)tq), b_k1 = __shfl(tb, 3 * kGroupTiles + (int)tq);
+            if (act && j < p.c.cap) {
+                const uint64_t i = (uint64_t)tile * kTile + (r1.x & 255u);
+                const uint32_t k0 = (r1.x >> 20) & 63u;
+                uint64_t key, check = 0;
+                int qlen;
+                key_and_qlen_of(p, i, key, qlen, check);
+                p.c.tid[j] = (int32_t)r0.x;
+                p.c.pos[j] = (int32_t)r0.y;
+                p.c.isize[j] = (int32_t)r0.z;
+                p.c.meta[j] = r0.w | ((uint32_t)qlen << 16);
+                p.c.key[j] = key;
+                if (p.c.check) p.c.check[j] = check;
+                p.c.idx[j] = (uint32_t)i;
+                p.c.nn[j] = p.nn_base + b_nn + ((r1.x >> 8) & 511u);
+                p.c.pk[j] = p.pk_base[0] + b_k0 + (k0 == 0 ? r1.y : 0u);
+                if (nkeys > 1) p.c.pk[(size_t)p.c.cap + j] = p.pk_base[1] + b_k1 + (k0 == 1 ? r1.y : 0u);
+            }
+        }
+    }
+    for (int s = 0; s < kGroupSuper; ++s) {
+        if (!((badm >> (4 * s)) & 15u)) continue;
+        K2Pre pre{};
+        pre.l_anom = __shfl(tb, 4 * s); pre.l_norm = __shfl(tb, kGroupTiles + 4 * s);
+        pre.l_k0 = __shfl(tb, 2 * kGroupTiles + 4 * s); pre.l_k1 = __shfl(tb, 3 * kGroupTiles + 4 * s);
+        k2_from_columns<kBases, true>(p, super0 + s, chunk, pre, s_src, s_nn);
+    }
 }
 
 template <bool kBases> __device__ __forceinline__ void k2_body(const K2Params& p, uint32_t nblk) {
@@ -67,168 +280,20 @@
     const int lane = threadIdx.x & 63, w = threadIdx.x >> 6;
     const uint32_t nwaves = nblk * kWaves;
     const uint32_t ntiles2 = (p.ntiles + kSub - 1) / kSub;
+    if (p.stash) {
+        const uint32_t ngroups = (ntiles2 + kGroupSuper - 1) / kGroupSuper;
+        for (uint32_t grp = blockIdx.x * kWaves + w; grp < ngroups; grp += nwaves) k2_group<kBases>(p, grp, ntiles2, s_src, s_nn);
+        return;
+    }
     for (uint32_t tile2 = blockIdx.x * kWaves + w; tile2 < ntiles2; tile2 += nwaves) {
-        const uint64_t base = (uint64_t)tile2 * kTile2 + (uint64_t)lane * kPerLane;
         const uint32_t chunk = tile2 / p.chunk_super;
-        const uint32_t l_norm = p.tile_pre[(size_t)kColNormal * p.tstride + tile2], c_norm = chunk_word<kBases>(p, kColNormal, chunk, lane);
-        const uint32_t l_anom = p.tile_pre[(size_t)kColAnom * p.tstride + tile2], c_anom = chunk_word<kBases>(p, kColAnom, chunk, lane);
-        const uint32_t l_k0 = p.tile_pre[(size_t)kColKey0 * p.tstride + tile2], c_k0 = chunk_word<kBases>(p, kColKey0, chunk, lane);
-        const uint32_t l_k1 = nkeys > 1 ? p.tile_pre[(size_t)(kColKey0 + 1) * p.tstride + tile2] : 0u;
-        const uint32_t c_k1 = nkeys > 1 ? chunk_word<kBases>(p, kColKey0 + 1, chunk, lane) : 0u;
-        if (p.stash) {
-            static_assert(kSub == 4 && kStashKeys == 2, "lane layout of the totals");
-            const int t = lane & 3, col = lane >> 2;
-            uint32_t v = 0;
-            if (col < 2 + nkeys && tile2 * kSub + t < p.ntiles) v = p.tile_tot[(size_t)col * p.tstride + tile2 * kSub + t];
-            const uint32_t a0 = __shfl(v, 0), a1 = __shfl(v, 1), a2 = __shfl(v, 2), a3 = __shfl(v, 3);
-            const uint32_t A = a0 + a1 + a2 + a3;
-            if (A == 0) continue;
-            if (max(max(a0, a1), max(a2, a3)) <= (uint32_t)kStashCap) {
-                const uint32_t pre_norm = l_norm + chunk_sum<kBases>(c_norm, chunk, lane), rank0 = l_anom + chunk_sum<kBases>(c_anom, chunk, lane);
-                const uint32_t pre_k0 = l_k0 + chunk_sum<kBases>(c_k0, chunk, lane), pre_k1 = l_k1 + chunk_sum<kBases>(c_k1, chunk, lane);
-                const uint32_t q = (uint32_t)lane;
-                const uint32_t tq = (q >= a0 ? 1u : 0u) + (q >= a0 + a1 ? 1u : 0u) + (q >= a0 + a1 + a2 ? 1u : 0u);
-                const uint32_t before = tq == 0 ? 0u : (tq == 1 ? a0 : (tq == 2 ? a0 + a1 : a0 + a1 + a2));
-                uint32_t e[3];
-#pragma unroll
-                for (int c = 1; c <= 3; ++c) {
-                    const uint32_t x0 = __shfl(v, c * 4), x1 = __shfl(v, c * 4 + 1), x2 = __shfl(v, c * 4 + 2);
-                    e[c - 1] = tq == 0 ? 0u : (tq == 1 ? x0 : (tq == 2 ? x0 + x1 : x0 + x1 + x2));
-                }
-                const uint32_t j = rank0 + q;
-                const uint32_t tile = tile2 * kSub + min(tq, 3u);
-                uint4 r0 = make_uint4(0u, 0u, 0u, 0u);
-                uint2 r1 = make_uint2(0u, 0u);
-                if (q < A) {
-                    const StashRec* src = p.stash + (size_t)tile * kStashCap + (q - before);
-                    r0 = *(const uint4*)src;
-                    r1 = *(const uint2*)&src->where;
-                }
-                if (!__any(r1.x == 0xFFFFFFFFu)) {
-                    if (q < A && j < p.c.cap) {
-                        const uint64_t i = (uint64_t)tile * kTile + (r1.x & 255u);
-                        const uint32_t k0 = (r1.x >> 20) & 63u;
-                        uint64_t key, check = 0;
-                        int qlen;
-                        key_and_qlen_of(p, i, key, qlen, check);
-                        p.c.tid[j] = (int32_t)r0.x;
-                        p.c.pos[j] = (int32_t)r0.y;
-                        p.c.isize[j] = (int32_t)r0.z;
-                        p.c.meta[j] = r0.w | ((uint32_t)qlen << 16);
-                        p.c.key[j] = key;
-                        if (p.c.check) p.c.check[j] = check;
-                        p.c.idx[j] = (uint32_t)i;
-                        p.c.nn[j] = p.nn_base + pre_norm + e[0] + ((r1.x >> 8) & 511u);
-                        p.c.pk[j] = p.pk_base[0] + pre_k0 + e[1] + (k0 == 0 ? r1.y : 0u);
-                        if (nkeys > 1) p.c.pk[(size_t)p.c.cap + j] = p.pk_base[1] + pre_k1 + e[2] + (k0 == 1 ? r1.y : 0u);
-                    }
-                    continue;
-                }
-            }
-        }
-        uint64_t cq[kSub / 2];
-#pragma unroll
-        for (int q = 0; q < kSub / 2; ++q) cq[q] = 0;
-        int nvalid = 0;
-        if (base + kPerLane <= p.n) {
-            nvalid = kPerLane;
-#pragma unroll
-            for (int q = 0; q < kSub / 4; ++q) {
-                const uint4 x = *(const uint4*)(p.cls + base + 16 * q);
-                cq[2 * q] = (uint64_t)x.x | ((uint64_t)x.y << 32);
-                cq[2 * q + 1] = (uint64_t)x.z | ((uint64_t)x.w << 32);
-            }
-        } else {
-#pragma unroll
-            for (int r = 0; r < kPerLane; ++r)
-                if (base + r < p.n) { ++nvalid; cq[r >> 3] |= (uint64_t)p.cls[base + r] << (8 * (r & 7)); }
-        }
-        uint32_t m_anom = 0, m_nleft = 0, m_pk = 0;
-#pragma unroll
-        for (int r = 0; r < kPerLane; ++r) {
-            const unsigned c = (unsigned)((cq[r >> 3] >> (8 * (r & 7))) & 255u);
-            const unsigned f = c & 15u;
-            const bool pass = r < nvalid && (c & 0x10u);
-            const bool normal = f == F_NORMAL_FR || f == F_NORMAL_RF;
-            m_anom |= (pass && !normal) ? 1u << r : 0u;
-            m_nleft |= (pass && (c & 0x40u)) ? 1u << r : 0u;
-            m_pk |= (pass && (c & 0x20u)) ? 1u << r : 0u;
-        }
-        if (!__any(m_anom != 0)) continue;
-        const uint32_t pre_norm = l_norm + chunk_sum<kBases>(c_norm, chunk, lane), rank0 = l_anom + chunk_sum<kBases>(c_anom, chunk, lane);
-        const uint32_t pre_k0 = l_k0 + chunk_sum<kBases>(c_k0, chunk, lane), pre_k1 = l_k1 + chunk_sum<kBases>(c_k1, chunk, lane);
-
-        const uint32_t tot = (uint32_t)__popc(m_anom) + ((uint32_t)__popc(m_nleft) << 16);
-        const uint32_t ex0 = wave_incl_scan(tot) - tot;
-        const uint32_t nn0 = p.nn_base + pre_norm + (ex0 >> 16);
-        const uint32_t local0 = ex0 & 0xFFFFu;
-        const uint32_t cnt = __shfl((ex0 + tot) & 0xFFFFu, 63);
-        for (uint32_t win = 0; win < cnt; win += kSlice) {
-            {
-                uint32_t local = local0;
-                for (uint32_t mm = m_anom; mm; mm &= mm - 1, ++local) {
-                    if (local < win || local >= win + kSlice) continue;
-                    const int r = __builtin_ctz(mm);
-                    s_src[w * kSlice + (local - win)] = (uint32_t)(lane * kPerLane + r) | (class_byte(cq, r) << kOffBits);
-                    s_nn[w * kSlice + (local - win)] = nn0 + (uint32_t)__popc(m_nleft & ((1u << r) - 1u));
-                }
-            }
-            __builtin_amdgcn_wave_barrier();
-            const uint32_t wcnt = min((uint32_t)kSlice, cnt - win);
-            for (uint32_t b = 0; b < wcnt; b += 64) {
-                const uint32_t q = b + lane;
-                if (q < wcnt && rank0 + win + q < p.c.cap) {
-                    const uint32_t src = s_src[w * kSlice + q];
-                    const uint64_t i = (uint64_t)tile2 * kTile2 + (src & ((1u << kOffBits) - 1u));
-                    const uint32_t j = rank0 + win + q;
-                    const unsigned sam = p.r.flag[i];
-                    p.c.tid[j] = p.r.tid[i];
-                    p.c.pos[j] = p.r.pos[i];
-                    p.c.isize[j] = abs(p.r.isize[i]);
-                    uint64_t key, check = 0;
-                    int qlen;
-                    key_and_qlen_of(p, i, key, qlen, check);
-                    p.c.meta[j] = meta_pack((int)((src >> kOffBits) & 15u), (sam >> 4) & 1u, lib_of(p, i), qlen);
-                    p.c.key[j] = key;
-                    if (p.c.check) p.c.check[j] = check;
-                    p.c.idx[j] = (uint32_t)i;
-                    p.c.nn[j] = s_nn[w * kSlice + q];
-                }
-            }
-            __builtin_amdgcn_wave_barrier();
-        }
-        uint64_t kq[kSub / 2];
-#pragma unroll
-        for (int q = 0; q < kSub / 2; ++q) kq[q] = 0;
-        if (nkeys > 1) {
-#pragma unroll
-            for (int r = 0; r < kPerLane; ++r)
-                if (r < nvalid) kq[r >> 3] |= (uint64_t)(p.libs[lib_of(p, base + r)].key & 255) << (8 * (r & 7));
-        }
-        for (int k0 = 0; k0 < nkeys; k0 += 2) {
-            uint32_t mk0 = 0, mk1 = 0;
-            if (nkeys > 1) {
-#pragma unroll
-                for (int r = 0; r < kPerLane; ++r) {
-                    const int key = (int)((kq[r >> 3] >> (8 * (r & 7))) & 255u);
-                    if ((m_pk >> r) & 1u) { mk0 |= key == k0 ? 1u << r : 0u; mk1 |= key == k0 + 1 ? 1u << r : 0u; }
-                }
-            } else {
-                mk0 = m_pk;
-            }
-            const uint32_t v = (uint32_t)__popc(mk0) + ((uint32_t)__popc(mk1) << 16);
-            const uint32_t ex = wave_incl_scan(v) - v;
-            const uint32_t b0 = p.pk_base[k0] + (k0 == 0 ? pre_k0 : col_prefix<kBases>(p, kColKey0 + k0, tile2, chunk, lane));
-            const uint32_t b1 = k0 + 1 < nkeys ? p.pk_base[k0 + 1] + (k0 == 0 ? pre_k1 : col_prefix<kBases>(p, kColKey0 + k0 + 1, tile2, chunk, lane)) : 0u;
-            uint32_t j = rank0 + local0;
-            for (uint32_t mm = m_anom; mm; mm &= mm - 1, ++j) {
-                if (j >= p.c.cap) break;
-                const int r = __builtin_ctz(mm);
-                const uint32_t upto = (2u << r) - 1u;
-                p.c.pk[(size_t)k0 * p.c.cap + j] = b0 + (ex & 0xFFFFu) + (uint32_t)__popc(mk0 & upto);
-                if (k0 + 1 < nkeys) p.c.pk[(size_t)(k0 + 1) * p.c.cap + j] = b1 + (ex >> 16) + (uint32_t)__popc(mk1 & upto);
-            }
-        }
+        K2Pre pre;
+        pre.l_norm = p.tile_pre[(size_t)kColNormal * p.tstride + tile2]; pre.c_norm = chunk_word<kBases>(p, kColNormal, chunk, lane);
+        pre.l_anom = p.tile_pre[(size_t)kColAnom * p.tstride + tile2]; pre.c_anom = chunk_word<kBases>(p, kColAnom, chunk, lane);
+        pre.l_k0 = p.tile_pre[(size_t)kColKey0 * p.tstride + tile2]; pre.c_k0 = chunk_word<kBases>(p, kColKey0, chunk, lane);
+        pre.l_k1 = nkeys > 1 ? p.tile_pre[(size_t)(kColKey0 + 1) * p.tstride + tile2] : 0u;
+        pre.c_k1 = nkeys > 1 ? chunk_word<kBases>(p, kColKey0 + 1, chunk, lane) : 0u;
+        k2_from_columns<kBases, false>(p, tile2, chunk, pre, s_src, s_nn);
     }
 }
 
@@ -246,7 +311,7 @@
 __global__ __launch_bounds__(kBlock) void k2_compact_side_kernel(const K2Params p, const FinalizeParams fp) {
     k2_fills(p);
     if (blockIdx.x == gridDim.x - 1) {
-        finalize2_body(fp);
+        finalize2_body<kBlock>(fp);
         return;
     }
     k2_body<false>(p, gridDim.x - 1);
@@ -254,7 +319,8 @@
 
 void launch_k2(const K2Params& p, size_t lds, hipStream_t s, const FinalizeParams* side) {
     const uint32_t ntiles2 = (p.ntiles + kSub - 1) / kSub;
-    const uint32_t nblk = (ntiles2 + kWaves - 1) / kWaves;
+    const uint32_t nunits = p.stash ? (ntiles2 + kGroupSuper - 1) / kGroupSuper : ntiles2;
+    const uint32_t nblk = (nunits + kWaves - 1) / kWaves;
     const uint32_t cap = 8192u;
     const uint32_t grid = nblk < cap ? nblk : cap;
     if (side) hipLaunchKernelGGL(k2_compact_side_kernel, dim3(grid + 1), dim3(kBlock), lds, s, p, *side);
diff --git a/breakdancer_amd/csrc/k6_assemble.hip b/breakdancer_amd/csrc/k6_assemble.hip
--- a/breakdancer_amd/csrc/k6_assemble.hip
+++ b/breakdancer_amd/csrc/k6_assemble.hip
@@ -1059,7 +1059,7 @@
 
 constexpr uint32_t kInsLds = 2048;
 constexpr uint32_t kInsThreads = 1024;
-constexpr uint32_t kInsBucketMax = 8192;
+constexpr uint32_t kInsBucketMax = kK6InsBucketMax;
 constexpr uint32_t kInsCntLds = 10240;
 constexpr uint32_t kInsBuckets = 2048;
 constexpr uint32_t kInsBucketDepth = 128;
@@ -1549,10 +1549,20 @@
         }
         __builtin_amdgcn_wave_barrier();
     }
+    if (a.done_ticket && (bid * (kScanBlock / 64) + (uint32_t)w) * 64u < n_sv) __threadfence_system();
     __syncthreads();
     if (tid == 0) {
         if (s_printed) atomicAdd(&a.counts->n_printed, s_printed);
         if (a.printed_host) a.printed_host[bid] = s_printed;
+        if (a.done_ticket) {
+            __threadfence_system();
+            if (atomicInc(a.done_ticket, gridDim.x - 1) == gridDim.x - 1) {
+                __threadfence();
+                if (a.counts_host2) a.counts_host2->n_printed = atomicAdd(&a.counts->n_printed, 0u);
+                __threadfence_system();
+                *(volatile uint32_t*)a.flag_done = a.flag_value;
+            }
+        }
     }
     KPROF(kp, 5);
 }
@@ -1621,7 +1631,7 @@
         hipLaunchKernelGGL(k6_place_kernel, dim3(scan_grid(a.fin_regions ? a.fin_regions : a.cap, 1)), dim3(kScanBlock), 0, s, a);
         hipLaunchKernelGGL(k6_score_kernel, dim3(k6_score_grid(a)), dim3(kScanBlock), 0, s, a, ln10, score_threshold, with_scores);
     }
-    if (!a.printed_host || a.flag_done) hipLaunchKernelGGL(k6_done_kernel, dim3(1), dim3(64), 0, s, a);
+    if ((!a.printed_host || a.flag_done) && !(n_anom_host && a.done_ticket)) hipLaunchKernelGGL(k6_done_kernel, dim3(1), dim3(64), 0, s, a);
 }
 
 }
```

New measurement: 25.13 billion. -12.0%, worse.
